# NVIDIA/tensorrt-laboratory

Measured on NVIDIA H100. Metric: ResNet-50 fp16 b=8 inferences/sec, higher is better.
Workload: dtype f16

## Files before the change

__graft_entry__.py:

```python
from __future__ import annotations

import os
import re
import shutil
import subprocess
import sysconfig
import sys

ROOT = os.path.dirname(os.path.abspath(__file__))
PKG = os.path.join(ROOT, "tensorrt_laboratory_b200")
CSRC = os.path.join(PKG, "csrc")
LIB = os.path.join(PKG, "libb200infer.so")

NVCC_FLAGS = [
    "-gencode", "arch=compute_90a,code=sm_90a", "-lineinfo", "-O3", "-std=c++17",
    "-Xcompiler", "-fPIC,-Wall,-Wno-unused-function", "-cudart", "static",
]


def _nvcc() -> str:
    for cand in (os.environ.get("NVCC"), shutil.which("nvcc"), "/usr/local/cuda/bin/nvcc"):
        if cand and os.path.exists(cand):
            return cand
    raise RuntimeError("nvcc not found")


def _sources():
    srcs = []
    for root, _, files in os.walk(CSRC):
        for f in sorted(files):
            if f.endswith((".cu", ".cc")) and not f.endswith(("_main.cc", "_module.cc")):
                srcs.append(os.path.join(root, f))
    return srcs


def _stale(target: str, deps) -> bool:
    if not os.path.exists(target):
        return True
    t = os.path.getmtime(target)
    for d in deps:
        if os.path.getmtime(d) > t:
            return True
    return False


def _all_deps():
    deps = []
    for root, _, files in os.walk(CSRC):
        deps += [os.path.join(root, f) for f in files if f.endswith((".cu", ".cc", ".h", ".cuh", ".hpp"))]
    deps.append(os.path.join(ROOT, "include", "b200infer.h"))
    inc = os.path.join(ROOT, "include")
    for root, _, files in os.walk(inc):
        deps += [os.path.join(root, f) for f in files]
    return deps


_CONV_KERNEL = re.compile(r"conv|attention_f16_wgmma|embed_ln|layernorm_h8|pooler|patchify|tokens_kernel|cls_head")


_SHARED_SM_KERNEL = re.compile(r"_ZN3b2k(?:16conv_f16_tcgen05|20conv3x3_halo_tcgen05|24conv3x3_halo_1x1_tcgen05)ILi(\d+)E")
_SHARED_SM_THREADS = 320


def _shared_sm_register_budget(bn: int):
    ctas = 3 if bn <= 64 else 2 if bn <= 128 else 1
    return None if ctas == 1 else 65536 // (_SHARED_SM_THREADS * ctas) // 8 * 8


def _ptxas_violations(log: str):
    bad = [line.strip() for line in log.splitlines() if "(C7520)" in line or "(C7518)" in line]
    func = None
    for line in log.splitlines():
        m = re.search(r"Function properties for (\S+)", line)
        if m:
            func = m.group(1)
            continue
        m = re.search(r"(\d+) bytes spill stores, (\d+) bytes spill loads", line)
        if m and func and _CONV_KERNEL.search(func) and (int(m.group(1)) or int(m.group(2))):
            bad.append(f"{func}: {line.strip()}")
        m = re.search(r"Used (\d+) registers", line)
        k = _SHARED_SM_KERNEL.match(func) if (m and func) else None
        if k:
            budget = _shared_sm_register_budget(int(k.group(1)))
            if budget is not None and int(m.group(1)) > budget:
                bad.append(f"{func}: {m.group(1)} registers, more than the {budget} at which its CTAs share an SM")
    return bad


def _compile_object(cmd, obj: str, verbose: bool) -> None:
    r = subprocess.run(cmd + ["-Xptxas", "-v"], capture_output=True, text=True)
    log = r.stdout + r.stderr
    shown = [line for line in log.splitlines() if verbose or not (line.startswith("ptxas info") or "bytes stack frame" in line)]
    if shown:
        sys.stderr.write("\n".join(shown) + "\n")
    if r.returncode:
        raise subprocess.CalledProcessError(r.returncode, cmd)
    bad = _ptxas_violations(log)
    if bad:
        os.remove(obj)
        raise RuntimeError(f"{os.path.basename(obj)}: ptxas reports serialised wgmma, spilling convolution / transformer "
                           "kernels or tile kernels over their register budget:\n  " +
                           "\n  ".join(bad))


def build(force: bool = False, verbose: bool = False) -> None:
    nvcc = _nvcc()
    objdir = os.path.join(ROOT, "build", "obj")
    os.makedirs(objdir, exist_ok=True)
    deps = _all_deps()
    objs = []
    for src in _sources():
        obj = os.path.join(objdir, os.path.relpath(src, CSRC).replace(os.sep, "_") + ".o")
        objs.append(obj)
        if force or _stale(obj, deps):
            cmd = [nvcc] + NVCC_FLAGS + ["-I", os.path.join(ROOT, "include"), "-I", CSRC]
            if src.endswith(".cc"):
                cmd += ["-x", "cu"]
            cmd += ["-c", src, "-o", obj]
            if verbose:
                print(" ".join(cmd))
            _compile_object(cmd, obj, verbose)
    if force or _stale(LIB, objs):
        cmd = [nvcc, "-shared", "-cudart", "static", "-o", LIB] + objs + ["-lpthread", "-ldl", "-lrt"]
        if verbose:
            print(" ".join(cmd))
        subprocess.run(cmd, check=True)
    main_src = os.path.join(CSRC, "trtlab", "infer_main.cc")
    exe = os.path.join(ROOT, "examples", "infer.x")
    os.makedirs(os.path.dirname(exe), exist_ok=True)
    if os.path.exists(main_src) and (force or _stale(exe, deps + [LIB])):
        cmd = [nvcc] + NVCC_FLAGS + ["-I", os.path.join(ROOT, "include"), "-I", CSRC, "-x", "cu", main_src,
                                     "-o", exe, "-L", PKG, "-lb200infer", "-Xlinker", "-rpath,$ORIGIN/../tensorrt_laboratory_b200",
                                     "-lpthread", "-ldl"]
        if verbose:
            print(" ".join(cmd))
        subprocess.run(cmd, check=True)
    py_src = os.path.join(CSRC, "pybind", "trtlab_module.cc")
    py_mod = os.path.join(PKG, "trtlab" + sysconfig.get_config_var("EXT_SUFFIX"))
    if os.path.exists(py_src) and (force or _stale(py_mod, deps + [LIB, py_src])):
        import pybind11
        cmd = [nvcc] + NVCC_FLAGS + ["-I", os.path.join(ROOT, "include"), "-I", CSRC, "-I", pybind11.get_include(),
                                     "-I", sysconfig.get_paths()["include"], "-Xcompiler", "-fvisibility=hidden", "-x", "cu", "-shared", py_src,
                                     "-o", py_mod,
# ... 25 lines not shown
```

tensorrt_laboratory_b200/csrc/engine.cu:

```cuda
#include <cuda.h>
#include <cuda_runtime.h>
#include <stdarg.h>
#include <stdio.h>
#include <stdlib.h>
#include <string.h>

#include <algorithm>
#include <map>
#include <memory>
#include <mutex>
#include <string>
#include <vector>

#include "../../include/b200infer.h"
#include "kernels.h"
#include "plan_format.h"

#include "b2_internal.h"

namespace b2i {
thread_local std::string g_err;
int fail(int code, const char* fmt, ...) {
    char buf[1024];
    va_list ap;
// ... 45 lines not shown
        }
        g_encode_im2col = reinterpret_cast<EncodeIm2colFn>(fn);
        cudaDriverGetVersion(&g_driver_version);
    });
    return g_driver_status;
}

size_t align_up(size_t v, size_t a) { return (v + a - 1) / a * a; }
constexpr size_t kSplitWorkspaceBytes = 12u << 20;
constexpr int kMaxSplitTiles = 4096;
constexpr int kSmemLimit = 227 * 1024;

int env_int(const char* name, int dflt) {
    const char* v = getenv(name);
    return v ? atoi(v) : dflt;
}

struct Tensor {
    std::string name;
    uint32_t kind, h, w, c, c_phys;
    int binding;
    float scale = 0.f;
    size_t item_bytes = 0;
    size_t offset = 0;
    int def = -1, last_use = -1;
};

struct Op {
    b2plan::OpRec r;
    int groups = 1;
    int heads = 0, vocab = 0, positions = 0, types = 0;
    int binding2 = -1, binding3 = -1, out2 = -1;
    float eps = 0.f;
    uint32_t flags = 0;
    std::string name;
    int side_join = -1;
    int kh() const { return int(r.k); }
    int kw() const { return int(r.kw ? r.kw : r.k); }
    int sh() const { return int(r.stride); }
    int sw() const { return int(r.kw ? r.stride_w : r.stride); }
    int ph() const { return int(r.pad_); }
    int pw_lo() const { return int(r.kw ? r.pad_w_lo : r.pad_); }
    int pw_hi() const { return int(r.kw ? r.pad_w_hi : r.pad_); }
    double algo_k() const { return r.ceil_mode ? double(r.ceil_mode) : double(r.cin / uint32_t(groups)) * r.taps; }
    int group_span() const {
        return groups > 1 && (r.relu & 2) ? std::max(int(r.cin) / groups, (r.relu & 4) ? 128 : 64) : 0;
    }
};

struct Binding {
    std::string name;
    bool is_input;
    int dtype;
    int tensor;
    int nd;
    int32_t dims[8];
    size_t item_bytes;
};

enum LKind { L_INPUT_CAST, L_CONV_TC, L_CONV_SIMT, L_MAXPOOL, L_AVGPOOL, L_FC, L_SOFTMAX, L_OUTPUT_CAST, L_TAIL, L_QUANTIZE, L_CONV_I8, L_AVGPOOL_I8, L_OUTPUT_CAST_I8,
             L_EMBED_LN, L_LAYERNORM, L_ATTENTION, L_POOLER, L_OUTPUT_ROWS, L_OUTPUT_UNPACK, L_QUANTIZE_F8, L_CONV_F8, L_AVGPOOL_F8,
             L_OUTPUT_CAST_F8, L_PATCHIFY, L_TOKENS, L_CLS_HEAD };

int attention_keys(int S) {
    for (int sk : {64, 128, 256, 384, 512})
        if (S <= sk) return sk;
    return 0;
}

struct Launch {
    LKind kind;
    std::string name;
    double flops = 0, bytes = 0;
    b2k::ConvLaunch conv;
    b2k::SimtConvArgs simt;
    const void* in = nullptr;
    void* out = nullptr;
    const void* w = nullptr;
    const float* bias = nullptr;
    int in_binding = -1, out_binding = -1;
    bool src_half = false;
    int max_blocks = 0;
    int side_join = -1;
    b2k::TailArgs tail{};
    b2k::I8ConvLaunch i8{};
    float qscale = 0.f;
    int C_in_phys = 0;
    b2k::EmbedArgs embed{};
    int in_binding2 = -1, in_binding3 = -1;
    b2k::AttnLaunch attn{};
    float eps = 0.f;
    const int* live = nullptr;
    const int* pos_map = nullptr;
    int N = 0, C = 0, H = 0, W = 0, C_phys = 0, Ho = 0, Wo = 0, k = 0, stride = 0, pad = 0, K = 0, Cout = 0;
};

struct Segment {
    int begin = 0, end = 0;
    bool graphable = false;
    cudaGraphExec_t exec = nullptr;
};
struct BindPatch {
    int launch = -1;
    cudaGraphNode_t node = nullptr;
    cudaKernelNodeParams np{};
    std::vector<void*> params;
    int n_params = 0;
    std::vector<std::pair<int, int>> slots;
    std::vector<void*> values;
    b2k::TailArgs tail{};
    bool is_tail = false;
};
struct Plan {
    int batch = 0;
    std::vector<Launch> launches;
    std::vector<Segment> segments;
    bool graph_failed = false;
    cudaGraph_t graph = nullptr;
    cudaGraphExec_t exec = nullptr;
    std::vector<BindPatch> patches;
    ~Plan() {
        for (Segment& sg : segments)
            if (sg.exec) cudaGraphExecDestroy(sg.exec);
        if (exec) cudaGraphExecDestroy(exec);
        if (graph) cudaGraphDestroy(graph);
    }
};

}

struct ConvConfig {
    int bn, stages, splits;
    double est_us;
    int sps = 1;
    int ws = 0;
    int cn = 1;
    int halo = 0;
};
static bool stage_depth_useful(int bn, int kb, int st, int kpc) {
    const int stgs[4] = {1, 2, 4, 8};
    int cover = 0, deepest = 0;
    for (int s2 : stgs) {
        if (!b2k::conv_config_exists(bn, kb, s2)) continue;
        deepest = s2;
        if (!cover && s2 >= kpc) cover = s2;
    }
    return st <= (cover ? cover : deepest);
}


constexpr int kHaloStagesTag = 2;

struct b2_runtime {
    b2_alloc_fn alloc = nullptr;
    b2_free_fn free_ = nullptr;
    void* user = nullptr;
};

struct b2_engine {
    b2_runtime* rt = nullptr;
    b2_alloc_fn alloc = nullptr;
    b2_free_fn free_ = nullptr;
    void* alloc_user = nullptr;
    std::string name;
    int precision = 0, max_batch = 0;
    std::vector<Tensor> tensors;
    std::vector<Op> ops;
    std::vector<Binding> bindings;
    uint8_t* d_payload = nullptr;
    size_t payload_bytes = 0;
    size_t arena_bytes = 0;
    size_t act_bytes = 0;
    int device = -1;
    bool inspect_only = false;
    double flops_per_item = 0;
    std::mutex tune_mutex;
    std::mutex tune_run_mutex;
    std::map<std::pair<int, int>, ConvConfig> tuned;
    bool tune_cache_loaded = false;
    std::map<int, float> requant_r;
    bool tactics_from_plan = false;
    bool tuned_at_load = false;
    int pack_tensor = -1;
    bool half() const { return precision != B2_PREC_FP32; }
    bool one_byte() const { return precision == B2_PREC_INT8 || precision == B2_PREC_FP8; }
    bool fp8() const { return precision == B2_PREC_FP8; }
};

struct b2_context {
    b2_engine* e = nullptr;
    uint8_t* scratch = nullptr;
    struct ScratchState {
        std::map<int, std::unique_ptr<Plan>> plans;
    };
    std::map<uint8_t*, ScratchState> states;
    ScratchState* cur = nullptr;
    int* d_counters = nullptr;
    int use_graph = 1;
    int force_simt = 0;
    int force_im2col = 0;
    int force_bn = 0;
    int force_stages = 0;
    int force_splits = 0;
    int force_sps = 0;
    int force_halo = 0;
    int force_fuse = 0;
    int force_cn = 0;
    int force_ws = 0;
    int pdl_trigger = 1;
    int no_fold = 0;
    int autotune = 4;
    int fork = 0;
    int i8_bn = 0;
    int i8_stages = 0;
    int fuse_tail = 1;
    int input_ctas = 0;
    int* d_tail_ctrl = nullptr;
    cudaStream_t side = nullptr;
    cudaEvent_t fork_ev = nullptr, join_ev = nullptr;
};

namespace {

std::string fixed_str(const char* p, size_t n) {
    size_t len = 0;
    while (len < n && p[len]) ++len;
    return std::string(p, len);
}

int validate_transformer_op(b2_engine* e, const Op& op) {
    using namespace b2plan;
    const OpRec& r = op.r;
    const char* nm = op.name.c_str();
    auto act_ok = [&](const Tensor& t) { return t.kind == T_ACT && t.scale == 0.f && t.c % 8 == 0 && t.c <= 1024; };
    switch (r.type) {
        case OP_EMBED_LN: {
            const Tensor& to = e->tensors[r.out];
            const Tensor& tm = e->tensors[op.out2];
            const uint32_t want_c = (op.flags & kOpPacked) ? to.w + 2 : to.w;
            if (!act_ok(to) || to.h != 1 || tm.kind != T_VEC || tm.c != want_c || tm.binding >= 0)
                return fail(B2_EINVAL, "plan: embedding %s: needs an fp16 [1, S, C <= 1024, C %% 8 == 0] output and an fp32 [S] mask tensor "
                            "([S + 2] packing index when packed)", nm);
            if ((op.flags & kOpPacked) && to.w % 32)
                return fail(B2_EINVAL, "plan: packed embedding %s: S = %u is not a multiple of 32", nm, to.w);
            if (op.vocab < 1 || op.types < 1 || op.positions < int(to.w))
                return fail(B2_EINVAL, "plan: embedding %s: vocab %d / positions %d / types %d do not cover S = %u", nm, op.vocab, op.positions,
                            op.types, to.w);
            if (r.w_bytes != uint64_t(op.vocab + op.positions + op.types) * to.c * 2 || r.b_bytes != uint64_t(to.c) * 8)
                return fail(B2_EINVAL, "plan: embedding %s: table / gamma / beta sizes do not match hidden size %u", nm, to.c);
            if (!(op.eps >= 0.f && op.eps < 1.f)) return fail(B2_EINVAL, "plan: embedding %s: bad eps", nm);
            break;
        }
        case OP_LAYERNORM: {
            const Tensor& ti = e->tensors[r.in];
            const Tensor& to = e->tensors[r.out];
            if (!act_ok(ti) || !act_ok(to) || ti.h != to.h || ti.w != to.w || ti.c != to.c || ti.c_phys != to.c_phys)
                return fail(B2_EINVAL, "plan: layernorm %s: needs fp16 input and output of one shape, C %% 8 == 0, C <= 1024", nm);
            if (r.w_bytes != 0 || r.b_bytes != uint64_t(ti.c) * 8) return fail(B2_EINVAL, "plan: layernorm %s: gamma / beta size mismatch", nm);
            if (!(op.eps >= 0.f && op.eps < 1.f)) return fail(B2_EINVAL, "plan: layernorm %s: bad eps", nm);
            break;
        }
        case OP_ATTENTION: {
            const Tensor& ti = e->tensors[r.in];
            const Tensor& to = e->tensors[r.out];
            if (r.res < 0) return fail(B2_EINVAL, "plan: attention %s: no mask tensor", nm);
            const Tensor& tm = e->tensors[r.res];
            if (op.heads < 1 || uint32_t(op.heads) * 64 != to.c)
                return fail(B2_EINVAL, "plan: attention %s: heads * 64 (%d * 64) != hidden size %u", nm, op.heads, to.c);
            if (!act_ok(to) || ti.kind != T_ACT || ti.scale != 0.f || ti.c != 3 * to.c || ti.c_phys != ti.c)
                return fail(B2_EINVAL, "plan: attention %s: needs a fused fp16 QKV input of 3 x %u channels", nm, to.c);
            if (ti.h != 1 || to.h != 1 || ti.w != to.w || tm.kind != T_VEC || tm.c != ((op.flags & kOpPacked) ? ti.w + 2 : ti.w))
                return fail(B2_EINVAL, "plan: attention %s: S does not match between QKV, output and mask", nm);
            if ((op.flags & kOpPacked) && (ti.w == 0 || ti.w > 512))
                return fail(B2_EINVAL, "plan: packed attention %s: S = %u (1 ... 512)", nm, ti.w);
            if (!(op.flags & kOpPacked) && ti.w != 64 && (ti.w == 0 || ti.w % 128 || ti.w > 512))
                return fail(B2_EINVAL, "plan: attention %s: S = %u (64, or a multiple of 128 up to 512)", nm, ti.w);
            if (r.w_bytes || r.b_bytes) return fail(B2_EINVAL, "plan: attention %s carries no weights", nm);
            e->flops_per_item += 4.0 * double(ti.w) * ti.w * to.c;
            break;
        }
        case OP_POOLER: {
            const Tensor& ti = e->tensors[r.in];
            const Tensor& to = e->tensors[r.out];
            if (!act_ok(ti) || ti.h != 1 || to.kind != T_VEC || to.c != ti.c)
                return fail(B2_EINVAL, "plan: pooler %s: needs an fp16 [1, S, C] input and an fp32 [C] output", nm);
            if (r.w_bytes != uint64_t(ti.c) * ti.c * 2 || r.b_bytes != uint64_t(ti.c) * 4)
                return fail(B2_EINVAL, "plan: pooler %s: weight / bias size mismatch", nm);
            e->flops_per_item += 2.0 * ti.c * ti.c;
            break;
// ... 295 lines not shown
            const Tensor& ti = e->tensors[r.in];
            const size_t K = size_t(ti.h) * ti.w * ti.c_phys;
            if (r.w_bytes != size_t(r.cout) * K * elt || r.b_bytes != size_t(r.cout) * 4)
                return fail(B2_EINVAL, "plan: fc %s weight size mismatch", op.name.c_str());
            e->flops_per_item += 2.0 * ti.h * ti.w * ti.c * r.cout;
        } else if (transformer_op) {
            int rc = validate_transformer_op(e, op);
            if (rc) return rc;
        }
        e->ops.push_back(op);
    }
    if (int rc = validate_packed_ops(e)) return rc;
    for (uint32_t i = 0; i < h.n_bindings; ++i, p += sizeof(BindingRec)) {
        BindingRec r;
        memcpy(&r, p, sizeof r);
        Binding b;
        b.name = fixed_str(r.name, 64);
        b.is_input = r.is_input != 0;
        b.dtype = r.dtype;
        b.tensor = r.tensor;
        b.nd = r.nd;
        if (r.nd == 0 || r.nd > 8) return fail(B2_EINVAL, "plan: binding %s has bad rank", b.name.c_str());
        if (r.dtype != B2_DT_FLOAT && !(r.dtype == B2_DT_HALF && b.is_input && h.precision == B2_PREC_FP16) &&
            !(r.dtype == B2_DT_INT32 && b.is_input && v3))
            return fail(B2_EINVAL, "plan: binding %s: bindings are fp32 (inputs of fp16 engines may be fp16)", b.name.c_str());
        size_t n = 1;
        for (uint32_t d = 0; d < 8; ++d) {
            b.dims[d] = d < r.nd ? r.dims[d] : 0;
            if (d < r.nd) n *= size_t(r.dims[d]);
        }
        b.item_bytes = n * (r.dtype == B2_DT_HALF ? 2 : 4);
        e->bindings.push_back(b);
    }
    for (const Op& op : e->ops) {
        const OpRec& r = op.r;
        if (r.type != OP_INPUT_CAST && r.type != OP_OUTPUT_CAST) continue;
        const Binding& b = e->bindings[size_t(r.binding)];
        const Tensor& t = e->tensors[size_t(r.type == OP_INPUT_CAST ? r.out : r.in)];
        size_t n = 1;
        for (int d = 0; d < b.nd; ++d) n *= size_t(b.dims[d] > 0 ? b.dims[d] : 0);
        const bool s2d = r.type == OP_INPUT_CAST && r.k == 2;
        if (b.is_input != (r.type == OP_INPUT_CAST) || (!s2d && n != size_t(t.c) * t.h * t.w))
            return fail(B2_EINVAL, "plan: cast op %s: binding %s and tensor %s disagree", op.name.c_str(), b.name.c_str(), t.name.c_str());
        if (b.dtype == B2_DT_INT32)
            return fail(B2_EINVAL, "plan: cast op %s reads int32 binding %s (int32 bindings feed the embedding op only)", op.name.c_str(),
                        b.name.c_str());
    }
    for (const Op& op : e->ops)
        if (op.r.type == OP_PATCHIFY)
            if (int rc = validate_patchify_binding(e, op)) return rc;
    std::vector<int> int32_readers(e->bindings.size(), 0);
    for (const Op& op : e->ops) {
        const OpRec& r = op.r;
        if (r.type == OP_POOLER && e->tensors[r.out].binding >= 0 && e->bindings[size_t(e->tensors[r.out].binding)].is_input)
            return fail(B2_EINVAL, "plan: pooler %s writes an input binding", op.name.c_str());
        if (r.type != OP_EMBED_LN) continue;
        const uint32_t S = e->tensors[r.out].w;
        for (int bi : {r.binding, op.binding2, op.binding3}) {
            if (bi < 0 || bi >= int(h.n_bindings)) return fail(B2_EINVAL, "plan: embedding %s has a bad binding", op.name.c_str());
            const Binding& b = e->bindings[size_t(bi)];
            if (b.dtype != B2_DT_INT32 || !b.is_input || b.nd != 1 || b.dims[0] != int32_t(S))
                return fail(B2_EINVAL, "plan: embedding %s: binding %s must be an int32 input of shape [S = %u]", op.name.c_str(), b.name.c_str(), S);
            ++int32_readers[size_t(bi)];
        }
    }
    for (size_t i = 0; i < e->bindings.size(); ++i) {
        if (e->bindings[i].dtype != B2_DT_INT32) continue;
        if (int32_readers[i] != 1)
            return fail(B2_EINVAL, "plan: int32 binding %s must feed exactly one embedding op slot", e->bindings[i].name.c_str());
        for (const Tensor& t : e->tensors)
            if (t.binding == int(i))
                return fail(B2_EINVAL, "plan: int32 binding %s is the storage of tensor %s (int32 bindings feed the embedding op only)",
                            e->bindings[i].name.c_str(), t.name.c_str());
    }
    if (h.n_tactics) {
        if (h.tactics_offset > nbytes || size_t(h.n_tactics) > (nbytes - h.tactics_offset) / sizeof(TacticRec))
            return fail(B2_EINVAL, "plan: tactic table outside the blob");
        for (uint32_t i = 0; i < h.n_tactics; ++i) {
            TacticRec t;
            memcpy(&t, base + h.tactics_offset + size_t(i) * sizeof(TacticRec), sizeof t);
            if (t.op >= h.n_ops || t.batch == 0 || t.batch > h.max_batch) return fail(B2_EINVAL, "plan: tactic %u out of range", i);
            ConvConfig cfg{int(t.bn), int(t.stages), int(t.splits), 0.0, int(t.sps), int(t.ws), int(t.cn)};
            cfg.halo = int(t.halo);
            e->tuned[{int(t.op), int(t.batch)}] = cfg;
        }
        e->tactics_from_plan = true;
    }
    *payload = base + h.payload_offset;
    return B2_OK;
}

int fuse_partner(const b2_engine* e, int i);

void plan_arena(b2_engine* e) {
    int busy_until = -1;
    for (size_t i = 0; i < e->ops.size(); ++i) {
        Op& op = e->ops[i];
        op.side_join = -1;
        if (int(i) <= busy_until || op.r.type != b2plan::OP_CONV || op.r.out < 0 || e->tensors[op.r.out].binding >= 0) continue;
        int consumers = 0, join = -1;
        bool as_residual_only = true;
        for (size_t k = i + 1; k < e->ops.size(); ++k) {
            const auto& rk = e->ops[k].r;
            if (rk.in == op.r.out) ++consumers, as_residual_only = false;
            if (rk.res == op.r.out) ++consumers, join = int(k);
        }
        if (consumers == 1 && as_residual_only && join > int(i) + 1) {
            op.side_join = join;
            busy_until = join;
        }
    }
    for (size_t i = 0; i < e->ops.size(); ++i) {
        const auto& r = e->ops[i].r;
        for (int t : {r.out, e->ops[i].out2})
            if (t >= 0 && e->tensors[t].def < 0) e->tensors[t].def = int(i);
        for (int t : {r.in, r.res})
            if (t >= 0) e->tensors[t].last_use = std::max(e->tensors[t].last_use, int(i));
        if (e->ops[i].side_join >= 0 && r.in >= 0) e->tensors[r.in].last_use = std::max(e->tensors[r.in].last_use, e->ops[i].side_join);
        const int j = fuse_partner(e, int(i));
        if (j >= 0) e->tensors[r.in].last_use = std::max(e->tensors[r.in].last_use, j);
    }
    if (e->pack_tensor >= 0) e->tensors[size_t(e->pack_tensor)].last_use = int(e->ops.size()) - 1;
    struct Live {
        size_t off, size;
        int last;
    };
    std::vector<Live> live;
    size_t top = 0;
    std::vector<int> order;
    for (size_t i = 0; i < e->tensors.size(); ++i)
        if (e->tensors[i].binding < 0 && e->tensors[i].def >= 0) order.push_back(int(i));
    std::stable_sort(order.begin(), order.end(), [&](int a, int b) { return e->tensors[a].def < e->tensors[b].def; });
    for (int ti : order) {
        Tensor& t = e->tensors[ti];
        if (t.last_use < t.def) t.last_use = t.def;
        const size_t size = align_up(t.item_bytes * e->max_batch, 1024);
        live.erase(std::remove_if(live.begin(), live.end(), [&](const Live& l) { return l.last < t.def; }), live.end());
        std::sort(live.begin(), live.end(), [](const Live& a, const Live& b) { return a.off < b.off; });
        size_t off = 0;
        for (const Live& l : live) {
            if (off + size <= l.off) break;
            off = std::max(off, l.off + l.size);
        }
        t.offset = off;
        live.push_back({off, size, t.last_use});
        top = std::max(top, off + size);
    }
    e->act_bytes = align_up(std::max<size_t>(top, 1024), 1024);
    e->arena_bytes = e->act_bytes + (e->half() ? kSplitWorkspaceBytes : 0);
}

int make_map_2d(CUtensorMap* map, const void* base, uint64_t inner, uint64_t outer, uint32_t box_inner,
                uint32_t box_outer, CUtensorMapSwizzle swz, bool int8 = false) {
    cuuint64_t dims[2] = {inner, outer};
    cuuint64_t strides[1] = {inner * (int8 ? 1u : 2u)};
    cuuint32_t box[2] = {box_inner, box_outer};
    cuuint32_t estr[2] = {1, 1};
    CUresult r = g_encode_tiled(map, int8 ? CU_TENSOR_MAP_DATA_TYPE_UINT8 : CU_TENSOR_MAP_DATA_TYPE_FLOAT16, 2, const_cast<void*>(base), dims, strides, box,
                                estr, CU_TENSOR_MAP_INTERLEAVE_NONE, swz, CU_TENSOR_MAP_L2_PROMOTION_L2_256B,
                                CU_TENSOR_MAP_FLOAT_OOB_FILL_NONE);
    if (r != CUDA_SUCCESS)
        return fail(B2_ECUDA, "cuTensorMapEncodeTiled failed (%d) dims=%llu,%llu box=%u,%u", int(r),
                    (unsigned long long)inner, (unsigned long long)outer, box_inner, box_outer);
    return B2_OK;
}

// ... 42 lines not shown
        if (cout_phys % bn || (group_span && group_span % bn)) continue;
        if (honor_forced && c->force_bn && bn != c->force_bn) continue;
        const int tiles = m_tiles * (cout_phys / bn);
        for (int splits = 1; splits <= 8; ++splits) {
            if (honor_forced && c->force_splits && !group_span ? splits != c->force_splits : splits != 1) continue;
            if (splits > 1 && (kb != 64 || kblocks / splits < 4 || tiles * splits > 160 || tiles > kMaxSplitTiles ||
                               size_t(tiles) * splits * 128 * bn * 4 > kSplitWorkspaceBytes))
                continue;
            const int kpc = (kblocks + splits - 1) / splits;
            if (splits > 1 && (splits - 1) * kpc >= kblocks) continue;
            for (int st : stgs) {
                if (!b2k::conv_config_exists(bn, kb, st)) continue;
                if (b2k::conv_smem_bytes(bn, st, residual) > kSmemLimit) continue;
                if (honor_forced && c->force_stages && st != c->force_stages) continue;
                if (!(honor_forced && c->force_stages) && !stage_depth_useful(bn, kb, st, kpc)) continue;
                const int per_sm = std::max(1, b2k::conv_residency(bn, kb, st, 1, residual));
                const int ctas = tiles * splits;
                const int waves = (ctas + g_sms * per_sm - 1) / (g_sms * per_sm);
                const int sharing = std::max(1, std::min(per_sm, (ctas + g_sms - 1) / g_sms));
                const double stage_bytes = 16384.0 + bn * 128.0;
                const double t_kb = std::max(stage_bytes / (70000.0 / sharing), 1.0 / st);
                double t_epi = 0.6 + bn / 64.0 * 0.4 + (residual ? 0.4 : 0.0);
                if (splits > 1) t_epi += 1.0 + 0.3 * splits;
                const double t_cta = 2.0 + kpc * t_kb + t_epi;
                double total = waves * t_cta;
                const double traffic = double(ctas) * kpc * stage_bytes;
                total = std::max(total, traffic / 5.0e6 + 2.0);
                if (total < best.est_us) best = ConvConfig{bn, st, splits, total};
            }
        }
    }
    return best;
}

bool conv_is_row_folded(const b2_context* c, const Op& op) {
    const b2plan::OpRec& r = op.r;
    return !c->no_fold && r.cin_phys == 8 && op.kw() * 8 * 2 == 64 && op.sw() == 1 && op.pw_lo() == 0 && op.pw_hi() == 0;
}
int conv_kb(const b2_context* c, const Op& op) {
    if (op.r.cin_phys % 64 == 0) return 64;
    return conv_is_row_folded(c, op) ? 32 : 8;
}
int conv_num_kblocks(const b2_context* c, const Op& op) {
    const b2plan::OpRec& r = op.r;
    if (op.group_span()) return int(r.taps) * (op.group_span() / 64);
    if (r.cin_phys % 64 == 0) return int(r.taps) * (int(r.cin_phys) / 64);
    if (conv_is_row_folded(c, op)) return (op.kh() + 1) / 2;
    return (int(r.taps_phys) + 7) / 8;
}

int conv_halo_rows(const b2_engine* e, const Op& op) {
    const b2plan::OpRec& r = op.r;
    const Tensor& ti = e->tensors[r.in];
    const Tensor& to = e->tensors[r.out];
    if (op.groups > 1 || r.cin_phys % 64 || r.cout_phys % 64 || op.kh() != 3 || op.kw() != 3 || op.sh() != 1 || op.sw() != 1 || op.ph() != 1 ||
        op.pw_lo() != 1 || op.pw_hi() != 1 || r.res >= 0 || !(r.relu & 2) || ti.h != to.h || ti.w != to.w)
        return 0;
    const int wp = int(to.w) + 2;
    if (wp > 128) return 0;
    return std::min(128 / wp, int(to.h));
}
int conv_halo_rows(const b2_context* c, const Op& op) { return conv_halo_rows(c->e, op); }
bool conv_on_tensor_cores(const b2_engine* e, const Op& op);

int fuse_partner(const b2_engine* e, int i) {
    if (!e->half() || e->one_byte() || i < 0 || size_t(i) + 1 >= e->ops.size()) return -1;
    const Op &oi = e->ops[size_t(i)], &oj = e->ops[size_t(i) + 1];
    const b2plan::OpRec &ri = oi.r, &rj = oj.r;
    if (ri.type != b2plan::OP_CONV || rj.type != b2plan::OP_CONV || (ri.relu & (4 | b2plan::kConvGelu)) || conv_halo_rows(e, oi) == 0 ||
        !b2k::conv_halo_config_exists(int(ri.cout_phys)) || ri.cin_phys / 64 > 8)
        return -1;
    if (rj.in != ri.out || rj.res < 0 || rj.res == ri.out || oj.kh() != 1 || oj.kw() != 1 || oj.sh() != 1 || oj.sw() != 1 || oj.ph() != 0 ||
        oj.pw_lo() != 0 || oj.pw_hi() != 0 || oj.groups != 1 || !(rj.relu & 2) || (rj.relu & (4 | b2plan::kConvGelu)) ||
        rj.cin_phys != ri.cout_phys || rj.cout_phys % 64 || !conv_on_tensor_cores(e, oj) || e->tensors[ri.out].binding >= 0)
        return -1;
    for (size_t k = 0; k < e->ops.size(); ++k) {
        const b2plan::OpRec& rk = e->ops[k].r;
        if (k != size_t(i) + 1 && (rk.in == ri.out || rk.res == ri.out || e->ops[k].out2 == ri.out)) return -1;
        if (k == size_t(i) + 1 && rk.res == ri.out) return -1;
    }
    return i + 1;
}

bool conv_on_tensor_cores(const b2_engine* e, const Op& op) {
    const b2plan::OpRec& r = op.r;
    const bool kb64 = r.cin_phys % 64 == 0, kb8 = r.cin_phys == 8;
    return e->half() && (kb64 || kb8) && r.cout_phys % 32 == 0 && (kb64 || r.taps_phys % 2 == 0) && (op.groups == 1 || op.group_span() > 0);
}

bool conv_takes_stem_ws(const b2_context* c, const Op& op) {
    const b2plan::OpRec& r = op.r;
    return conv_is_row_folded(c, op) && op.kh() == 7 && op.sh() == 2 && r.cout_phys == 64 && c->e->tensors[r.out].w <= 128 &&
           (r.relu & b2plan::kConvRelu) && !(r.relu & 2) && !(r.relu & b2plan::kConvGelu) && r.res < 0 && op.groups == 1;
}

bool conv_takes_ws(const b2_context* c, const Op& op) {
    return conv_takes_stem_ws(c, op) || (conv_kb(c, op) == 64 && (op.r.relu & 2) && op.groups == 1 && !(op.r.relu & b2plan::kConvGelu));
}

bool tactic_applies(const b2_context* c, const Op& op, int batch, const ConvConfig& cfg) {
    const b2plan::OpRec& r = op.r;
    const Tensor& to = c->e->tensors[r.out];
    const int span = op.group_span(), kb = conv_kb(c, op);
    if (cfg.bn <= 0 || int(r.cout_phys) % cfg.bn || cfg.splits < 1 || cfg.sps < 1 || cfg.ws < 0) return false;
    if (op.groups > 1 && (!span || span % cfg.bn || cfg.splits > 1)) return false;
    if ((op.groups > 1 || (r.relu & b2plan::kConvGelu)) && (cfg.ws || cfg.cn > 1 || cfg.halo)) return false;
    if ((op.flags & b2plan::kOpPacked) && (cfg.ws || cfg.cn > 1 || cfg.halo || cfg.splits > 1)) return false;
    if (cfg.halo == 2) {
        const int j = fuse_partner(c->e, int(&op - &c->e->ops[0]));
        const int R = conv_halo_rows(c, op), cblocks = int(r.cin_phys) / 64;
        return j >= 0 && c->force_fuse >= 0 && cfg.bn == int(r.cout_phys) && cfg.splits == 1 && !cfg.ws && cfg.cn <= 1 &&
               b2k::conv_halo_fused_smem(cfg.bn, int(to.w), R, cblocks, int(c->e->ops[size_t(j)].r.cout_phys)) <= kSmemLimit;
    }
    if (cfg.halo) {
        const int R = conv_halo_rows(c, op), cblocks = int(r.cin_phys) / 64;
        return cfg.halo == 1 && R && cfg.splits == 1 && !cfg.ws && cfg.cn <= 1 && b2k::conv_halo_config_exists(cfg.bn) && cblocks <= 8 &&
               b2k::conv_halo_smem(cfg.bn, int(to.w), R, cblocks) <= kSmemLimit;
    }
    if (cfg.ws && conv_is_row_folded(c, op))
        return conv_takes_stem_ws(c, op) && cfg.bn == 64 && cfg.stages == b2k::kStemWsRing && cfg.sps == 1 && cfg.splits == 1 &&
               cfg.cn <= 1 && b2k::conv_stem_ws_smem() <= kSmemLimit;
    if (cfg.ws)
        return conv_takes_ws(c, op) && cfg.splits == 1 && cfg.cn <= 1 && b2k::conv_ws_config_exists(cfg.bn, cfg.stages, cfg.sps) &&
               b2k::conv_ws_smem(cfg.bn, cfg.stages, cfg.sps, r.res >= 0) <= kSmemLimit;
    if (!b2k::conv_config_exists(cfg.bn, kb, cfg.stages, cfg.sps) || b2k::conv_smem_bytes(cfg.bn, cfg.stages, r.res >= 0, cfg.sps) > kSmemLimit)
        return false;
    const int grid_n = int(r.cout_phys) / cfg.bn;
    if (cfg.cn > 1 && (kb != 64 || grid_n % cfg.cn || !b2k::conv_cluster_config_exists(cfg.bn, cfg.stages, cfg.sps, cfg.cn))) return false;
    if (cfg.splits > 1) {
        const int nkb = conv_num_kblocks(c, op), kpc = (nkb + cfg.splits - 1) / cfg.splits;
        const int tiles = (batch * int(to.h * to.w) + 127) / 128 * grid_n;
        if (kb != 64 || kpc < 4 || (cfg.splits - 1) * kpc >= nkb || tiles > kMaxSplitTiles ||
            size_t(tiles) * cfg.splits * 128 * cfg.bn * 4 > kSplitWorkspaceBytes)
            return false;
    }
    return true;
}

constexpr int kFuseMinStreams = 4;

ConvConfig fused_conv_config(const Op& op) {
    ConvConfig f{int(op.r.cout_phys), kHaloStagesTag, 1, 0.0, 1, 0, 1};
    f.halo = 2;
    return f;
}

std::vector<ConvConfig> conv_candidates(const b2_context* c, const Op& op, int batch, int fixed_splits) {
    const b2plan::OpRec& r = op.r;
    const int kbsz = conv_kb(c, op), nkb = conv_num_kblocks(c, op);
    const int m_tiles = (batch * int(c->e->tensors[r.out].h * c->e->tensors[r.out].w) + 127) / 128;
    const bool ws_only = c->force_ws > 0 && conv_takes_ws(c, op);
    auto ok = [&](const ConvConfig& t) { return tactic_applies(c, op, batch, t); };
    std::vector<ConvConfig> out;
    for (int bn : {256, 128, 64, 32}) {
        if (int(r.cout_phys) % bn) continue;
        const int tiles = m_tiles * (int(r.cout_phys) / bn);
        for (int ws = 0; ws <= 1; ++ws)
        for (int sp : {1, 2, 4, 8})
        for (int sps = 1; sps <= 2; ++sps)
        for (int st : {1, 2, 4, 8}) {
            if ((fixed_splits > 0 && sp != fixed_splits) || (ws ? c->force_ws < 0 : ws_only)) continue;
            ConvConfig t{bn, st, sp, 0.0, sps, ws ? std::min(tiles, g_sms) : 0, 1};
            if (!ok(t)) continue;
            if (ws) {
                if (sps == 2 && nkb < 4) continue;
                out.push_back(t);
                if (tiles > g_sms / 2) t.ws = g_sms / 2, out.push_back(t);
                continue;
            }
            const int kpc = (nkb + sp - 1) / sp;
            if (sps == 2 ? (kpc < 4 || st * 2 > kpc + 2) : !stage_depth_useful(bn, kbsz, st, kpc)) continue;
            if (sp > 1 && (tiles >= 100 || tiles > kMaxSplitTiles / 8 || tiles * sp > 160)) continue;
            ConvConfig cl = t;
            cl.cn = c->force_cn;
            out.push_back(c->force_cn > 1 && ok(cl) ? cl : t);
        }
    }
    if (conv_takes_stem_ws(c, op) && c->force_ws >= 0 && fixed_splits <= 1) {
        const int rows = batch * int(c->e->tensors[r.out].h);
        ConvConfig t{64, b2k::kStemWsRing, 1, 0.0, 1, std::min(rows, g_sms), 1};
        if (ok(t)) {
            out.push_back(t);
            if (rows > g_sms / 2) t.ws = g_sms / 2, out.push_back(t);
        }
    }
    if (c->force_halo >= 0 && fixed_splits <= 1) {
        std::vector<ConvConfig> halo;
        for (int bn : {256, 128, 64, 32}) {
            const ConvConfig h{bn, kHaloStagesTag, 1, 0.0, 1, 0, 1, 1};
            if (ok(h)) halo.push_back(h);
        }
        if (!halo.empty() && c->force_halo > 0) out.clear();
        out.insert(out.end(), halo.begin(), halo.end());
    }
    return out;
}

ConvConfig forced_conv_config(const b2_context* c, const Op& op, int batch) {
    const b2plan::OpRec& r = op.r;
    const int M = batch * int(c->e->tensors[r.out].h * c->e->tensors[r.out].w);
    const int kbsz = conv_kb(c, op), nkb = conv_num_kblocks(c, op);
    ConvConfig cfg = pick_conv_config(M, int(r.cout_phys), nkb, kbsz, r.res >= 0, c, true, op.group_span());
    if (cfg.bn == 0 || ((op.flags & b2plan::kOpPacked) && cfg.splits > 1))
        cfg = pick_conv_config(M, int(r.cout_phys), nkb, kbsz, r.res >= 0, c, false, op.group_span());
    if (cfg.bn == 0) return cfg;
    auto force = [&](auto set) {
        ConvConfig t = cfg;
        set(t);
        if (tactic_applies(c, op, batch, t)) cfg = t;
    };
    if (c->force_sps == 2) force([](ConvConfig& t) { t.sps = 2; });
    if (c->force_ws > 0)
        force([&](ConvConfig& t) {
            if (conv_takes_stem_ws(c, op)) {
                t = ConvConfig{64, b2k::kStemWsRing, 1, t.est_us, 1, 0, 1};
                t.ws = std::min(batch * int(c->e->tensors[r.out].h), c->force_ws > 1 ? c->force_ws : g_sms);
                return;
            }
            t.ws = std::min((M + 127) / 128 * (int(r.cout_phys) / t.bn), c->force_ws > 1 ? c->force_ws : g_sms);
        });
    if (c->force_halo > 0) force([](ConvConfig& t) { t.halo = 1, t.ws = 0, t.cn = 1; });
    if (c->force_cn > 1) force([&](ConvConfig& t) { t.cn = c->force_cn; });
    return cfg;
}

int make_conv_launch(b2_context* c, const Op& op, int batch, const ConvConfig& cfg, b2k::ConvLaunch* out) {
    b2_engine* e = c->e;
// ... 23 lines not shown
    cl.cn = std::max(cfg.cn, 1);
    cl.args.cn = cl.cn;
    cl.args.tiles_m = cl.grid_m;
    cl.args.tiles_n = cl.grid_n;
    b2k::ConvArgs& a = cl.args;
    a.splits = cfg.splits;
    a.kb_per_split = (nkb + cfg.splits - 1) / cfg.splits;
    a.workspace = reinterpret_cast<float*>(c->scratch + e->act_bytes);
    a.tile_counters = c->d_counters;
    a.pdl_trigger = c->pdl_trigger;
    a.bias = reinterpret_cast<const float*>(e->d_payload + r.b_off);
    a.residual = r.res >= 0 ? reinterpret_cast<const __half*>(tptr(r.res)) : nullptr;
    a.out = reinterpret_cast<__half*>(tptr(r.out));
    a.M = M;
    a.Cout = int(r.cout_phys);
    a.taps = fold ? op.kh() : int(r.taps);
    a.taps_phys = fold ? op.kh() : int(r.taps_phys);
    a.kw = fold ? 1 : op.kw();
    a.cblocks = span ? span / 64 : kb64 ? int(r.cin_phys) / 64 : 1;
    a.group_span = span;
    a.num_kblocks = nkb;
    a.HoWo = int(to.h * to.w);
    a.Wo = int(to.w);
    a.stride_h = op.sh();
    a.stride_w = op.sw();
    a.pad_h = op.ph();
    a.pad_w = op.pw_lo();
    a.relu = int(r.relu & (b2plan::kConvRelu | b2plan::kConvGelu));
    a.wpacked = (r.relu & 2) ? w : nullptr;
    const bool tiled = r.k == 1 && op.kw() == 1 && r.stride == 1 && op.sw() == 1 && r.pad_ == 0 && op.pw_lo() == 0 &&
                       op.pw_hi() == 0 && kb64 && (!c->force_im2col || gelu || (op.flags & b2plan::kOpPacked));
    a.a_mode = tiled ? b2k::A_TILED : b2k::A_IM2COL;
    if (cfg.halo) {
        const int R = conv_halo_rows(c, op);
        cl.halo = 1;
        cl.ws_ctas = 0, cl.cn = 1, a.cn = 1, a.splits = 1, cl.stages = kHaloStagesTag, cl.sps = 1;
        a.halo_rows = R;
        cl.grid_m = batch * ((int(to.h) + R - 1) / R);
        int rc = make_map_nhwc(&cl.mapA, tptr(r.in), int(r.cin_phys), int(ti.w), int(ti.h), batch, uint32_t(ti.w) + 2, uint32_t(R) + 2);
        if (rc) return rc;
        cl.mapB = cl.mapA;
        if (cfg.halo == 2) {
            const Op& oj = e->ops[size_t(fuse_partner(e, int(&op - &e->ops[0])))];
            const b2plan::OpRec& rj = oj.r;
            cl.halo = 2;
            cl.c2.wpacked = e->d_payload + rj.w_off;
            cl.c2.bias = reinterpret_cast<const float*>(e->d_payload + rj.b_off);
            cl.c2.Cout = int(rj.cout_phys);
            cl.c2.relu = int(rj.relu & b2plan::kConvRelu);
            rc = make_map_nhwc(&cl.mapOut, tptr(rj.out), int(rj.cout_phys), int(to.w), int(to.h), batch, uint32_t(to.w) + 2, uint32_t(R));
            if (!rc) rc = make_map_nhwc(&cl.mapRes, tptr(rj.res), int(rj.cout_phys), int(to.w), int(to.h), batch, uint32_t(to.w) + 2, uint32_t(R));
            return rc;
        }
        rc = make_map_nhwc(&cl.mapOut, tptr(r.out), int(r.cout_phys), int(to.w), int(to.h), batch, uint32_t(to.w) + 2, uint32_t(R));
        cl.mapRes = cl.mapOut;
        return rc;
    }
    const CUtensorMapSwizzle swz = kb64 ? CU_TENSOR_MAP_SWIZZLE_128B : (fold ? CU_TENSOR_MAP_SWIZZLE_64B : CU_TENSOR_MAP_SWIZZLE_NONE);
    const uint64_t pix = uint64_t(r.cin_phys) * 2, rowb = uint64_t(ti.w) * pix, imgb = uint64_t(ti.h) * rowb;
    int rc;
    if (tiled)
        rc = make_map_2d(&cl.mapA, tptr(r.in), r.cin_phys, uint64_t(M), 64, uint32_t(128 / cl.cn), swz);
    else if (fold)
        rc = make_map_im2col(&cl.mapA, tptr(r.in), int(r.cin_phys) * op.kw(), int(ti.w) - op.kw() + 1, int(ti.h), batch, pix,
                             rowb, imgb, op.kh(), 1, op.sh(), 1, op.ph(), 0, 0, 32, 128, swz);
    else
        rc = make_map_im2col(&cl.mapA, tptr(r.in), int(r.cin_phys), int(ti.w), int(ti.h), batch, pix, rowb, imgb, op.kh(),
                             op.kw(), op.sh(), op.sw(), op.ph(), op.pw_lo(), op.pw_hi(), uint32_t(cl.kb), uint32_t(128 / cl.cn), swz);
    if (rc) return rc;
    if (r.relu & 2)
        cl.mapB = cl.mapA;
    else
        rc = make_map_2d(&cl.mapB, w, uint64_t(r.taps_phys) * r.cin_phys, r.cout_phys, uint32_t(cl.kb), uint32_t(cl.bn), swz);
    if (rc) return rc;
    if (cfg.ws && fold) {
        rc = make_map_nhwc(&cl.mapOut, tptr(r.out), int(r.cout_phys), int(to.w), int(to.h), batch, 128, 1);
        cl.mapRes = cl.mapOut;
        return rc;
    }
    const uint32_t ow = cl.bn >= 64 ? 64 : 32;
    const CUtensorMapSwizzle oswz = cl.bn >= 64 ? CU_TENSOR_MAP_SWIZZLE_128B : CU_TENSOR_MAP_SWIZZLE_64B;
    rc = make_map_2d(&cl.mapOut, tptr(r.out), r.cout_phys, uint64_t(M), ow, 128, oswz);
    if (rc) return rc;
    if (r.res >= 0) rc = make_map_2d(&cl.mapRes, tptr(r.res), r.cout_phys, uint64_t(M), ow, 128, oswz);
    else cl.mapRes = cl.mapOut;
    return rc;
}

int make_i8_conv_launch(b2_context* c, const Op& op, int batch, int bn, int stages, b2k::I8ConvLaunch* out) {
    b2_engine* e = c->e;
    const b2plan::OpRec& r = op.r;
    const Tensor& ti = e->tensors[r.in];
    const Tensor& to = e->tensors[r.out];
    auto tptr = [&](int idx) -> uint8_t* { return c->scratch + e->tensors[idx].offset; };
    b2k::I8ConvLaunch& cl = *out;
    memset(&cl, 0, sizeof cl);
    const int M = batch * int(to.h) * int(to.w);
    cl.bn = bn, cl.stages = stages;
    cl.grid_m = (M + 127) / 128;
    cl.grid_n = int(r.cout_phys) / bn;
    b2k::I8ConvArgs& a = cl.args;
    a.wpacked = e->d_payload + r.w_off;
    const float* rq = reinterpret_cast<const float*>(e->d_payload + r.b_off);
    a.m = rq;
    a.b = rq + r.cout_phys;
    a.r = e->requant_r.at(int(&op - &e->ops[0]));
    a.has_res = r.res >= 0 ? 1 : 0;
    a.relu = int(r.relu & 1);
    a.M = M, a.Cout = int(r.cout_phys);
    const int span = op.group_span(), cpg = int(r.cin) / op.groups;
    a.group_span = span;
    cl.group_mode = !span ? 0 : cpg <= 32 ? 32 : cpg == 64 ? 64 : 128;
    a.cblocks = (span ? span : int(r.cin_phys)) / 128;
    a.last_cb_mmas = (int(r.cin) % 128) ? (int(r.cin) % 128 + 31) / 32 : 4;
    a.cout_real = int(r.cout);
    a.num_kblocks = int(r.taps) * a.cblocks;
    a.kw = op.kw(), a.HoWo = int(to.h * to.w), a.Wo = int(to.w);
    a.stride_h = op.sh(), a.stride_w = op.sw(), a.pad_h = op.ph(), a.pad_w = op.pw_lo();
    const bool tiled = r.k == 1 && r.stride == 1 && r.pad_ == 0;
    a.a_mode = tiled ? b2k::A_TILED : b2k::A_IM2COL;
    int rc;
    if (tiled)
        rc = make_map_2d(&cl.mapA, tptr(r.in), r.cin_phys, uint64_t(M), 128, 128, CU_TENSOR_MAP_SWIZZLE_128B, true);
    else {
        const uint64_t pix = uint64_t(r.cin_phys), rowb = uint64_t(ti.w) * pix, imgb = uint64_t(ti.h) * rowb;
        rc = make_map_im2col(&cl.mapA, tptr(r.in), int(r.cin_phys), int(ti.w), int(ti.h), batch, pix, rowb, imgb, op.kh(), op.kw(), op.sh(),
                             op.sw(), op.ph(), op.pw_lo(), op.pw_hi(), 128, 128, CU_TENSOR_MAP_SWIZZLE_128B, true);
    }
    if (rc) return rc;
    rc = make_map_2d(&cl.mapOut, tptr(r.out), r.cout_phys, uint64_t(M), 128, 128, CU_TENSOR_MAP_SWIZZLE_128B, true);
    if (rc) return rc;
    if (r.res >= 0) rc = make_map_2d(&cl.mapRes, tptr(r.res), r.cout_phys, uint64_t(M), 128, 128, CU_TENSOR_MAP_SWIZZLE_128B, true);
    else cl.mapRes = cl.mapOut;
    return rc;
}

struct TuneTimer {
    const int ns;
    const int iters = std::max(4, env_int("B2_TUNE_ITERS", 12));
    const int reps = std::max(1, env_int("B2_TUNE_REPS", 3));
    std::vector<cudaStream_t> ss;
    std::vector<cudaEvent_t> done;
    cudaEvent_t e0 = nullptr, e1 = nullptr;

    explicit TuneTimer(const b2_context* c) : ns(std::max(1, std::min(c->autotune, 8))), ss(size_t(ns), nullptr), done(size_t(ns), nullptr) {}
    ~TuneTimer() {
        for (auto s : ss)
            if (s) cudaStreamDestroy(s);
        for (auto d : done)
            if (d) cudaEventDestroy(d);
        if (e0) cudaEventDestroy(e0);
        if (e1) cudaEventDestroy(e1);
    }
    int init() {
        bool ok = cudaEventCreate(&e0) == cudaSuccess && cudaEventCreate(&e1) == cudaSuccess;
        for (int i = 0; i < ns && ok; ++i)
            ok = cudaStreamCreateWithFlags(&ss[size_t(i)], cudaStreamNonBlocking) == cudaSuccess &&
                 cudaEventCreateWithFlags(&done[size_t(i)], cudaEventDisableTiming) == cudaSuccess;
        if (ok) return B2_OK;
        cudaGetLastError();
        return fail(B2_ECUDA, "autotune: cannot create streams/events");
    }
    template <class F>
    cudaError_t time(F launch, float* ms) {
        int rc = 0;
        for (int i = 0; i < 2 && !rc; ++i)
            for (int k = 0; k < ns && !rc; ++k) rc = launch(k, ss[size_t(k)]);
        for (auto s : ss) cudaStreamSynchronize(s);
        *ms = 1e30f;
// ... 2 lines not shown
        cudaGraphExec_t ge = nullptr;
        cudaError_t se = cudaStreamBeginCapture(ss[0], cudaStreamCaptureModeThreadLocal);
        if (se != cudaSuccess) return se;
        cudaEventRecord(done[0], ss[0]);
        for (int k = 1; k < ns; ++k) cudaStreamWaitEvent(ss[size_t(k)], done[0], 0);
        for (int i = 0; i < iters && !rc; ++i)
            for (int k = 0; k < ns && !rc; ++k) rc = launch(k, ss[size_t(k)]);
        for (int k = 1; k < ns; ++k) {
            cudaEventRecord(done[size_t(k)], ss[size_t(k)]);
            cudaStreamWaitEvent(ss[0], done[size_t(k)], 0);
        }
        se = cudaStreamEndCapture(ss[0], &g);
        if (!rc && se == cudaSuccess) se = cudaGraphInstantiate(&ge, g, 0);
        if (!rc && se == cudaSuccess) se = cudaGraphLaunch(ge, ss[0]);
        if (!rc && se == cudaSuccess) se = cudaStreamSynchronize(ss[0]);
        for (int rep = 0; rep < reps && !rc && se == cudaSuccess; ++rep) {
            cudaEventRecord(e0, ss[0]);
            se = cudaGraphLaunch(ge, ss[0]);
            cudaEventRecord(e1, ss[0]);
            if (se == cudaSuccess) se = cudaStreamSynchronize(ss[0]);
            float t = 0.f;
            if (se == cudaSuccess && cudaEventElapsedTime(&t, e0, e1) == cudaSuccess) *ms = std::min(*ms, t);
        }
        if (ge) cudaGraphExecDestroy(ge);
        if (g) cudaGraphDestroy(g);
        if (rc || se != cudaSuccess) cudaGetLastError();
        return rc ? cudaError_t(rc) : se;
    }
    double us_per_launch(double ms) const { return ms * 1e3 / (iters * ns); }
};

int autotune_conv(b2_context* c, const Op& op, int batch, int fixed_splits, ConvConfig* best_out) {
    const b2plan::OpRec& r = op.r;
    const Tensor& to = c->e->tensors[r.out];
    const int M = batch * int(to.h) * int(to.w);
    TuneTimer tt(c);
    int status = tt.init();
    if (status) return status;
    const int verbose = env_int("B2_TUNE_VERBOSE", 0);
    ConvConfig best = *best_out;
    double best_ms = 1e30;
    for (const ConvConfig& cand : conv_candidates(c, op, batch, fixed_splits)) {
        b2k::ConvLaunch cl0;
        if ((status = make_conv_launch(c, op, batch, cand, &cl0))) return status;
        std::vector<b2k::ConvLaunch> cls(size_t(tt.ns), cl0);
        void* tmp_ws = nullptr;
        if (cand.splits > 1) {
            const size_t ws_bytes = size_t(cl0.grid_m) * cl0.grid_n * cand.splits * 128 * cand.bn * 4;
            if (cudaMalloc(&tmp_ws, ws_bytes * tt.ns) != cudaSuccess) {
                cudaGetLastError();
                continue;
            }
            for (int k = 0; k < tt.ns; ++k) {
                cls[size_t(k)].args.workspace = reinterpret_cast<float*>(static_cast<uint8_t*>(tmp_ws) + ws_bytes * k);
                cls[size_t(k)].args.tile_counters = c->d_counters + k * (kMaxSplitTiles / 8);
            }
        }
        float ms = 0.f;
        const cudaError_t err = tt.time([&](int k, cudaStream_t s) { return b2k::launch_conv_f16_tcgen05(cls[size_t(k)], s); }, &ms);
        if (tmp_ws) cudaFree(tmp_ws);
        if (err != cudaSuccess)
            return fail(B2_ECUDA, "autotune of %s (bn=%d st=%d) failed: %s", op.name.c_str(), cand.bn, cand.stages, cudaGetErrorString(err));
        if (verbose > 1)
            fprintf(stderr, "[b2 tune]   %s b=%d cand bn=%d st=%d sp=%d sps=%d ws=%d cn=%d halo=%d : %.3f us/launch\n", op.name.c_str(),
                    batch, cand.bn, cand.stages, cand.splits, cand.sps, cand.ws, cand.cn, cand.halo, tt.us_per_launch(ms));
        if (ms < best_ms) best_ms = ms, best = cand;
    }
    best.est_us = tt.us_per_launch(best_ms);
    if (verbose)
        fprintf(stderr, "[b2 tune] %s b=%d M=%d N=%d K=%d best bn=%d st=%d sp=%d sps=%d ws=%d cn=%d halo=%d : %.3f us/launch (%d streams)\n",
                op.name.c_str(), batch, M, int(r.cout_phys), conv_num_kblocks(c, op) * conv_kb(c, op), best.bn, best.stages, best.splits,
                best.sps, best.ws, best.cn, best.halo, best.est_us, tt.ns);
    *best_out = best;
    return B2_OK;
}

void tune_cache_load(b2_engine* e) {
    if (e->tune_cache_loaded) return;
    e->tune_cache_loaded = true;
    const char* path = getenv("B2_TUNE_CACHE");
    if (!path) return;
    FILE* f = fopen(path, "r");
    if (!f) return;
    char name[128];
    int op, batch, bn, st, sp, sps, ws, cn, halo;
    while (fscanf(f, "%127s %d %d %d %d %d %d %d %d %d", name, &op, &batch, &bn, &st, &sp, &sps, &ws, &cn, &halo) == 10)
        if (e->name == name && op >= 0 && op < int(e->ops.size())) {
            ConvConfig cfg{bn, st, sp, 0.0, sps, ws, cn};
            cfg.halo = halo;
            e->tuned[{op, batch}] = cfg;
        }
    fclose(f);
}
void tune_cache_append(const b2_engine* e, int op, int batch, const ConvConfig& cfg) {
    const char* path = getenv("B2_TUNE_CACHE");
    if (!path) return;
    FILE* f = fopen(path, "a");
    if (!f) return;
    fprintf(f, "%s %d %d %d %d %d %d %d %d %d\n", e->name.c_str(), op, batch, cfg.bn, cfg.stages, cfg.splits, cfg.sps, cfg.ws, cfg.cn,
            cfg.halo);
    fclose(f);
}

bool i8_bn_fits(const Op& op, int bn) {
    const int span = op.group_span();
    return int(op.r.cout_phys) % bn == 0 && (!span || span % bn == 0);
}
bool i8_tactic_ok(const Op& op, int bn, int stages) { return i8_bn_fits(op, bn) && b2k::conv_i8_config_exists(bn, stages); }

int autotune_i8_conv(b2_context* c, const Op& op, int batch, ConvConfig* best_out) {
    const b2plan::OpRec& r = op.r;
    TuneTimer tt(c);
    int status = tt.init();
    if (status) return status;
    const int verbose = env_int("B2_TUNE_VERBOSE", 0);
    const bool fp8 = c->e->fp8();
    const char* fmt = fp8 ? "fp8" : "int8";
    double best_ms = 1e30;
    ConvConfig best = *best_out;
    for (int bn : {128, 256}) {
        for (int st = 1; st <= 4; ++st) {
            if (!i8_tactic_ok(op, bn, st)) continue;
            b2k::I8ConvLaunch cl;
            if ((status = make_i8_conv_launch(c, op, batch, bn, st, &cl))) return status;
            float ms = 0.f;
            const cudaError_t err = tt.time(
                [&](int, cudaStream_t s) { return fp8 ? b2k::launch_conv_f8_tcgen05(cl, s) : b2k::launch_conv_i8_tcgen05(cl, s); }, &ms);
            if (err != cudaSuccess)
                return fail(B2_ECUDA, "autotune of %s (%s bn=%d st=%d) failed: %s", op.name.c_str(), fmt, bn, st, cudaGetErrorString(err));
            if (verbose > 1)
                fprintf(stderr, "[b2 tune]   %s b=%d cand %s bn=%d st=%d : %.3f us/launch\n", op.name.c_str(), batch, fmt, bn, st,
                        tt.us_per_launch(ms));
            if (ms < best_ms) best_ms = ms, best = ConvConfig{bn, st, 1, 0.0, 1, 0, 1};
        }
    }
    best.est_us = tt.us_per_launch(best_ms);
    if (verbose) {
        const Tensor& to = c->e->tensors[r.out];
        const long long M = (long long)batch * to.h * to.w, K = (long long)r.k * r.k * r.cin_phys;
        fprintf(stderr, "[b2 tune] %s b=%d M=%lld N=%d K=%lld best %s bn=%d st=%d : %.3f us/launch (%d streams) %.0f TOP/s\n",
                op.name.c_str(), batch, M, int(r.cout_phys), K, fmt, best.bn, best.stages, best.est_us, tt.ns,
                2.0 * M * r.cout_phys * K / best.est_us * 1e-6);
    }
    *best_out = best;
    return B2_OK;
}

int tune_engine_batch(b2_context* c, int batch) {
    b2_engine* e = c->e;
    for (size_t i = 0; i < e->ops.size(); ++i) {
        const Op& op = e->ops[i];
        const b2plan::OpRec& r = op.r;
        if (r.type != b2plan::OP_CONV || !e->half()) continue;
        if (r.relu & 4) {
            {
                std::lock_guard<std::mutex> lock(e->tune_mutex);
                if (e->tuned.count({int(i), batch})) continue;
            }
            ConvConfig cfg{128, 2, 1, 0.0, 1, 0, 1};
            int rc = autotune_i8_conv(c, op, batch, &cfg);
            if (rc) return rc;
            std::lock_guard<std::mutex> lock(e->tune_mutex);
            e->tuned[{int(i), batch}] = cfg;
            tune_cache_append(e, int(i), batch, cfg);
            continue;
        }
        if (!conv_on_tensor_cores(e, op)) continue;
        {
            std::lock_guard<std::mutex> lock(e->tune_mutex);
            if (e->tuned.count({int(i), batch})) continue;
        }
        const Tensor& to = e->tensors[r.out];
        const int kbsz = conv_kb(c, op), nkb = conv_num_kblocks(c, op);
        const bool side = op.side_join >= 0;
        const bool no_split = side || op.groups > 1;
        static const bool tune_splitk = env_int("B2_TUNE_SPLITK", 0) != 0;
        int splits = (no_split || !tune_splitk) ? 1 : 0;
        if (batch != e->max_batch && !no_split && tune_splitk) {
            std::lock_guard<std::mutex> lock(e->tune_mutex);
            auto it = e->tuned.find({int(i), e->max_batch});
            if (it != e->tuned.end()) splits = it->second.splits;
        }
        ConvConfig cfg = pick_conv_config(batch * int(to.h) * int(to.w), int(r.cout_phys), nkb, kbsz, r.res >= 0, c, false,
                                          op.group_span());
        int rc = autotune_conv(c, op, batch, splits, &cfg);
        if (rc) return rc;
        std::lock_guard<std::mutex> lock(e->tune_mutex);
        e->tuned[{int(i), batch}] = cfg;
        tune_cache_append(e, int(i), batch, cfg);
    }
    for (size_t i = 0; i < e->ops.size() && c->force_fuse >= 0 && c->autotune >= kFuseMinStreams; ++i) {
        const Op& op = e->ops[i];
        const int j = fuse_partner(e, int(i));
        if (j < 0) continue;
        double unfused_us = 0;
        {
            std::lock_guard<std::mutex> lock(e->tune_mutex);
            const auto a = e->tuned.find({int(i), batch}), b = e->tuned.find({j, batch});
            if (a == e->tuned.end() || b == e->tuned.end() || a->second.halo == 2 || !(a->second.est_us > 0) || !(b->second.est_us > 0)) continue;
            unfused_us = a->second.est_us + b->second.est_us;
        }
        ConvConfig f = fused_conv_config(op);
        if (!tactic_applies(c, op, batch, f)) continue;
        b2k::ConvLaunch cl;
        int rc = make_conv_launch(c, op, batch, f, &cl);
        if (rc) return rc;
        TuneTimer tt(c);
        if ((rc = tt.init())) return rc;
        float ms = 0.f;
        const cudaError_t err = tt.time([&](int, cudaStream_t s) { return b2k::launch_conv_f16_tcgen05(cl, s); }, &ms);
        if (err != cudaSuccess) return fail(B2_ECUDA, "autotune of %s fused with %s failed: %s", op.name.c_str(), e->ops[size_t(j)].name.c_str(), cudaGetErrorString(err));
        f.est_us = tt.us_per_launch(ms);
        if (env_int("B2_TUNE_VERBOSE", 0))
            fprintf(stderr, "[b2 tune] %s+%s b=%d fused : %.3f us/launch against %.3f unfused (%d streams) -> %s\n", op.name.c_str(),
                    e->ops[size_t(j)].name.c_str(), batch, f.est_us, unfused_us, tt.ns, f.est_us < unfused_us ? "fused" : "unfused");
        if (f.est_us < unfused_us) {
            std::lock_guard<std::mutex> lock(e->tune_mutex);
            e->tuned[{int(i), batch}] = f;
            tune_cache_append(e, int(i), batch, f);
        }
    }
    return B2_OK;
}

void fuse_bottlenecks(b2_context* c, Plan* plan, int batch) {
    std::vector<Launch>& ls = plan->launches;
    if (std::none_of(ls.begin(), ls.end(), [](const Launch& L) { return L.kind == L_CONV_TC && L.conv.halo == 2; })) return;
    std::vector<int> new_index(ls.size());
    std::vector<Launch> out;
    for (size_t k = 0; k < ls.size(); ++k) {
        new_index[k] = int(out.size());
        if (ls[k].kind == L_CONV_TC && ls[k].conv.halo == 2 && k + 1 < ls.size()) {
            Launch& J = ls[k + 1];
            Launch L = std::move(ls[k]);
            const Tensor& mid = c->e->tensors[c->e->ops[k].r.out];
            L.name += "+" + J.name;
            L.flops += J.flops;
            L.bytes += J.bytes - 2.0 * batch * double(mid.item_bytes);
            new_index[k + 1] = new_index[k];
            ++k;
            out.push_back(std::move(L));
            continue;
        }
        out.push_back(std::move(ls[k]));
    }
    for (Launch& L : out)
        if (L.side_join >= 0) L.side_join = new_index[size_t(L.side_join)];
    ls = std::move(out);
}

void fuse_tail(b2_context* c, Plan* plan, int batch) {
    if (!c->fuse_tail || !c->e->half()) return;
    std::vector<Launch>& ls = plan->launches;
    for (size_t i = 0; i + 2 < ls.size(); ++i) {
        const Launch &P = ls[i], &F = ls[i + 1], &S = ls[i + 2];
        if (P.kind != L_AVGPOOL || F.kind != L_FC || S.kind != L_SOFTMAX) continue;
        if (F.in != P.out || S.in != F.out || F.out_binding >= 0 || S.in_binding >= 0 || S.out_binding < 0 || P.C_phys % 8) continue;
        if (F.K != P.C_phys || S.C != F.Cout || !b2k::tail_f16_applies(batch, P.H * P.W, P.C_phys, F.Cout)) continue;
        Launch T;
        T.kind = L_TAIL;
        T.name = P.name + "+" + F.name + "+" + S.name;
        T.N = batch;
        T.flops = F.flops, T.bytes = P.bytes + F.bytes + S.bytes;
        T.out_binding = S.out_binding;
        T.tail.in = static_cast<const __half*>(P.in);
        T.tail.w = static_cast<const __half*>(F.w);
        T.tail.bias = F.bias;
        T.tail.pooled = static_cast<__half*>(P.out);
        T.tail.logits = static_cast<float*>(F.out);
        T.tail.ctrl = c->d_tail_ctrl;
        T.tail.N = batch, T.tail.HW = P.H * P.W, T.tail.C = P.C_phys, T.tail.Cout = F.Cout;
        ls[i] = std::move(T);
        ls.erase(ls.begin() + long(i) + 1, ls.begin() + long(i) + 3);
        return;
    }
}

int build_plan(b2_context* c, int batch, Plan** out) {
    b2_engine* e = c->e;
    if (!c->scratch || !c->cur) return fail(B2_ESTATE, "b2_context_set_device_memory has not been called");
    auto it = c->cur->plans.find(batch);
    if (it != c->cur->plans.end()) {
        *out = it->second.get();
        return B2_OK;
    }
    if (load_driver_entry_points() != 0) return fail(B2_ECUDA, "cuTensorMapEncode* driver entry points unavailable");
    auto plan = std::make_unique<Plan>();
    plan->batch = batch;
    const bool half = e->half();
    const size_t elt = half ? 2 : 4;
    auto tptr = [&](int ti) -> uint8_t* {
        const Tensor& t = e->tensors[ti];
        return t.binding >= 0 ? nullptr : c->scratch + t.offset;
    };
    int* pos_map = nullptr;
    int* seq_off = nullptr;
    if (e->pack_tensor >= 0) {
        pos_map = reinterpret_cast<int*>(tptr(e->pack_tensor));
        seq_off = pos_map + size_t(batch) * (e->tensors[size_t(e->pack_tensor)].c - 2);
    }
    for (const Op& op : e->ops) {
        const b2plan::OpRec& r = op.r;
        Launch L;
        L.name = op.name;
        L.N = batch;
        L.side_join = op.side_join;
        switch (r.type) {
            case b2plan::OP_INPUT_CAST: {
                const Tensor& t = e->tensors[r.out];
                L.kind = L_INPUT_CAST;
                L.in_binding = r.binding;
                L.src_half = e->bindings[r.binding].dtype == B2_DT_HALF;
                L.out = tptr(r.out);
                L.C = t.c, L.H = t.h, L.W = t.w, L.C_phys = t.c_phys;
                L.k = int(r.k);
                L.max_blocks = c->input_ctas;
                if (r.k == 2) {
                    const Binding& b = e->bindings[r.binding];
                    if (!half || b.nd != 3 || b.dims[0] > 4 || t.c_phys != 8 || int(t.h) != b.dims[1] ||
                        int(t.w) != b.dims[2] / 2 + int(r.pad_) + int(r.stride) || b.dims[2] % 2)
                        return fail(B2_EINVAL, "input cast %s: inconsistent space-to-depth geometry", op.name.c_str());
                    L.C = b.dims[0], L.W = b.dims[2];
                    L.pad = int(r.pad_), L.stride = int(r.stride);
                }
                L.bytes = double(batch) * t.h * t.w * (t.c * 4.0 + t.c_phys * elt);
                break;
            }
            case b2plan::OP_QUANTIZE: {
                const Tensor& ti = e->tensors[r.in];
                const Tensor& to = e->tensors[r.out];
                L.kind = e->fp8() ? L_QUANTIZE_F8 : L_QUANTIZE;
                L.in = tptr(r.in), L.out = tptr(r.out);
                L.C = ti.c, L.H = ti.h, L.W = ti.w, L.C_in_phys = ti.c_phys, L.C_phys = to.c_phys;
                L.qscale = float(1.0 / double(to.scale));
                L.bytes = double(batch) * (ti.item_bytes + to.item_bytes);
                break;
            }
            case b2plan::OP_OUTPUT_CAST: {
                const Tensor& t = e->tensors[r.in];
                L.kind = t.scale > 0.f ? (e->fp8() ? L_OUTPUT_CAST_F8 : L_OUTPUT_CAST_I8) : (op.flags & b2plan::kOpPacked) ? L_OUTPUT_UNPACK : (op.flags & 1) ? L_OUTPUT_ROWS : L_OUTPUT_CAST;
                if (L.kind == L_OUTPUT_UNPACK) L.pos_map = pos_map;
                if (L.kind == L_OUTPUT_ROWS && !half) return fail(B2_EINVAL, "output cast %s: channels-last outputs need an fp16 engine", op.name.c_str());
                L.qscale = t.scale;
                L.in = tptr(r.in);
                L.out_binding = r.binding;
                L.C = t.c, L.H = t.h, L.W = t.w, L.C_phys = t.c_phys;
                L.bytes = double(batch) * t.h * t.w * (t.c * 4.0 + t.c_phys * elt);
                break;
            }
            case b2plan::OP_CONV: {
                const Tensor& ti = e->tensors[r.in];
                const Tensor& to = e->tensors[r.out];
                const uint8_t* w = e->d_payload + r.w_off;
                const float* bias = reinterpret_cast<const float*>(e->d_payload + r.b_off);
                const int M = batch * int(to.h) * int(to.w);
                L.flops = 2.0 * M * r.cout * op.algo_k();
                L.bytes = double(batch) * (ti.item_bytes + to.item_bytes * (r.res >= 0 ? 2 : 1)) + double(r.w_bytes);
                if (r.relu & 4) {
                    L.kind = e->fp8() ? L_CONV_F8 : L_CONV_I8;
                    const int m_tiles = (batch * int(e->tensors[r.out].h * e->tensors[r.out].w) + 127) / 128;
                    int bn = 128, st = m_tiles * (int(r.cout_phys) / 128) >= 2 * g_sms ? 1 : 2;
                    if (c->autotune) {
                        std::lock_guard<std::mutex> lock(e->tune_mutex);
                        tune_cache_load(e);
                        const int op_index = int(&op - &e->ops[0]);
                        auto it = e->tuned.find({op_index, batch});
                        if (it == e->tuned.end()) it = e->tuned.find({op_index, e->max_batch});
                        if (it != e->tuned.end()) bn = it->second.bn, st = it->second.stages;
                    }
                    if (c->i8_bn > 0) bn = c->i8_bn;
                    if (c->i8_stages > 0) st = c->i8_stages;
                    if (!i8_bn_fits(op, bn)) bn = 128;
                    if (!i8_tactic_ok(op, bn, st)) bn = 128, st = 2;
                    int rc = make_i8_conv_launch(c, op, batch, bn, st, &L.i8);
                    if (rc) return rc;
                } else if (!c->force_simt && conv_on_tensor_cores(e, op)) {
                    L.kind = L_CONV_TC;
                    ConvConfig cfg = forced_conv_config(c, op, batch);
                    if (cfg.bn == 0) return fail(B2_EINVAL, "conv %s: no kernel configuration", op.name.c_str());
                    const bool forced = c->force_bn || c->force_stages || c->force_splits || c->force_sps;
                    const int op_index = int(&op - &e->ops[0]);
                    if (!forced && c->autotune) {
                        std::lock_guard<std::mutex> lock(e->tune_mutex);
                        tune_cache_load(e);
                        auto it = e->tuned.find({op_index, batch});
                        if (it == e->tuned.end()) it = e->tuned.find({op_index, e->max_batch});
                        if (it != e->tuned.end() && tactic_applies(c, op, batch, it->second)) cfg = it->second;
                    }
                    if (c->force_fuse > 0) {
                        const ConvConfig f = fused_conv_config(op);
                        if (tactic_applies(c, op, batch, f)) cfg = f;
                    }
                    if (op.side_join >= 0 && cfg.splits > 1) cfg.splits = 1;
                    int rc = make_conv_launch(c, op, batch, cfg, &L.conv);
                    if (rc) return rc;
                    if (op.flags & b2plan::kOpPacked) L.conv.args.live_rows = seq_off + batch, L.conv.args.live = 1;
                } else {
                    L.kind = L_CONV_SIMT;
                    b2k::SimtConvArgs& a = L.simt;
                    memset(&a, 0, sizeof a);
                    a.in = tptr(r.in), a.w = w, a.bias = bias;
                    a.residual = r.res >= 0 ? tptr(r.res) : nullptr;
                    a.out = tptr(r.out);
                    a.N = batch, a.H = int(ti.h), a.W = int(ti.w), a.Cin = int(r.cin), a.Cin_phys = int(r.cin_phys);
                    a.Ho = int(to.h), a.Wo = int(to.w), a.Cout = int(r.cout), a.Cout_phys = int(r.cout_phys);
                    a.kh = op.kh(), a.kw = op.kw(), a.taps_phys = int(r.taps_phys);
                    a.stride_h = op.sh(), a.stride_w = op.sw(), a.pad_h = op.ph(), a.pad_w = op.pw_lo();
                    a.relu = int(r.relu & (b2plan::kConvRelu | b2plan::kConvGelu));
                    a.w_packed = int((r.relu >> 1) & 1);
                    a.groups = op.groups;
                    a.wk_tap = op.groups == 1 ? int(r.cin_phys) : op.group_span() ? op.group_span() : int(r.cin) / op.groups;
                }
                break;
            }
            case b2plan::OP_MAXPOOL: {
                const Tensor& ti = e->tensors[r.in];
                const Tensor& to = e->tensors[r.out];
                L.kind = L_MAXPOOL;
                L.in = tptr(r.in), L.out = tptr(r.out);
                L.H = ti.h, L.W = ti.w, L.C_phys = ti.c_phys, L.Ho = to.h, L.Wo = to.w;
                L.k = r.k, L.stride = r.stride, L.pad = r.pad_;
                L.bytes = double(batch) * (ti.item_bytes + to.item_bytes);
                break;
            }
            case b2plan::OP_AVGPOOL: {
                const Tensor& ti = e->tensors[r.in];
                L.kind = ti.scale > 0.f ? (e->fp8() ? L_AVGPOOL_F8 : L_AVGPOOL_I8) : L_AVGPOOL;
                L.in = tptr(r.in), L.out = tptr(r.out);
                L.H = ti.h, L.W = ti.w, L.C_phys = ti.c_phys;
                if (ti.scale > 0.f) {
                    L.C = ti.c, L.C_in_phys = ti.c_phys, L.C_phys = e->tensors[r.out].c_phys;
                    L.qscale = float(double(ti.scale) / double(ti.h * ti.w));
                }
                L.bytes = double(batch) * ti.item_bytes;
                break;
            }
            case b2plan::OP_FC: {
                const Tensor& ti = e->tensors[r.in];
                const Tensor& to = e->tensors[r.out];
                L.kind = L_FC;
                L.in = tptr(r.in);
                L.out = tptr(r.out);
                L.out_binding = to.binding;
                L.w = e->d_payload + r.w_off;
                L.bias = reinterpret_cast<const float*>(e->d_payload + r.b_off);
                L.K = int(ti.h * ti.w * ti.c_phys);
                L.Cout = int(r.cout);
                L.flops = 2.0 * batch * ti.h * ti.w * ti.c * r.cout;
                L.bytes = double(r.w_bytes) + double(batch) * (ti.item_bytes + to.item_bytes);
                break;
            }
            case b2plan::OP_SOFTMAX: {
                const Tensor& ti = e->tensors[r.in];
                const Tensor& to = e->tensors[r.out];
                L.kind = L_SOFTMAX;
                L.in = tptr(r.in);
                L.in_binding = ti.binding;
                L.out = tptr(r.out);
                L.out_binding = to.binding;
                L.C = int(ti.c);
                L.bytes = double(batch) * ti.c * 8.0;
                break;
            }
            case b2plan::OP_EMBED_LN: {
                const Tensor& to = e->tensors[r.out];
                L.kind = L_EMBED_LN;
                L.in_binding = r.binding, L.in_binding2 = op.binding2, L.in_binding3 = op.binding3;
                b2k::EmbedArgs& a = L.embed;
                a.tables = reinterpret_cast<const __half*>(e->d_payload + r.w_off);
                a.gamma = reinterpret_cast<const float*>(e->d_payload + r.b_off);
                a.beta = a.gamma + to.c;
                a.out = reinterpret_cast<__half*>(tptr(r.out));
                if (op.flags & b2plan::kOpPacked) a.pack = reinterpret_cast<int*>(tptr(op.out2));
                else a.mask_add = reinterpret_cast<float*>(tptr(op.out2));
                a.N = batch, a.S = int(to.w), a.C = int(to.c), a.C_phys = int(to.c_phys);
// ... 7 lines not shown
                L.in = tptr(r.in), L.out = tptr(r.out);
                L.bias = reinterpret_cast<const float*>(e->d_payload + r.b_off);
                L.H = int(ti.h) * int(ti.w), L.C = int(ti.c), L.C_phys = int(ti.c_phys), L.eps = op.eps;
                if (op.flags & b2plan::kOpPacked) L.live = seq_off + batch;
                L.bytes = 2.0 * batch * ti.item_bytes;
                break;
            }
            case b2plan::OP_ATTENTION: {
                const Tensor& ti = e->tensors[r.in];
                const Tensor& to = e->tensors[r.out];
                L.kind = L_ATTENTION;
                b2k::AttnLaunch& a = L.attn;
                if (op.flags & b2plan::kOpPacked) a.seq_off = seq_off;
                else a.mask_add = reinterpret_cast<const float*>(tptr(r.res));
                a.out = reinterpret_cast<__half*>(tptr(r.out));
                a.N = batch, a.S = int(ti.w), a.heads = op.heads, a.H = int(to.c), a.out_pitch = int(to.c_phys);
                if (op.flags & b2plan::kOpPacked) a.S = attention_keys(int(ti.w));
                L.W = int(ti.w);
                int rc = make_map_2d(&a.mapQKV, tptr(r.in), ti.c_phys, uint64_t(batch) * ti.w, 64, 64, CU_TENSOR_MAP_SWIZZLE_128B);
                if (rc) return rc;
                L.flops = 4.0 * batch * double(ti.w) * ti.w * to.c;
                L.bytes = double(batch) * (ti.item_bytes + to.item_bytes);
                break;
            }
            case b2plan::OP_POOLER: {
                const Tensor& ti = e->tensors[r.in];
                const Tensor& to = e->tensors[r.out];
                L.kind = L_POOLER;
                L.in = tptr(r.in);
                L.out = tptr(r.out);
                L.out_binding = to.binding;
                L.w = e->d_payload + r.w_off;
                L.bias = reinterpret_cast<const float*>(e->d_payload + r.b_off);
                L.W = int(ti.w), L.C = int(ti.c), L.C_phys = int(ti.c_phys);
                if (op.flags & b2plan::kOpPacked) L.pos_map = pos_map;
                L.flops = 2.0 * batch * ti.c * ti.c;
                L.bytes = double(r.w_bytes) + double(batch) * (ti.c * 2.0 + to.item_bytes);
                break;
            }
            case b2plan::OP_PATCHIFY: {
                const Tensor& to = e->tensors[r.out];
                const Binding& b = e->bindings[r.binding];
                L.kind = L_PATCHIFY;
                L.in_binding = r.binding;
                L.out = tptr(r.out);
                L.H = b.dims[1], L.W = b.dims[2], L.k = int(r.k);
                L.max_blocks = c->input_ctas;
                L.bytes = double(batch) * (3.0 * b.dims[1] * b.dims[2] * 4 + to.item_bytes);
                break;
            }
            case b2plan::OP_TOKENS: {
                const Tensor& ti = e->tensors[r.in];
                const Tensor& to = e->tensors[r.out];
                L.kind = L_TOKENS;
                L.in = tptr(r.in), L.out = tptr(r.out);
                L.w = e->d_payload + r.w_off;
                L.pos_map = pos_map;
                L.W = int(to.w), L.C = int(to.c);
                L.flops = double(batch) * to.w * to.c;
                L.bytes = double(batch) * (ti.item_bytes + to.item_bytes + (to.w + 2) * 4.0) + double(r.w_bytes);
                break;
            }
            case b2plan::OP_CLS_HEAD: {
                const Tensor& ti = e->tensors[r.in];
                const Tensor& to = e->tensors[r.out];
                L.kind = L_CLS_HEAD;
                L.in = tptr(r.in);
                L.out = tptr(r.out);
                L.out_binding = to.binding;
                L.w = e->d_payload + r.w_off;
                L.bias = reinterpret_cast<const float*>(e->d_payload + r.b_off);
                L.W = int(ti.w), L.C = int(ti.c), L.Cout = int(r.cout), L.eps = op.eps;
                if (op.flags & b2plan::kOpPacked) L.pos_map = pos_map;
                L.flops = 2.0 * batch * double(r.cout) * ti.c;
                L.bytes = double(r.w_bytes) + double(batch) * (ti.c * 2.0 + to.item_bytes);
                break;
            }
            default:
                return fail(B2_EINVAL, "op %s: unknown type", op.name.c_str());
        }
        plan->launches.push_back(std::move(L));
    }
    fuse_bottlenecks(c, plan.get(), batch);
    fuse_tail(c, plan.get(), batch);
    {
        const std::vector<Launch>& ls = plan->launches;
        size_t i = 0;
        while (i < ls.size()) {
            const bool dep = ls[i].in_binding >= 0 || ls[i].out_binding >= 0;
            size_t j = i + 1;
            if (!dep)
                while (j < ls.size() && ls[j].in_binding < 0 && ls[j].out_binding < 0) ++j;
            Segment sg;
            sg.begin = int(i), sg.end = int(j);
            sg.graphable = !dep && (j - i) >= 3;
            plan->segments.push_back(sg);
            i = j;
        }
    }
    *out = plan.get();
    c->cur->plans[batch] = std::move(plan);
    return B2_OK;
}

int run_launch(const b2_engine* e, const Launch& L, void* const* bindings, cudaStream_t s) {
    const bool half = e->half();
    const void* in = L.in_binding >= 0 ? bindings[L.in_binding] : L.in;
    void* out = L.out_binding >= 0 ? bindings[L.out_binding] : L.out;
    switch (L.kind) {
        case L_INPUT_CAST:
            if (L.k == 2) return b2k::launch_input_cast_s2d(in, L.src_half, out, L.N, L.C, L.H, L.W, L.pad, L.stride, L.max_blocks, s);
            return b2k::launch_input_cast(in, L.src_half, out, L.N, L.C, L.H, L.W, L.C_phys, half, L.max_blocks, s);
        case L_OUTPUT_CAST:
            return b2k::launch_output_cast(in, static_cast<float*>(out), L.N, L.C, L.H, L.W, L.C_phys, half, s);
        case L_CONV_TC:
            return b2k::launch_conv_f16_tcgen05(L.conv, s);
        case L_CONV_SIMT:
            return b2k::launch_conv_simt(L.simt, half, s);
        case L_MAXPOOL:
            return b2k::launch_maxpool(in, out, L.N, L.H, L.W, L.C_phys, L.Ho, L.Wo, L.k, L.stride, L.pad, half, s);
        case L_AVGPOOL:
            return b2k::launch_avgpool(in, out, L.N, L.H * L.W, L.C_phys, half, s);
        case L_FC:
            return b2k::launch_fc(in, L.w, L.bias, static_cast<float*>(out), L.N, L.K, L.Cout, half, s);
        case L_SOFTMAX:
            return b2k::launch_softmax(static_cast<const float*>(in), static_cast<float*>(out), L.N, L.C, s);
        case L_QUANTIZE:
            return b2k::launch_quantize_h_to_i8(in, out, static_cast<long long>(L.N) * L.H * L.W, L.C, L.C_in_phys, L.C_phys, L.qscale, s);
        case L_CONV_I8:
            return b2k::launch_conv_i8_tcgen05(L.i8, s);
        case L_AVGPOOL_I8:
            return b2k::launch_avgpool_i8(in, out, L.N, L.H * L.W, L.C, L.C_in_phys, L.C_phys, L.qscale, s);
        case L_OUTPUT_CAST_I8:
            return b2k::launch_output_cast_i8(in, static_cast<float*>(out), L.N, L.C, L.H, L.W, L.C_phys, L.qscale, s);
        case L_QUANTIZE_F8:
            return b2k::launch_quantize_h_to_f8(in, out, static_cast<long long>(L.N) * L.H * L.W, L.C, L.C_in_phys, L.C_phys, L.qscale, s);
        case L_CONV_F8:
            return b2k::launch_conv_f8_tcgen05(L.i8, s);
        case L_AVGPOOL_F8:
            return b2k::launch_avgpool_f8(in, out, L.N, L.H * L.W, L.C, L.C_in_phys, L.C_phys, L.qscale, s);
        case L_OUTPUT_CAST_F8:
            return b2k::launch_output_cast_f8(in, static_cast<float*>(out), L.N, L.C, L.H, L.W, L.C_phys, L.qscale, s);
        case L_TAIL: {
            b2k::TailArgs t = L.tail;
            t.out = static_cast<float*>(out);
            return b2k::launch_tail_f16(t, s);
        }
        case L_EMBED_LN: {
            b2k::EmbedArgs a = L.embed;
            a.ids = static_cast<const int*>(in);
            a.segs = static_cast<const int*>(bindings[L.in_binding2]);
            a.mask = static_cast<const int*>(bindings[L.in_binding3]);
            return b2k::launch_embed_ln(a, s);
        }
        case L_LAYERNORM:
            return b2k::launch_layernorm(static_cast<const __half*>(in), static_cast<__half*>(out), L.bias, L.bias + L.C,
                                         static_cast<long long>(L.N) * L.H, L.C, L.C_phys, L.eps, L.live, s);
        case L_ATTENTION:
            return b2k::launch_attention(L.attn, s);
        case L_POOLER:
            return b2k::launch_pooler(static_cast<const __half*>(in), static_cast<const __half*>(L.w), L.bias, static_cast<float*>(out), L.N,
                                      L.W, L.C, L.C_phys, L.pos_map, s);
        case L_OUTPUT_ROWS:
            return b2k::launch_output_cast_rows(static_cast<const __half*>(in), static_cast<float*>(out), static_cast<long long>(L.N) * L.H * L.W,
                                                L.C, L.C_phys, s);
        case L_OUTPUT_UNPACK:
// ... 275 lines not shown
        if (rt && rt->alloc) {
            e->alloc = rt->alloc, e->free_ = rt->free_, e->alloc_user = rt->user;
            e->d_payload = static_cast<uint8_t*>(rt->alloc(rt->user, bytes, 256, 0));
            if (!e->d_payload) return fail(B2_ENOMEM, "user allocator returned null for %zu weight bytes", bytes);
        } else {
            void* p = nullptr;
            if (cudaMalloc(&p, bytes) != cudaSuccess) {
                cudaGetLastError();
                return fail(B2_ENOMEM, "cudaMalloc(%zu) for weights failed", bytes);
            }
            e->d_payload = static_cast<uint8_t*>(p);
        }
        if (e->payload_bytes) B2_CUDA(cudaMemcpy(e->d_payload, payload, e->payload_bytes, cudaMemcpyHostToDevice));
    }
    *out = e.release();
    return B2_OK;
}

int b2_engine_deserialize(b2_runtime* rt, const void* blob, size_t nbytes, b2_engine** out) {
    return deserialize_impl(rt, blob, nbytes, false, out);
}

int b2_engine_inspect(const void* blob, size_t nbytes, b2_engine** out) {
    return deserialize_impl(nullptr, blob, nbytes, true, out);
}

void b2_engine_destroy(b2_engine* e) {
    if (!e) return;
    if (e->d_payload) {
        if (e->free_)
            e->free_(e->alloc_user, e->d_payload);
        else
            cudaFree(e->d_payload);
    }
    delete e;
}

int b2_engine_nb_bindings(const b2_engine* e) { return e ? int(e->bindings.size()) : 0; }
const char* b2_engine_binding_name(const b2_engine* e, int i) {
    return (e && i >= 0 && i < int(e->bindings.size())) ? e->bindings[i].name.c_str() : nullptr;
}
int b2_engine_binding_index(const b2_engine* e, const char* name) {
    if (!e || !name) return -1;
    for (size_t i = 0; i < e->bindings.size(); ++i)
        if (e->bindings[i].name == name) return int(i);
    return -1;
}
int b2_engine_binding_is_input(const b2_engine* e, int i) {
    return (e && i >= 0 && i < int(e->bindings.size())) ? int(e->bindings[i].is_input) : 0;
}
int b2_engine_binding_dtype(const b2_engine* e, int i) {
    return (e && i >= 0 && i < int(e->bindings.size())) ? e->bindings[i].dtype : -1;
}
int b2_engine_binding_dims(const b2_engine* e, int i, int32_t* dims, int* nd) {
    if (!e || i < 0 || i >= int(e->bindings.size()) || !dims || !nd) return fail(B2_EINVAL, "bad binding query");
    *nd = e->bindings[i].nd;
    for (int d = 0; d < 8; ++d) dims[d] = e->bindings[i].dims[d];
    return B2_OK;
}
int b2_engine_max_batch(const b2_engine* e) { return e ? e->max_batch : 0; }
int b2_engine_precision(const b2_engine* e) { return e ? e->precision : -1; }
const char* b2_engine_name(const b2_engine* e) { return e ? e->name.c_str() : nullptr; }
size_t b2_engine_device_memory_size(const b2_engine* e) { return e ? e->arena_bytes : 0; }
size_t b2_engine_weights_size(const b2_engine* e) { return e ? e->payload_bytes : 0; }
double b2_engine_flops(const b2_engine* e, int batch) { return e ? e->flops_per_item * batch : 0.0; }
int b2_engine_nb_layers(const b2_engine* e) { return e ? int(e->ops.size()) : 0; }

int b2_context_create(b2_engine* e, b2_context** out) {
    if (!e || !out) return fail(B2_EINVAL, "null engine or out");
    if (e->inspect_only) return fail(B2_ESTATE, "engine was loaded with b2_engine_inspect (no device resources)");
    b2_context* c = new b2_context();
    c->e = e;
    c->use_graph = env_int("B2_GRAPH", 1);
    c->force_simt = env_int("B2_FORCE_SIMT", 0);
    c->force_im2col = env_int("B2_FORCE_IM2COL", 0);
    c->force_bn = env_int("B2_FORCE_BN", 0);
    c->force_stages = env_int("B2_FORCE_STAGES", 0);
    c->force_splits = env_int("B2_FORCE_SPLITS", 0);
    c->force_sps = env_int("B2_FORCE_SPS", 0);
    c->force_ws = env_int("B2_FORCE_WS", 0);
    c->force_cn = env_int("B2_FORCE_CN", 0);
    c->force_halo = env_int("B2_FORCE_HALO", 0);
    c->force_fuse = env_int("B2_FORCE_FUSE", 0);
    c->pdl_trigger = env_int("B2_PDL_TRIGGER", 1);
    c->autotune = env_int("B2_AUTOTUNE", 4);
    c->fork = env_int("B2_FORK", 0);
    c->fuse_tail = env_int("B2_FUSE_TAIL", 1);
    c->input_ctas = env_int("B2_INPUT_CTAS", 0);
    c->i8_bn = env_int("B2_I8_BN", 0);
    c->i8_stages = env_int("B2_I8_STAGES", 0);
    if (getenv("B2_PDL")) b2k::set_pdl(env_int("B2_PDL", 1) != 0);
    void* p = nullptr;
    if (cudaMalloc(&p, (kMaxSplitTiles + 16) * sizeof(int)) != cudaSuccess || cudaMemset(p, 0, (kMaxSplitTiles + 16) * sizeof(int)) != cudaSuccess) {
        cudaGetLastError();
        delete c;
        return fail(B2_ENOMEM, "cudaMalloc for split-K counters failed");
    }
    c->d_counters = static_cast<int*>(p);
    c->d_tail_ctrl = c->d_counters + kMaxSplitTiles;
    *out = c;
    return B2_OK;
}

static void drop_cached(b2_context* c) {
    c->states.clear();
    c->cur = c->scratch ? &c->states[c->scratch] : nullptr;
}

void b2_context_destroy(b2_context* c) {
    if (!c) return;
    drop_cached(c);
    if (c->d_counters) cudaFree(c->d_counters);
    if (c->side) cudaStreamDestroy(c->side);
    if (c->fork_ev) cudaEventDestroy(c->fork_ev);
    if (c->join_ev) cudaEventDestroy(c->join_ev);
    delete c;
}

int b2_context_set_device_memory(b2_context* c, void* scratch) {
    if (!c || !scratch) return fail(B2_EINVAL, "null context or scratch");
    if (reinterpret_cast<uintptr_t>(scratch) % 256 != 0) return fail(B2_EINVAL, "scratch must be 256-byte aligned (cudaMalloc alignment)");
    if (c->states.size() >= 32 && c->states.find(static_cast<uint8_t*>(scratch)) == c->states.end()) drop_cached(c);
    c->scratch = static_cast<uint8_t*>(scratch);
    c->cur = &c->states[c->scratch];
    return B2_OK;
}

int b2_context_set_option(b2_context* c, const char* key, int value) {
    if (!c || !key) return fail(B2_EINVAL, "null context or key");
    const std::string k(key);
    if (k == "graph") {
        c->use_graph = value;
        return B2_OK;
    }
    if (k == "pdl") {
        b2k::set_pdl(value != 0);
        value = 0;
    } else if (k == "simt") c->force_simt = value;
    else if (k == "im2col") c->force_im2col = value;
    else if (k == "bn") c->force_bn = value;
    else if (k == "stages") c->force_stages = value;
    else if (k == "splits") c->force_splits = value;
    else if (k == "sps") c->force_sps = value;
    else if (k == "ws") c->force_ws = value;
    else if (k == "cn") c->force_cn = value;
    else if (k == "halo") c->force_halo = value;
    else if (k == "fuse") c->force_fuse = value;
    else if (k == "fork") c->fork = value;
    else if (k == "fuse_tail") c->fuse_tail = value;
    else if (k == "i8_bn") c->i8_bn = value;
    else if (k == "i8_stages") c->i8_stages = value;
    else if (k == "input_ctas") c->input_ctas = value;
    else if (k == "pdl_trigger") c->pdl_trigger = value;
    else if (k == "autotune") c->autotune = value;
    else if (k == "no_fold") c->no_fold = value;
    else return fail(B2_EINVAL, "unknown option '%s'", key);
    drop_cached(c);
    return B2_OK;
}

int b2_context_nb_launches(b2_context* c, int batch) {
    if (!c) return -1;
    Plan* plan = nullptr;
    if (build_plan(c, batch, &plan)) return -1;
    return int(plan->launches.size());
}

int b2_engine_tune(b2_engine* e, int streams, int all_batches) {
    if (!e) return fail(B2_EINVAL, "null engine");
    if (e->inspect_only) return fail(B2_ESTATE, "engine was loaded with b2_engine_inspect (no device resources)");
    if (!e->half() || e->tactics_from_plan) return B2_OK;
    std::lock_guard<std::mutex> run_lock(e->tune_run_mutex);
    b2_context* c = nullptr;
    int rc = b2_context_create(e, &c);
    if (rc) return rc;
    c->autotune = streams > 0 ? streams : c->autotune;
    void* scratch = nullptr;
    if (c->autotune <= 0) {
        b2_context_destroy(c);
        return B2_OK;
    }
    if (cudaMalloc(&scratch, std::max<size_t>(e->arena_bytes, 1024)) != cudaSuccess) {
        cudaGetLastError();
        b2_context_destroy(c);
        return fail(B2_ENOMEM, "cudaMalloc(%zu) for the tuning arena failed", e->arena_bytes);
    }
    rc = b2_context_set_device_memory(c, scratch);
    if (!rc && load_driver_entry_points() != 0) rc = fail(B2_ECUDA, "cuTensorMapEncode* driver entry points unavailable");
    {
        std::lock_guard<std::mutex> lock(e->tune_mutex);
        tune_cache_load(e);
    }
    if (!rc) rc = tune_engine_batch(c, e->max_batch);
    for (int b = 1; !rc && all_batches && b < e->max_batch; ++b) rc = tune_engine_batch(c, b);
    cudaDeviceSynchronize();
    b2_context_destroy(c);
    cudaFree(scratch);
    if (!rc) e->tuned_at_load = true;
    return rc;
}

namespace {
struct RefineCtx {
    b2_context* c = nullptr;
    void* scratch = nullptr;
    std::vector<void*> bind;
    cudaStream_t s = nullptr;
};
}

int b2_engine_refine_tactics(b2_engine* e, int streams, int passes, double* gain_out) {
    if (gain_out) *gain_out = 1.0;
    if (!e) return fail(B2_EINVAL, "null engine");
    if (e->inspect_only) return fail(B2_ESTATE, "engine was loaded with b2_engine_inspect (no device resources)");
    if (!e->half() || e->tactics_from_plan) return B2_OK;
    streams = std::max(1, std::min(streams > 0 ? streams : 4, 8));
    int rc = b2_engine_tune(e, streams, 0);
    if (rc) return rc;
    std::lock_guard<std::mutex> run_lock(e->tune_run_mutex);
    const int batch = e->max_batch;
    std::vector<RefineCtx> ctx(static_cast<size_t>(streams));
    cudaEvent_t e0 = nullptr, e1 = nullptr;
    auto cleanup = [&] {
        cudaDeviceSynchronize();
        for (auto& x : ctx) {
            if (x.c) b2_context_destroy(x.c);
            if (x.scratch) cudaFree(x.scratch);
            for (void* p : x.bind)
                if (p) cudaFree(p);
            if (x.s) cudaStreamDestroy(x.s);
// ... 44 lines not shown
            if (cudaStreamSynchronize(ctx[0].s) != cudaSuccess) {
                status = fail(B2_ECUDA, "refine: forward pass failed: %s", cudaGetErrorString(cudaGetLastError()));
                break;
            }
            float ms = 0.f;
            cudaEventElapsedTime(&ms, e0, e1);
            if (rep > 0) best = std::min(best, double(ms) / (double(n) * double(ctx.size())));
        }
        return best;
    };
    double base = measure();
    const double first = base;
    const double keep = 1.0 - std::max(0.0, double(env_int("B2_REFINE_MIN_GAIN_PERMILLE", 7))) / 1000.0;
    for (int pass = 0; pass < std::max(1, passes) && !status; ++pass) {
        int changed = 0;
        for (size_t i = 0; i < e->ops.size() && !status; ++i) {
            const Op& op = e->ops[i];
            const b2plan::OpRec& r = op.r;
            if (r.type != b2plan::OP_CONV || (r.relu & 4)) continue;
            ConvConfig cur;
            {
                std::lock_guard<std::mutex> lock(e->tune_mutex);
                auto it = e->tuned.find({int(i), batch});
                if (it == e->tuned.end()) continue;
                cur = it->second;
            }
            const int kbsz = conv_kb(ctx[0].c, op);
            if (kbsz != 64 || cur.ws || cur.cn > 1) continue;
            const int nkb = conv_num_kblocks(ctx[0].c, op);
            std::vector<ConvConfig> cands;
            if (env_int("B2_TUNE_SPLITK", 0) != 0 && !(op.side_join >= 0) && op.groups == 1 && cur.splits == 1 && !cur.halo) {
                const int m_tiles = (batch * int(e->tensors[r.out].h * e->tensors[r.out].w) + 127) / 128;
                for (int sp : {2, 4}) {
                    const int tiles = m_tiles * (int(r.cout_phys) / cur.bn);
                    if (nkb < 16 || tiles >= 100 || tiles * sp > 160 || tiles > kMaxSplitTiles / 8) continue;
                    for (int st : {2, 4})
                        if (tactic_applies(ctx[0].c, op, batch, ConvConfig{cur.bn, st, sp, 0.0, 1, 0, 1}))
                            cands.push_back(ConvConfig{cur.bn, st, sp, 0.0, 1, 0, 1});
                }
            }
            if (cur.splits > 1) continue;
            for (const ConvConfig& t : conv_candidates(ctx[0].c, op, batch, 1))
                if (!t.ws && t.cn <= 1 && t.splits == 1 &&
                    !(t.bn == cur.bn && t.stages == cur.stages && t.sps == cur.sps && t.halo == cur.halo))
                    cands.push_back(t);
            if (streams >= kFuseMinStreams && cur.halo != 2 && tactic_applies(ctx[0].c, op, batch, fused_conv_config(op)))
                cands.push_back(fused_conv_config(op));
            ConvConfig best = cur;
            for (const ConvConfig& cand : cands) {
                {
                    std::lock_guard<std::mutex> lock(e->tune_mutex);
                    e->tuned[{int(i), batch}] = cand;
                }
                const double t = measure();
                if (status) break;
                if (t < base * keep) base = t, best = cand, ++changed;
            }
            std::lock_guard<std::mutex> lock(e->tune_mutex);
            e->tuned[{int(i), batch}] = best;
        }
        if (!changed) break;
    }
    if (!status) {
        const double last = measure();
        if (gain_out && last > 0 && last < 1e29) *gain_out = first / last;
    }
    cleanup();
    return status;
}

int b2_engine_nb_tactics(const b2_engine* e) {
    if (!e) return 0;
    std::lock_guard<std::mutex> lock(const_cast<b2_engine*>(e)->tune_mutex);
    return int(e->tuned.size());
}
int b2_engine_get_tactics(const b2_engine* e, uint32_t* out, int cap) {
    if (!e || !out) return 0;
    std::lock_guard<std::mutex> lock(const_cast<b2_engine*>(e)->tune_mutex);
    int n = 0;
    for (const auto& kv : e->tuned) {
        if (n >= cap) break;
        const ConvConfig& g = kv.second;
        const uint32_t rec[10] = {uint32_t(kv.first.first), uint32_t(kv.first.second), uint32_t(g.bn), uint32_t(g.stages), uint32_t(g.splits),
                                  uint32_t(g.sps), uint32_t(g.ws), uint32_t(g.cn), uint32_t(g.halo), 0u};
        memcpy(out + size_t(n) * 10, rec, sizeof rec);
        ++n;
    }
    return n;
}

int b2_context_prepare(b2_context* c, int batch, b2_stream_t stream_) {
    if (!c) return fail(B2_EINVAL, "null context");
    if (batch < 1 || batch > c->e->max_batch) return fail(B2_EINVAL, "batch %d outside [1, %d]", batch, c->e->max_batch);
    Plan* plan = nullptr;
    int rc = build_plan(c, batch, &plan);
    if (rc) return rc;
    if (!c->use_graph) return B2_OK;
    cudaStream_t stream = static_cast<cudaStream_t>(stream_);
    cudaStream_t own = nullptr;
    if (!stream) {
        B2_CUDA(cudaStreamCreateWithFlags(&own, cudaStreamNonBlocking));
        stream = own;
    }
    std::vector<void*> dummy(c->e->bindings.size(), reinterpret_cast<void*>(uintptr_t(256)));
    if (c->use_graph != 3 && !plan->exec && !plan->graph_failed) {
        rc = instantiate_plan_graph(c, plan, dummy.data(), stream);
        plan->graph_failed = !rc && plan->exec == nullptr;
    }
    if (!rc && !plan->exec)
        for (Segment& sg : plan->segments)
            if (sg.graphable && !sg.exec && (rc = instantiate_segment(c, plan, &sg, dummy.data(), stream))) break;
    if (own) cudaStreamDestroy(own);
    return rc;
}

int b2_context_enqueue(b2_context* c, int batch, void* const* bindings, b2_stream_t stream_, b2_event_t consumed) {
    int rc = check_args(c, batch, bindings);
    if (rc) return rc;
    cudaStream_t stream = static_cast<cudaStream_t>(stream_);
    Plan* plan = nullptr;
    if ((rc = build_plan(c, batch, &plan))) return rc;
    cudaStreamCaptureStatus cap = cudaStreamCaptureStatusNone;
    B2_CUDA(cudaStreamIsCapturing(stream, &cap));
    if (cap != cudaStreamCaptureStatusNone || !c->use_graph) {
        if ((rc = run_all(c, *plan, bindings, stream))) return rc;
    } else {
        if (c->use_graph != 3 && !plan->exec && !plan->graph_failed) {
            if ((rc = instantiate_plan_graph(c, plan, bindings, stream))) return rc;
            plan->graph_failed = plan->exec == nullptr;
        }
        if (plan->exec) {
            if ((rc = patch_plan_graph(plan, bindings))) return rc;
            B2_CUDA(cudaGraphLaunch(plan->exec, stream));
        } else {
            for (Segment& sg : plan->segments) {
                if (!sg.graphable) {
                    if ((rc = run_range(c, *plan, size_t(sg.begin), size_t(sg.end), bindings, stream))) return rc;
                    continue;
                }
                if (!sg.exec && (rc = instantiate_segment(c, plan, &sg, bindings, stream))) return rc;
                B2_CUDA(cudaGraphLaunch(sg.exec, stream));
            }
        }
    }
    if (consumed) B2_CUDA(cudaEventRecord(static_cast<cudaEvent_t>(consumed), stream));
    return B2_OK;
}

int b2_context_profile(b2_context* c, int batch, void* const* bindings, b2_stream_t stream_, float* ms, int cap) {
    if (check_args(c, batch, bindings)) return -1;
    cudaStream_t stream = static_cast<cudaStream_t>(stream_);
    Plan* plan = nullptr;
    if (build_plan(c, batch, &plan)) return -1;
    const int n = int(plan->launches.size());
    std::vector<cudaEvent_t> ev(n + 1);
    for (auto& e : ev) cudaEventCreate(&e);
    int rc = 0;
    cudaEventRecord(ev[0], stream);
    for (int i = 0; i < n && !rc; ++i) {
        rc = run_launch(c->e, plan->launches[i], bindings, stream);
        cudaEventRecord(ev[i + 1], stream);
    }
    cudaError_t se = cudaStreamSynchronize(stream);
    if (rc || se != cudaSuccess) {
        fail(B2_ECUDA, "profile run failed: %s", cudaGetErrorString(rc ? cudaError_t(rc) : se));
        n > 0 ? (void)0 : (void)0;
    } else {
        for (int i = 0; i < n && i < cap; ++i) cudaEventElapsedTime(&ms[i], ev[i], ev[i + 1]);
    }
    for (auto& e : ev) cudaEventDestroy(e);
    return (rc || se != cudaSuccess) ? -1 : n;
}

static const Launch* get_launch(b2_context* c, int batch, int i) {
    if (!c) return nullptr;
    Plan* plan = nullptr;
    if (build_plan(c, batch, &plan)) return nullptr;
    if (i < 0 || i >= int(plan->launches.size())) return nullptr;
    return &plan->launches[i];
}
int b2_context_debug_conv_timing(b2_context* c, int batch, int i, int reps, b2_stream_t stream_, long long* stamps,
                                 int cap_ctas, int* n_ctas) {
    const int dbg_mode = env_int("B2_DBG_MODE", 0);
    Plan* plan = nullptr;
    if (!c || build_plan(c, batch, &plan)) return fail(B2_EINVAL, "no plan");
    if (i < 0 || i >= int(plan->launches.size()) || plan->launches[i].kind != L_CONV_TC) return fail(B2_EINVAL, "not a tcgen05 conv launch");
    b2k::ConvLaunch cl = plan->launches[i].conv;
    const int ctas = cl.ws_ctas > 0 ? cl.ws_ctas : cl.grid_m * cl.grid_n * cl.args.splits;
    if (n_ctas) *n_ctas = ctas;
    if (ctas > cap_ctas) return fail(B2_EINVAL, "stamp buffer too small (%d CTAs)", ctas);
    long long* d = nullptr;
    B2_CUDA(cudaMalloc(&d, size_t(ctas) * 16 * sizeof(long long)));
    cudaMemset(d, 0, size_t(ctas) * 16 * sizeof(long long));
    cl.args.dbg = d;
    cl.args.dbg_mode = dbg_mode;
    cudaStream_t s = static_cast<cudaStream_t>(stream_);
    int rc = 0;
    for (int r = 0; r < reps && !rc; ++r) rc = b2k::launch_conv_f16_tcgen05(cl, s);
    cudaError_t se = cudaStreamSynchronize(s);
    if (!rc && se == cudaSuccess) cudaMemcpy(stamps, d, size_t(ctas) * 16 * sizeof(long long), cudaMemcpyDeviceToHost);
    cudaFree(d);
    if (rc || se != cudaSuccess) return fail(B2_ECUDA, "debug launch failed: %s", cudaGetErrorString(rc ? cudaError_t(rc) : se));
    return B2_OK;
}

int b2_debug_conv_residency(int bn, int kb, int stages, int sps, int residual, int halo_w, int halo_rows, int cblocks,
                            int* ctas_per_sm) {
    if (!ctas_per_sm) return fail(B2_EINVAL, "null output");
    const int rc = b2k::init_conv_kernels();
    if (rc) return fail(B2_ECUDA, "kernel attribute setup failed: %s", cudaGetErrorString(cudaError_t(rc)));
    *ctas_per_sm = b2k::conv_residency(bn, kb, stages, sps, residual != 0, halo_w, halo_rows, cblocks);
    if (*ctas_per_sm <= 0)
        return fail(B2_EINVAL, "no residency for bn=%d kb=%d st=%dx%d res=%d halo_w=%d", bn, kb, stages, sps, residual, halo_w);
    return B2_OK;
}

const char* b2_context_launch_name(b2_context* c, int batch, int i) {
    static thread_local std::string s;
    const Launch* L = get_launch(c, batch, i);
    if (!L) return nullptr;
    static const char* kinds[] = {"input_cast", "conv_tcgen05", "conv_simt", "maxpool", "avgpool", "fc", "softmax", "output_cast", "tail_pool_fc_softmax",
                                  "quantize", "conv_i8_tcgen05", "avgpool_i8", "output_cast_i8", "embed_ln", "layernorm", "attention_f16_wgmma",
                                  "pooler", "output_cast_rows", "output_unpack_rows", "quantize_f8", "conv_f8_tcgen05", "avgpool_f8",
                                  "output_cast_f8", "patchify", "tokens", "cls_head"};
    static_assert(sizeof(kinds) / sizeof(kinds[0]) == L_CLS_HEAD + 1, "kinds[] is indexed by LKind");
    s = std::string(kinds[L->kind]) + (L->kind == L_ATTENTION && L->attn.S > 128 ? "_ks" : "") +
        (L->kind == L_ATTENTION && L->attn.seq_off ? "_varlen" : "") + ":" + L->name;
    if (L->kind == L_ATTENTION && L->attn.S != L->W) s += " sk=" + std::to_string(L->attn.S);
    if (L->kind == L_CONV_TC)
        s += " bn=" + std::to_string(L->conv.bn) + " kb=" + std::to_string(L->conv.kb) +
             " st=" + std::to_string(L->conv.stages) + "x" + std::to_string(L->conv.sps) +
             (L->conv.ws_ctas ? " ws=" + std::to_string(L->conv.ws_ctas) : std::string()) +
             (L->conv.cn > 1 ? " cn=" + std::to_string(L->conv.cn) : std::string()) +
             (L->conv.halo == 2 ? " halo fused" : L->conv.halo ? " halo" : "") +
             (L->conv.args.a_mode == b2k::A_TILED ? " tiled" : " im2col") +
             " grid=" + std::to_string(L->conv.grid_n) + "x" + std::to_string(L->conv.grid_m) + "x" +
             std::to_string(L->conv.args.splits) + " kblk=" + std::to_string(L->conv.args.num_kblocks) +
             (L->conv.args.group_span ? " span=" + std::to_string(L->conv.args.group_span) : std::string()) +
             ((L->conv.args.relu & b2plan::kConvGelu) ? " gelu" : "") + (L->conv.args.live ? " live" : "");
    if (L->kind == L_CONV_I8 || L->kind == L_CONV_F8)
        s += " bn=" + std::to_string(L->i8.bn) + " st=" + std::to_string(L->i8.stages) + (L->i8.args.a_mode == b2k::A_TILED ? " tiled" : " im2col") + " grid=" +
             std::to_string(L->i8.grid_n) + "x" + std::to_string(L->i8.grid_m) + " kblk=" + std::to_string(L->i8.args.num_kblocks) +
             (L->i8.group_mode ? " span=" + std::to_string(L->i8.args.group_span) + " mode=" +
                                     (L->i8.group_mode == 128 ? std::string("dense") : std::to_string(L->i8.group_mode))
                               : std::string());
    if (L->side_join >= 0) s += " side";
    return s.c_str();
}
double b2_context_launch_flops(b2_context* c, int batch, int i) {
    const Launch* L = get_launch(c, batch, i);
    return L ? L->flops : 0.0;
}
double b2_context_launch_bytes(b2_context* c, int batch, int i) {
    const Launch* L = get_launch(c, batch, i);
    return L ? L->bytes : 0.0;
}

}
```

tensorrt_laboratory_b200/csrc/kernels.cu:

```cuda
#include "kernels.h"

#include <stdio.h>
#include <stdlib.h>
#include <string.h>

#include <array>
#include <map>
#include <mutex>

#include "ptx_sm90.cuh"
#include "wgmma_sm90.cuh"

namespace b2k {

template <int BN, int STAGES, int SPS = 1>
struct ConvCfg {
    static constexpr int A_SUBBLK = 128 * 64 * 2;
    static constexpr int B_SUBBLK = BN * 64 * 2;
    static constexpr int A_STAGE = SPS * A_SUBBLK;
    static constexpr int B_STAGE = SPS * B_SUBBLK;
    static constexpr int PIPE_BYTES = STAGES * (A_STAGE + B_STAGE);
    static constexpr int TILE_BYTES = 128 * BN * 2;
    static_assert(TILE_BYTES <= PIPE_BYTES, "the output staging tile reuses the pipeline buffers");
};

__host__ __device__ constexpr int conv_smem_layout_bytes(int bn, int stages, bool residual, int sps = 1) {
    return stages * sps * (128 * 64 * 2 + bn * 64 * 2) + (residual ? 128 * bn * 2 : 0) + 256 + bn * 4 + 1024;
}

constexpr int kConvThreads = 320;
constexpr int kConsumerWarps = 8;
constexpr int kActWarp = 8;
constexpr int kWgtWarp = 9;
__host__ __device__ constexpr int conv_min_ctas(int bn) { return bn <= 64 ? 3 : bn <= 128 ? 2 : 1; }
constexpr int kConvWsThreads = 384;

struct FragPos {
    int row0, col0;
    __device__ FragPos(int consumer_warp, int lane)
        : row0(64 * (consumer_warp >> 2) + 16 * (consumer_warp & 3) + (lane >> 2)), col0(2 * (lane & 3)) {}
};

template <int BN, int KB, int STAGES, int SPS, int CN = 1, bool DBG = false, int AV = 0, bool GELU = false, bool LIVE = false>
__global__ void __launch_bounds__(kConvThreads, conv_min_ctas(BN))
conv_f16_tcgen05(const __grid_constant__ CUtensorMap mapA, const __grid_constant__ CUtensorMap mapB,
                 const __grid_constant__ CUtensorMap mapOut, const __grid_constant__ CUtensorMap mapRes,
                 const ConvArgs p) {
    static_assert(SPS == 1 || KB == 64, "multi-sub-block stages exist for the 64-wide K path only");
    static_assert(!LIVE || AV == 2, "live-row instantiations exist for the tiled packed-weight path only");
    using Cfg = ConvCfg<BN, STAGES, SPS>;
    constexpr int TPS = 64 / KB;
    constexpr int A_SUB = 128 * KB * 2;
    constexpr int B_SUB = BN * KB * 2;
    constexpr int OW = BN >= 64 ? 64 : 32;
    constexpr int OROWB = OW * 2;
    constexpr int NBOX = BN / OW;

    extern __shared__ uint8_t smem_raw[];
    uint8_t* smem = smem_raw + ((1024u - (smem_u32(smem_raw) & 1023u)) & 1023u);
    const bool has_res = p.residual != nullptr;
    uint8_t* sA = smem;
    uint8_t* sB = smem + STAGES * Cfg::A_STAGE;
    uint8_t* sOut = smem;
    uint8_t* sRes = smem + Cfg::PIPE_BYTES;
    uint8_t* tail = sRes + (has_res ? Cfg::TILE_BYTES : 0);
    uint64_t* full_bar = reinterpret_cast<uint64_t*>(tail);
    uint64_t* empty_bar = full_bar + STAGES;
    uint64_t* accum_bar = empty_bar + STAGES;
    uint64_t* res_bar = accum_bar + 1;
    uint32_t* last_flag = reinterpret_cast<uint32_t*>(res_bar + 1);
    float* s_bias = reinterpret_cast<float*>(tail + 256);

    const int warp = threadIdx.x >> 5;
    const int lane = threadIdx.x & 31;
    const int n0 = blockIdx.x * BN;
    const int m0 = blockIdx.y * 128;
    long long* dbg = (DBG && p.dbg) ? p.dbg + 16ll * ((blockIdx.z * gridDim.y + blockIdx.y) * gridDim.x + blockIdx.x) : nullptr;
    if (dbg && threadIdx.x == 0) {
        dbg[0] = clock64();
        unsigned long long gt;
        asm volatile("mov.u64 %0, %%globaltimer;" : "=l"(gt));
        dbg[8] = static_cast<long long>(gt);
        unsigned smid;
        asm volatile("mov.u32 %0, %%smid;" : "=r"(smid));
        dbg[10] = smid;
    }
    const int kb_begin = blockIdx.z * p.kb_per_split;
    const int kb_end = min(p.num_kblocks, kb_begin + p.kb_per_split);
    const int nk = (kb_end - kb_begin + SPS - 1) / SPS;
    auto subs_in_step = [&](int i) -> int {
        const int rem = (kb_end - kb_begin) - i * SPS;
        return rem < SPS ? rem : SPS;
    };
    const bool split = p.splits > 1;
    bool dead = false;
    static_assert(AV == 0 || (KB == 64 && CN == 1 && !DBG), "resolved operand paths exist for the plain 64-wide K kernels");
    const bool a_tiled = AV == 2 ? true : (AV == 1 ? false : p.a_mode == A_TILED);
    const bool w_packed = AV != 0 ? true : p.wpacked != nullptr;
    static_assert(CN == 1 || KB == 64, "clusters exist for the 64-wide K path only");
    constexpr int cn = CN;
    const uint32_t crank = cn > 1 ? cluster_ctarank() : 0u;
    constexpr uint16_t cmask = static_cast<uint16_t>((1u << cn) - 1u);

    if (threadIdx.x == 0) {
        tma_prefetch_desc(&mapA);
        tma_prefetch_desc(&mapB);
        tma_prefetch_desc(&mapOut);
        if (has_res) tma_prefetch_desc(&mapRes);
        for (int s = 0; s < STAGES; ++s) {
            mbar_init(&full_bar[s], 1);
            mbar_init(&empty_bar[s], static_cast<uint32_t>(kConsumerWarps * cn));
        }
        mbar_init(res_bar, 1);
        fence_barrier_init();
        fence_proxy_async();
    }
    __syncthreads();
    if (cn > 1) cluster_sync_all();
    if (warp == kWgtWarp) {
#pragma unroll
        for (int i = 0; i < BN / 32; ++i) s_bias[lane + 32 * i] = __ldg(p.bias + n0 + lane + 32 * i);
    }
    if (p.pdl_trigger == 0) pdl_launch_dependents();
    if (dbg && threadIdx.x == 0) dbg[1] = clock64();

    auto sub_tiles = [&](int kb) -> int {
        if (KB == 64) return 1;
        const int n = p.taps_phys - kb * TPS;
        return n > TPS ? TPS : n;
    };
    const bool skip_a = DBG && KB == 64 && (p.dbg_mode & 2), skip_b = DBG && KB == 64 && (p.dbg_mode & 4);
    auto stage_bytes = [&](int kb) -> uint32_t {
        if (KB == 64) {
            const int ns = subs_in_step((kb - kb_begin) / SPS);
            return static_cast<uint32_t>(ns * ((skip_a ? 0 : Cfg::A_SUBBLK) + (skip_b ? 0 : Cfg::B_SUBBLK)));
        }
        return static_cast<uint32_t>(sub_tiles(kb) * (A_SUB + B_SUB));
    };
    auto load_b = [&](int kb, int s) {
        if (skip_b) return;
        uint8_t* b_dst = sB + s * Cfg::B_STAGE;
        if (KB == 64) {
            const int ns = subs_in_step((kb - kb_begin) / SPS);
            for (int u = 0; u < ns; ++u) {
                if (w_packed) {
                    bulk_load_1d(&full_bar[s], b_dst + u * Cfg::B_SUBBLK,
                                 p.wpacked + (static_cast<size_t>(kb + u) * (p.Cout >> 5) + (n0 >> 5)) * 4096, BN * 128);
                } else {
                    tma_load_2d(&mapB, &full_bar[s], b_dst + u * Cfg::B_SUBBLK, (kb + u) * 64, n0);
                }
            }
        } else {
            const int nt = sub_tiles(kb);
            for (int t = 0; t < nt; ++t) tma_load_2d(&mapB, &full_bar[s], b_dst + t * B_SUB, (kb * TPS + t) * KB, n0);
        }
    };
    auto load_residual = [&]() {
        mbar_expect_tx(res_bar, Cfg::TILE_BYTES);
#pragma unroll
        for (int b = 0; b < NBOX; ++b) tma_load_2d(&mapRes, res_bar, sRes + b * (128 * OROWB), n0 + b * OW, m0);
    };

    if (warp == kActWarp) {
        {
            int img0 = 0, p0 = 0, q0 = 0;
            const int slice_rows = 128 / cn;
            int ms = m0 + static_cast<int>(crank) * slice_rows;
            const uint32_t slice_off = crank * static_cast<uint32_t>(slice_rows) * 128u;
            if (!a_tiled) {
                if (ms >= p.M) ms = 0;
                img0 = ms / p.HoWo;
                const int rem = ms - img0 * p.HoWo;
                p0 = rem / p.Wo;
                q0 = rem - p0 * p.Wo;
            }
            const int base_w = q0 * p.stride_w - p.pad_w;
            const int base_h = p0 * p.stride_h - p.pad_h;
            int cur_cb = 0, cur_r = 0, cur_sx = 0;
            int cb0 = 0;
            if (KB == 64) {
                const int tap0 = kb_begin / p.cblocks;
                cur_cb = kb_begin - tap0 * p.cblocks;
                cur_r = tap0 / p.kw;
                cur_sx = tap0 - cur_r * p.kw;
                if (p.group_span) cb0 = (n0 / p.group_span) * (p.group_span >> 6);
            }
            auto load_a = [&](int kb, int s) {
                if (skip_a) return;
                uint8_t* a_dst = sA + s * Cfg::A_STAGE;
                if (KB == 64) {
                    const int ns = subs_in_step((kb - kb_begin) / SPS);
                    for (int u = 0; u < ns; ++u) {
                        const int c0 = (cb0 + cur_cb) * 64;
                        if (cn > 1) {
                            if (a_tiled) {
                                tma_load_2d_mc(&mapA, &full_bar[s], a_dst + u * Cfg::A_SUBBLK + slice_off, c0, ms, cmask);
                            } else {
                                tma_load_im2col_4d_mc(&mapA, &full_bar[s], a_dst + u * Cfg::A_SUBBLK + slice_off, c0, base_w,
                                                      base_h, img0, static_cast<uint16_t>(cur_sx), static_cast<uint16_t>(cur_r), cmask);
                            }
                        } else if (a_tiled) {
                            tma_load_2d(&mapA, &full_bar[s], a_dst + u * Cfg::A_SUBBLK, c0, m0);
                        } else {
                            tma_load_im2col_4d(&mapA, &full_bar[s], a_dst + u * Cfg::A_SUBBLK, c0, base_w, base_h, img0,
                                               static_cast<uint16_t>(cur_sx), static_cast<uint16_t>(cur_r));
                        }
                        if (++cur_cb == p.cblocks) {
                            cur_cb = 0;
                            if (++cur_sx == p.kw) {
                                cur_sx = 0;
                                ++cur_r;
                            }
                        }
                    }
                } else {
                    const int nt = sub_tiles(kb);
                    for (int t = 0; t < nt; ++t) {
                        const int tap = kb * TPS + t;
                        const int tap_a = tap < p.taps ? tap : p.taps - 1;
                        const int r = tap_a / p.kw;
                        const int sx = tap_a - r * p.kw;
                        tma_load_im2col_4d(&mapA, &full_bar[s], a_dst + t * A_SUB, 0, base_w, base_h, img0,
                                           static_cast<uint16_t>(sx), static_cast<uint16_t>(r));
                    }
                }
            };
            constexpr bool kSplitProducers = KB == 64;
            const int npre = nk < STAGES ? nk : STAGES;
            if (!LIVE && elect_one_sync()) {
                for (int i = 0; i < npre; ++i) {
                    mbar_expect_tx(&full_bar[i], stage_bytes(kb_begin + i * SPS));
                    if (!kSplitProducers) load_b(kb_begin + i * SPS, i);
                }
            }
            __syncwarp();
            pdl_wait();
            if constexpr (LIVE) {
                dead = m0 >= *p.live_rows;
                if (elect_one_sync())
                    for (int i = 0; i < npre; ++i)
                        mbar_expect_tx(&full_bar[i], dead ? static_cast<uint32_t>(subs_in_step(i) * Cfg::B_SUBBLK) : stage_bytes(kb_begin + i * SPS));
                __syncwarp();
                if (dead)
                    for (int i = 0; i < npre; ++i) mbar_wait(&full_bar[i], 0);
            }
            if (dbg && lane == 0) dbg[2] = clock64();
            if (!dead && elect_one_sync()) {
                for (int i = 0; i < npre; ++i) load_a(kb_begin + i * SPS, i);
                if (has_res && !split) load_residual();
            }
            __syncwarp();
            long long tw = 0, te = 0, tl = 0;
            for (int i = npre; i < (dead ? 0 : nk); ++i) {
                const int s = i % STAGES;
                const uint32_t ph = (i / STAGES) & 1;
                long long c0 = 0, c1 = 0, c3 = 0;
                if (dbg) c0 = clock64();
                mbar_wait(&empty_bar[s], ph ^ 1);
                if (dbg) c1 = clock64();
                if (elect_one_sync()) {
                    mbar_expect_tx(&full_bar[s], stage_bytes(kb_begin + i * SPS));
                    load_a(kb_begin + i * SPS, s);
                    if (!kSplitProducers) load_b(kb_begin + i * SPS, s);
                }
                __syncwarp();
                if (dbg) {
                    c3 = clock64();
                    tw += c1 - c0, tl += c3 - c1;
                }
            }
            if (dbg && lane == 0) dbg[11] = tw, dbg[12] = te, dbg[13] = tl;
        }
        __syncwarp();
    }

    const int cw = warp;
    const bool consumer = warp < kConsumerWarps;
    float acc[BN / 2];
    if (consumer) {
        if constexpr (LIVE) {
            pdl_wait();
            dead = m0 >= *p.live_rows;
        }
        const int nk_mma = dead ? 0 : nk;
        const uint32_t wg = static_cast<uint32_t>(cw >> 2);
        auto release_stage = [&](int st) {
            __syncwarp();
            if (lane == 0) {
                if (cn > 1) {
                    for (uint32_t r = 0; r < static_cast<uint32_t>(cn); ++r) mbar_arrive_cluster(&empty_bar[st], r);
                } else {
                    mbar_arrive(&empty_bar[st]);
                }
            }
        };
        long long mw = 0, mi = 0;
        for (int i = 0; i < nk_mma; ++i) {
            const int s = i % STAGES;
            const uint32_t ph = (i / STAGES) & 1;
            long long m0c = 0, m1c = 0;
            if (dbg) m0c = clock64();
            mbar_wait(&full_bar[s], ph);
            if (dbg) m1c = clock64(), mw += m1c - m0c;
            if (dbg && i == 0 && cw == 0 && lane == 0) dbg[3] = clock64();
            const uint32_t a_addr = smem_u32(sA + s * Cfg::A_STAGE);
            const uint32_t b_addr = smem_u32(sB + s * Cfg::B_STAGE);
            if constexpr (KB == 64) {
                auto mma = [&](int t) {
                    const int u = t >> 2, j = t & 3;
                    const uint64_t ad = make_wgmma_desc(a_addr + u * Cfg::A_SUBBLK + wg * 8192 + j * 32, 16, 1024, WG_SW128);
                    const uint64_t bd = make_wgmma_desc(b_addr + u * Cfg::B_SUBBLK + j * 32, 16, 1024, WG_SW128);
                    wgmma_f16<BN>(acc, ad, bd, (i > 0 || t > 0) ? 1u : 0u);
                };
                if (SPS == 1 || subs_in_step(i) == SPS) wgmma_group<4 * SPS>(mma);
                else wgmma_group<4>(mma);
            } else if constexpr (KB == 32) {
                auto mma = [&](int t) {
                    const int st = t >> 1, j = t & 1;
                    const uint64_t ad = make_wgmma_desc(a_addr + st * A_SUB + wg * 4096 + j * 32, 16, 512, WG_SW64);
                    const uint64_t bd = make_wgmma_desc(b_addr + st * B_SUB + j * 32, 16, 512, WG_SW64);
                    wgmma_f16<BN>(acc, ad, bd, (i > 0 || t > 0) ? 1u : 0u);
                };
                if (sub_tiles(kb_begin + i) == TPS) wgmma_group<2 * TPS>(mma);
                else wgmma_group<2>(mma);
            } else {
                auto mma = [&](int j) {
                    const uint64_t ad = make_wgmma_desc(a_addr + 2 * j * A_SUB + wg * 1024, A_SUB, 128, WG_NOSWZ);
                    const uint64_t bd = make_wgmma_desc(b_addr + 2 * j * B_SUB, B_SUB, 128, WG_NOSWZ);
                    wgmma_f16<BN>(acc, ad, bd, (i > 0 || j > 0) ? 1u : 0u);
                };
                wgmma_group_upto<TPS / 2>(sub_tiles(kb_begin + i) / 2, mma);
            }
            if constexpr (STAGES == 1) {
                wgmma_wait<0>();
                release_stage(0);
            } else {
                wgmma_wait<1>();
                if (i > 0) release_stage((i - 1) % STAGES);
            }
            if (dbg) mi += clock64() - m1c;
        }
        if constexpr (STAGES > 1) {
            wgmma_wait<0>();
            if (nk_mma > 0) release_stage((nk_mma - 1) % STAGES);
        }
        if (dbg && cw == 0 && lane == 0) dbg[4] = clock64(), dbg[14] = mw, dbg[15] = mi;
    }

    if (warp == kWgtWarp && KB == 64) {
        for (int i = 0; i < nk; ++i) {
            const int s = i % STAGES;
            if constexpr (LIVE) {
                if (i == STAGES) {
                    pdl_wait();
                    if (m0 >= *p.live_rows) break;
                }
            }
            if (i >= STAGES) mbar_wait(&empty_bar[s], ((i / STAGES) & 1) ^ 1);
            if (elect_one_sync()) load_b(kb_begin + i * SPS, s);
            __syncwarp();
        }
    }

    pdl_wait();
    __syncthreads();
    if constexpr (LIVE) {
        if (m0 >= *p.live_rows) return;
    }
    if (dbg && threadIdx.x == 0) dbg[5] = clock64();
    if (p.pdl_trigger == 1) pdl_launch_dependents();
    const FragPos fp(cw, lane);

    auto finish_pair = [&](int row, int col, float v0, float v1) {
        const int box = col / OW;
        const int chunk = (col % OW) / 8;
        const uint32_t so = static_cast<uint32_t>(box * (128 * OROWB)) + swz_off<OROWB>(row, chunk) + (col % 8) * 2;
        v0 += s_bias[col];
        v1 += s_bias[col + 1];
        if (has_res) {
            const float2 rf = __half22float2(*reinterpret_cast<const __half2*>(sRes + so));
            v0 += rf.x;
            v1 += rf.y;
        }
        if constexpr (GELU) {
            v0 = gelu_erf(v0);
            v1 = gelu_erf(v1);
        } else if (p.relu) {
            v0 = fmaxf(v0, 0.0f);
            v1 = fmaxf(v1, 0.0f);
        }
        *reinterpret_cast<__half2*>(sOut + so) = __floats2half2_rn(v0, v1);
    };

    bool do_store = true;
    if (!split) {
        if (consumer) {
            if (has_res) mbar_wait(res_bar, 0);
#pragma unroll
            for (int j = 0; j < BN / 8; ++j)
#pragma unroll
                for (int h = 0; h < 2; ++h) finish_pair(fp.row0 + 8 * h, 8 * j + fp.col0, acc[4 * j + 2 * h], acc[4 * j + 2 * h + 1]);
        }
    } else {
        const int tile = blockIdx.y * gridDim.x + blockIdx.x;
        float* ws_tile = p.workspace + static_cast<size_t>(tile) * p.splits * (128 * BN);
        if (consumer) {
            float* mine = ws_tile + static_cast<size_t>(blockIdx.z) * (128 * BN);
#pragma unroll
            for (int j = 0; j < BN / 8; ++j)
#pragma unroll
                for (int h = 0; h < 2; ++h)
                    __stcg(reinterpret_cast<float2*>(mine + (fp.row0 + 8 * h) * BN + 8 * j + fp.col0),
                           make_float2(acc[4 * j + 2 * h], acc[4 * j + 2 * h + 1]));
        }
        __syncthreads();
        if (threadIdx.x == kActWarp * 32) {
            __threadfence();
            const int prev = atomicAdd(p.tile_counters + tile, 1);
            const uint32_t last = (prev == p.splits - 1) ? 1u : 0u;
            if (last) {
                p.tile_counters[tile] = 0;
                if (has_res) load_residual();
            }
            *last_flag = last;
        }
        __syncthreads();
        do_store = *last_flag != 0;
        if (do_store && consumer) {
            __threadfence();
            if (has_res) mbar_wait(res_bar, 0);
#pragma unroll 4
            for (int j = 0; j < BN / 8; ++j) {
#pragma unroll
                for (int h = 0; h < 2; ++h) {
                    const int row = fp.row0 + 8 * h, col = 8 * j + fp.col0;
                    float f0 = 0.f, f1 = 0.f;
                    for (int sp = 0; sp < p.splits; ++sp) {
                        const float2 t = __ldcg(reinterpret_cast<const float2*>(ws_tile + static_cast<size_t>(sp) * (128 * BN) + row * BN + col));
                        f0 += t.x;
                        f1 += t.y;
                    }
                    finish_pair(row, col, f0, f1);
                }
            }
        }
    }
    if (dbg && threadIdx.x == 0) dbg[6] = clock64();
    if (p.pdl_trigger == 2) pdl_launch_dependents();
    fence_proxy_async();
    __syncthreads();
    if (threadIdx.x == kActWarp * 32 && do_store) {
#pragma unroll
        for (int b = 0; b < NBOX; ++b) tma_store_2d(&mapOut, sOut + b * (128 * OROWB), n0 + b * OW, m0);
        tma_store_commit_and_wait_read();
    }
    if (cn > 1) {
        if (warp == kWgtWarp) {
            const int first = nk > STAGES ? nk - STAGES : 0;
            for (int i = first; i < nk; ++i) mbar_wait(&empty_bar[i % STAGES], (i / STAGES) & 1);
        }
        __syncthreads();
        cluster_sync_all();
    }
    if (dbg && threadIdx.x == 0) {
        dbg[7] = clock64();
        unsigned long long gt;
        asm volatile("mov.u64 %0, %%globaltimer;" : "=l"(gt));
        dbg[9] = static_cast<long long>(gt);
    }
}

__host__ __device__ constexpr int conv_ws_smem_bytes(int bn, int stages, int sps, bool residual) {
    return stages * sps * (128 * 64 * 2 + bn * 64 * 2) + 2 * 128 * bn * 2 + (residual ? 2 * 128 * bn * 2 : 0) + 256 + 1024;
}

template <int BN, int STAGES, int SPS>
__global__ void __launch_bounds__(kConvWsThreads, 1)
conv_f16_tcgen05_ws(const __grid_constant__ CUtensorMap mapA, const __grid_constant__ CUtensorMap mapOut,
                    const __grid_constant__ CUtensorMap mapRes, const ConvArgs p) {
    constexpr int A_SUBBLK = 128 * 64 * 2;
    constexpr int B_SUBBLK = BN * 64 * 2;
    constexpr int A_STAGE = SPS * A_SUBBLK;
    constexpr int B_STAGE = SPS * B_SUBBLK;
    constexpr int PIPE_BYTES = STAGES * (A_STAGE + B_STAGE);
    constexpr int TILE_BYTES = 128 * BN * 2;
    constexpr int OW = BN >= 64 ? 64 : 32;
    constexpr int OROWB = OW * 2;
    constexpr int NBOX = BN / OW;

    extern __shared__ uint8_t smem_raw[];
    uint8_t* smem = smem_raw + ((1024u - (smem_u32(smem_raw) & 1023u)) & 1023u);
    const bool has_res = p.residual != nullptr;
    uint8_t* sA = smem;
    uint8_t* sB = smem + STAGES * A_STAGE;
    uint8_t* sOut = smem + PIPE_BYTES;
    uint8_t* sRes = sOut + 2 * TILE_BYTES;
    uint8_t* tail = sRes + (has_res ? 2 * TILE_BYTES : 0);
    uint64_t* full_bar = reinterpret_cast<uint64_t*>(tail);
    uint64_t* empty_bar = full_bar + STAGES;
    uint64_t* res_full = empty_bar + STAGES;
    uint64_t* res_empty = res_full + 2;

    const int warp = threadIdx.x >> 5;
    const int lane = threadIdx.x & 31;
    const int num_tiles = p.tiles_m * p.tiles_n;
    const int nsteps = (p.num_kblocks + SPS - 1) / SPS;
    auto subs_in_step = [&](int i) -> int {
        const int rem = p.num_kblocks - i * SPS;
        return rem < SPS ? rem : SPS;
    };

    if (threadIdx.x == 0) {
        if (p.dbg) p.dbg[static_cast<size_t>(blockIdx.x) * 16] = clock64();
        tma_prefetch_desc(&mapA);
        tma_prefetch_desc(&mapOut);
        if (has_res) tma_prefetch_desc(&mapRes);
        for (int s = 0; s < STAGES; ++s) {
            mbar_init(&full_bar[s], 1);
            mbar_init(&empty_bar[s], kConsumerWarps);
        }
        for (int b = 0; b < 2; ++b) {
            mbar_init(&res_full[b], 1);
            mbar_init(&res_empty[b], 1);
        }
        fence_barrier_init();
        fence_proxy_async();
    }
    __syncthreads();
    if (p.pdl_trigger == 0) pdl_launch_dependents();
    long long* const dbg = p.dbg ? p.dbg + static_cast<size_t>(blockIdx.x) * 16 : nullptr;
    if (dbg && threadIdx.x == 0) dbg[1] = clock64();

    if (warp == 0) {
        pdl_wait();
        long long w_stage = 0;
        int g = 0;
        for (int tile = blockIdx.x; tile < num_tiles; tile += gridDim.x) {
            const int mt = tile / p.tiles_n;
            const int m0 = mt * 128;
            int img0 = 0, p0 = 0, q0 = 0;
            if (p.a_mode == A_IM2COL) {
                img0 = m0 / p.HoWo;
                const int rem = m0 - img0 * p.HoWo;
                p0 = rem / p.Wo;
                q0 = rem - p0 * p.Wo;
            }
            const int base_w = q0 * p.stride_w - p.pad_w;
            const int base_h = p0 * p.stride_h - p.pad_h;
            int cur_cb = 0, cur_r = 0, cur_sx = 0;
            for (int i = 0; i < nsteps; ++i, ++g) {
                const int s = g % STAGES;
                const long long t1 = dbg ? clock64() : 0;
// ... 677 lines not shown
    return static_cast<int>(cudaLaunchKernelEx(&cfg, kern, args...));
}
template <typename Kern, typename... Args>
static int launch_kernel(Kern kern, dim3 grid, dim3 block, size_t smem, cudaStream_t stream, bool pdl, Args... args) {
    return launch_kernel_cluster(kern, grid, block, smem, stream, pdl, 1u, args...);
}

template <int BN, int KB, int STAGES, int SPS, int CN = 1>
static int launch_one(const ConvLaunch& L, cudaStream_t stream) {
    dim3 grid(L.grid_n, L.grid_m, L.args.splits);
    const size_t smem = size_t(conv_smem_layout_bytes(BN, STAGES, L.args.residual != nullptr, SPS));
    if (CN > 1 && (KB != 64 || L.grid_n % CN != 0 || L.args.cn != CN)) return static_cast<int>(cudaErrorInvalidValue);
    if (L.args.live) {
        if constexpr (CN == 1 && KB == 64) {
            if (L.args.wpacked != nullptr && L.args.a_mode == A_TILED && L.args.splits == 1 && L.args.dbg == nullptr && L.args.dbg_mode == 0) {
                if (L.args.relu & 8)
                    return launch_kernel_cluster(conv_f16_tcgen05<BN, KB, STAGES, SPS, 1, false, 2, true, true>, grid, dim3(kConvThreads), smem,
                                                 stream, true, 1u, L.mapA, L.mapB, L.mapOut, L.mapRes, L.args);
                return launch_kernel_cluster(conv_f16_tcgen05<BN, KB, STAGES, SPS, 1, false, 2, false, true>, grid, dim3(kConvThreads), smem,
                                             stream, true, 1u, L.mapA, L.mapB, L.mapOut, L.mapRes, L.args);
            }
        }
        return static_cast<int>(cudaErrorInvalidValue);
    }
    if (L.args.relu & 8) {
        if constexpr (CN == 1 && KB == 64) {
            if (L.args.wpacked != nullptr && L.args.a_mode == A_TILED && L.args.dbg == nullptr && L.args.dbg_mode == 0)
                return launch_kernel_cluster(conv_f16_tcgen05<BN, KB, STAGES, SPS, 1, false, 2, true>, grid, dim3(kConvThreads), smem, stream,
                                             true, 1u, L.mapA, L.mapB, L.mapOut, L.mapRes, L.args);
        }
        return static_cast<int>(cudaErrorInvalidValue);
    }
    if (CN == 1 && (L.args.dbg != nullptr || L.args.dbg_mode != 0))
        return launch_kernel_cluster(conv_f16_tcgen05<BN, KB, STAGES, SPS, 1, true>, grid, dim3(kConvThreads), smem, stream, true, 1u, L.mapA,
                                     L.mapB, L.mapOut, L.mapRes, L.args);
    if constexpr (CN == 1 && KB == 64) {
        if (L.args.wpacked != nullptr) {
            if (L.args.a_mode == A_TILED)
                return launch_kernel_cluster(conv_f16_tcgen05<BN, KB, STAGES, SPS, 1, false, 2>, grid, dim3(kConvThreads), smem, stream, true, 1u,
                                             L.mapA, L.mapB, L.mapOut, L.mapRes, L.args);
            return launch_kernel_cluster(conv_f16_tcgen05<BN, KB, STAGES, SPS, 1, false, 1>, grid, dim3(kConvThreads), smem, stream, true, 1u,
                                         L.mapA, L.mapB, L.mapOut, L.mapRes, L.args);
        }
    }
    return launch_kernel_cluster(conv_f16_tcgen05<BN, KB, STAGES, SPS, CN>, grid, dim3(kConvThreads), smem, stream, true,
                                 static_cast<unsigned>(CN), L.mapA, L.mapB, L.mapOut, L.mapRes, L.args);
}

template <typename Kern>
static int set_conv_smem(Kern kern, int bytes) {
    int e = static_cast<int>(cudaFuncSetAttribute(kern, cudaFuncAttributeMaxDynamicSharedMemorySize, bytes));
    if (!e) e = static_cast<int>(cudaFuncSetAttribute(kern, cudaFuncAttributePreferredSharedMemoryCarveout, cudaSharedmemCarveoutMaxShared));
    return e;
}

template <int BN, int KB, int STAGES, int SPS, int CN = 1>
static int init_one() {
    const int want = conv_smem_layout_bytes(BN, STAGES, true, SPS);
    const int bytes = want > 227 * 1024 ? conv_smem_layout_bytes(BN, STAGES, false, SPS) : want;
    if (CN == 1) {
        int e = set_conv_smem(conv_f16_tcgen05<BN, KB, STAGES, SPS, 1, true>, bytes);
        if (e) return e;
        if constexpr (KB == 64) {
            if ((e = set_conv_smem(conv_f16_tcgen05<BN, KB, STAGES, SPS, 1, false, 1>, bytes))) return e;
            if ((e = set_conv_smem(conv_f16_tcgen05<BN, KB, STAGES, SPS, 1, false, 2>, bytes))) return e;
            if ((e = set_conv_smem(conv_f16_tcgen05<BN, KB, STAGES, SPS, 1, false, 2, true>, bytes))) return e;
            if ((e = set_conv_smem(conv_f16_tcgen05<BN, KB, STAGES, SPS, 1, false, 2, false, true>, bytes))) return e;
            if ((e = set_conv_smem(conv_f16_tcgen05<BN, KB, STAGES, SPS, 1, false, 2, true, true>, bytes))) return e;
        }
    }
    return set_conv_smem(conv_f16_tcgen05<BN, KB, STAGES, SPS, CN>, bytes);
}

int conv_smem_bytes(int bn, int stages, bool residual, int sps) { return conv_smem_layout_bytes(bn, stages, residual, sps); }

#define B2_FOR_EACH_CONV(X) \
    X(32, 64, 1, 1) X(32, 64, 2, 1) X(32, 64, 4, 1) X(32, 64, 8, 1) \
    X(64, 64, 1, 1) X(64, 64, 2, 1) X(64, 64, 4, 1) X(64, 64, 8, 1) \
    X(128, 64, 1, 1) X(128, 64, 2, 1) X(128, 64, 4, 1) X(256, 64, 2, 1) X(256, 64, 4, 1) \
    X(32, 64, 2, 2) X(32, 64, 4, 2) X(64, 64, 2, 2) X(64, 64, 4, 2) X(128, 64, 2, 2) X(256, 64, 2, 2) \
    X(32, 8, 2, 1) X(32, 8, 4, 1) X(64, 8, 2, 1) X(64, 8, 4, 1) X(64, 8, 8, 1) X(128, 8, 4, 1) \
    X(32, 32, 2, 1) X(32, 32, 4, 1) X(64, 32, 1, 1) X(64, 32, 2, 1) X(64, 32, 4, 1) X(128, 32, 2, 1) X(128, 32, 4, 1)

int conv_halo_smem(int bn, int w, int r, int cblocks) { return halo_smem_bytes(bn, w, r, cblocks); }
bool conv_halo_config_exists(int bn) { return bn == 64 || bn == 128 || bn == 256; }
static int init_conv_halo_kernels() {
    int e;
    if ((e = set_conv_smem(conv3x3_halo_tcgen05<64>, 227 * 1024))) return e;
    if ((e = set_conv_smem(conv3x3_halo_tcgen05<128>, 227 * 1024))) return e;
    if ((e = set_conv_smem(conv3x3_halo_tcgen05<256>, 227 * 1024))) return e;
    if ((e = set_conv_smem(conv3x3_halo_1x1_tcgen05<64>, 227 * 1024))) return e;
    if ((e = set_conv_smem(conv3x3_halo_1x1_tcgen05<128>, 227 * 1024))) return e;
    return set_conv_smem(conv3x3_halo_1x1_tcgen05<256>, 227 * 1024);
}
int conv_halo_fused_smem(int bn, int w, int r, int cblocks, int cout2) { return halo_fused_smem_bytes(bn, w, r, cblocks, cout2); }
static int launch_conv_halo_fused(const ConvLaunch& L, cudaStream_t stream) {
    const int R = L.args.halo_rows;
    const size_t smem = size_t(halo_fused_smem_bytes(L.bn, L.args.Wo, R, L.args.cblocks, L.c2.Cout));
    if (smem > 227 * 1024 || R < 1 || R * (L.args.Wo + 2) > 128 || L.args.cblocks > kHaloMaxCBlocks || L.grid_n != 1 ||
        L.bn != L.args.Cout || L.c2.Cout < kFuseChunk || L.c2.Cout % kFuseChunk)
        return static_cast<int>(cudaErrorInvalidValue);
    dim3 grid(1, L.grid_m, 1);
    switch (L.bn) {
        case 64: return launch_kernel(conv3x3_halo_1x1_tcgen05<64>, grid, dim3(kConvThreads), smem, stream, true, L.mapA, L.mapRes, L.mapOut, L.args, L.c2);
        case 128: return launch_kernel(conv3x3_halo_1x1_tcgen05<128>, grid, dim3(kConvThreads), smem, stream, true, L.mapA, L.mapRes, L.mapOut, L.args, L.c2);
        case 256: return launch_kernel(conv3x3_halo_1x1_tcgen05<256>, grid, dim3(kConvThreads), smem, stream, true, L.mapA, L.mapRes, L.mapOut, L.args, L.c2);
    }
    return static_cast<int>(cudaErrorInvalidValue);
}
static int launch_conv_halo(const ConvLaunch& L, cudaStream_t stream) {
    if (L.halo == 2) return launch_conv_halo_fused(L, stream);
    const int R = L.args.halo_rows;
    const size_t smem = size_t(halo_smem_bytes(L.bn, L.args.Wo, R, L.args.cblocks));
    if (smem > 227 * 1024 || R < 1 || R * (L.args.Wo + 2) > 128 || L.args.cblocks > kHaloMaxCBlocks) return static_cast<int>(cudaErrorInvalidValue);
    dim3 grid(L.grid_n, L.grid_m, 1);
    switch (L.bn) {
        case 64: return launch_kernel(conv3x3_halo_tcgen05<64>, grid, dim3(kConvThreads), smem, stream, true, L.mapA, L.mapOut, L.args);
        case 128: return launch_kernel(conv3x3_halo_tcgen05<128>, grid, dim3(kConvThreads), smem, stream, true, L.mapA, L.mapOut, L.args);
        case 256: return launch_kernel(conv3x3_halo_tcgen05<256>, grid, dim3(kConvThreads), smem, stream, true, L.mapA, L.mapOut, L.args);
    }
    return static_cast<int>(cudaErrorInvalidValue);
}

#define B2_FOR_EACH_CONV_CLUSTER(X) \
    X(32, 4, 1, 2) X(32, 4, 1, 4) X(64, 1, 1, 2) X(64, 2, 1, 2) X(64, 2, 1, 4) X(64, 2, 2, 2) X(64, 4, 2, 2) X(64, 4, 2, 4) \
    X(128, 2, 1, 2) X(128, 2, 1, 4) X(128, 2, 2, 2)

int init_conv_ws_kernels();
int launch_conv_f16_tcgen05_ws(const ConvLaunch& L, cudaStream_t stream);

int conv_stem_ws_smem() { return conv_stem_ws_smem_bytes(); }
static int launch_conv_stem_ws(const ConvLaunch& L, cudaStream_t stream) {
    const ConvArgs& a = L.args;
    if (L.bn != 64 || a.Cout != 64 || a.Wo > 128 || a.taps != kStemRows || a.stride_h != kStemStride || a.residual != nullptr)
        return static_cast<int>(cudaErrorInvalidValue);
    return launch_kernel(conv_stem_ws_tcgen05, dim3(L.ws_ctas), dim3(kConvWsThreads), size_t(conv_stem_ws_smem_bytes()), stream, true,
                         L.mapA, L.mapB, L.mapOut, L.args);
}

int init_conv_kernels() {
    int e = init_conv_ws_kernels();
    if (e) return e;
    if ((e = static_cast<int>(cudaFuncSetAttribute(conv_stem_ws_tcgen05, cudaFuncAttributeMaxDynamicSharedMemorySize,
                                                   conv_stem_ws_smem_bytes()))))
        return e;
    if ((e = init_conv_halo_kernels())) return e;
#define B2_INIT(BN_, KB_, ST_, SPS_) \
    if ((e = init_one<BN_, KB_, ST_, SPS_>())) return e;
    B2_FOR_EACH_CONV(B2_INIT)
#undef B2_INIT
#define B2_INIT_CL(BN_, ST_, SPS_, CN_) \
    if ((e = init_one<BN_, 64, ST_, SPS_, CN_>())) return e;
    B2_FOR_EACH_CONV_CLUSTER(B2_INIT_CL)
#undef B2_INIT_CL
    return 0;
}

int launch_conv_f16_tcgen05(const ConvLaunch& L, cudaStream_t stream) {
    if (L.halo) return launch_conv_halo(L, stream);
    if (L.ws_ctas > 0) return L.kb == 32 ? launch_conv_stem_ws(L, stream) : launch_conv_f16_tcgen05_ws(L, stream);
    if (L.cn > 1) {
#define B2_CASE_CL(BN_, ST_, SPS_, CN_) \
    if (L.bn == BN_ && L.kb == 64 && L.stages == ST_ && L.sps == SPS_ && L.cn == CN_) return launch_one<BN_, 64, ST_, SPS_, CN_>(L, stream);
        B2_FOR_EACH_CONV_CLUSTER(B2_CASE_CL)
#undef B2_CASE_CL
        return static_cast<int>(cudaErrorInvalidValue);
    }
#define B2_CASE(BN_, KB_, ST_, SPS_) \
    if (L.bn == BN_ && L.kb == KB_ && L.stages == ST_ && L.sps == SPS_) return launch_one<BN_, KB_, ST_, SPS_>(L, stream);
    B2_FOR_EACH_CONV(B2_CASE)
#undef B2_CASE
    return static_cast<int>(cudaErrorInvalidValue);
}

#define B2_FOR_EACH_CONV_WS(X) \
    X(32, 4, 1) X(64, 2, 1) X(64, 4, 1) X(64, 2, 2) X(64, 4, 2) X(128, 2, 1) X(128, 4, 1) X(128, 2, 2)

template <int BN, int STAGES, int SPS>
static int launch_one_ws(const ConvLaunch& L, cudaStream_t stream) {
    const size_t smem = size_t(conv_ws_smem_bytes(BN, STAGES, SPS, L.args.residual != nullptr));
    return launch_kernel(conv_f16_tcgen05_ws<BN, STAGES, SPS>, dim3(L.ws_ctas), dim3(kConvWsThreads), smem, stream, true, L.mapA, L.mapOut,
                         L.mapRes, L.args);
}

int init_conv_ws_kernels() {
    int e = 0;
#define B2_INIT_WS(BN_, ST_, SPS_)                                                                                        \
    {                                                                                                                     \
        const int want = conv_ws_smem_bytes(BN_, ST_, SPS_, true);                                                        \
        e = static_cast<int>(cudaFuncSetAttribute(conv_f16_tcgen05_ws<BN_, ST_, SPS_>,                                    \
                                                  cudaFuncAttributeMaxDynamicSharedMemorySize,                            \
                                                  want > 227 * 1024 ? conv_ws_smem_bytes(BN_, ST_, SPS_, false) : want)); \
        if (e) return e;                                                                                                  \
    }
    B2_FOR_EACH_CONV_WS(B2_INIT_WS)
#undef B2_INIT_WS
    return 0;
}

int launch_conv_f16_tcgen05_ws(const ConvLaunch& L, cudaStream_t stream) {
#define B2_CASE_WS(BN_, ST_, SPS_) \
    if (L.bn == BN_ && L.stages == ST_ && L.sps == SPS_) return launch_one_ws<BN_, ST_, SPS_>(L, stream);
    B2_FOR_EACH_CONV_WS(B2_CASE_WS)
#undef B2_CASE_WS
    return static_cast<int>(cudaErrorInvalidValue);
}

bool conv_ws_config_exists(int bn, int stages, int sps) {
#define B2_HAS_WS(BN_, ST_, SPS_) \
    if (bn == BN_ && stages == ST_ && sps == SPS_) return true;
    B2_FOR_EACH_CONV_WS(B2_HAS_WS)
#undef B2_HAS_WS
    return false;
}

int conv_ws_smem(int bn, int stages, int sps, bool residual) { return conv_ws_smem_bytes(bn, stages, sps, residual); }

bool conv_cluster_config_exists(int bn, int stages, int sps, int cn) {
#define B2_HAS_CL(BN_, ST_, SPS_, CN_) \
    if (bn == BN_ && stages == ST_ && sps == SPS_ && cn == CN_) return true;
    B2_FOR_EACH_CONV_CLUSTER(B2_HAS_CL)
#undef B2_HAS_CL
    return false;
}

bool conv_config_exists(int bn, int kb, int stages, int sps) {
#define B2_HAS(BN_, KB_, ST_, SPS_) \
    if (bn == BN_ && kb == KB_ && stages == ST_ && sps == SPS_) return true;
    B2_FOR_EACH_CONV(B2_HAS)
#undef B2_HAS
    return false;
}

int conv_residency(int bn, int kb, int stages, int sps, bool residual, int halo_w, int halo_rows, int cblocks) {
    static std::mutex mu;
    static std::map<std::array<int, 8>, int> cache;
    const std::array<int, 8> key{bn, kb, stages, sps, residual ? 1 : 0, halo_w, halo_rows, cblocks};
    {
        std::lock_guard<std::mutex> lock(mu);
        const auto it = cache.find(key);
        if (it != cache.end()) return it->second;
    }
// ... 819 lines not shown
```

tensorrt_laboratory_b200/csrc/kernels.h:

```cpp
#pragma once
#include <cuda.h>
#include <cuda_fp16.h>
#include <cuda_runtime.h>
#include <stdint.h>

namespace b2k {

enum { A_TILED = 0, A_IM2COL = 1 };

struct ConvArgs {
    const float* bias;
    const __half* residual;
    __half* out;
    int M;
    int Cout;
    int num_kblocks;
    int cblocks;
    int taps;
    int taps_phys;
    int kw;
    int HoWo, Wo;
    int stride_h, stride_w;
    int pad_h, pad_w;
    int relu;
    int a_mode;
    int splits;
    int kb_per_split;
    float* workspace;
    union {
        int* tile_counters;
        const int* live_rows;
    };
    int pdl_trigger;
    const uint8_t* wpacked;
    int halo_rows;
    int cn;
    int tiles_m, tiles_n;
    int dbg_mode;
    long long* dbg;
    int group_span;
    int live;
};
static_assert(sizeof(ConvArgs) == 168, "ConvArgs layout");

struct Conv1x1Args {
    const uint8_t* wpacked;
    const float* bias;
    int Cout;
    int relu;
};

struct ConvLaunch {
    CUtensorMap mapA;
    CUtensorMap mapB;
    CUtensorMap mapOut;
    CUtensorMap mapRes;
    ConvArgs args;
    int bn;
    int kb;
    int stages;
    int sps;
    int grid_m, grid_n;
    int cn;
    int halo;
    int ws_ctas;
    Conv1x1Args c2;
};

int launch_conv_f16_tcgen05(const ConvLaunch& L, cudaStream_t stream);
int init_conv_kernels();
bool conv_config_exists(int bn, int kb, int stages, int sps = 1);
int conv_smem_bytes(int bn, int stages, bool residual, int sps = 1);
bool conv_cluster_config_exists(int bn, int stages, int sps, int cn);
bool conv_halo_config_exists(int bn);
int conv_halo_smem(int bn, int w, int r, int cblocks);
int conv_halo_fused_smem(int bn, int w, int r, int cblocks, int cout2);
int conv_residency(int bn, int kb, int stages, int sps, bool residual, int halo_w = 0, int halo_rows = 0, int cblocks = 0);
bool conv_ws_config_exists(int bn, int stages, int sps);
int conv_ws_smem(int bn, int stages, int sps, bool residual);
constexpr int kStemWsRing = 16;
int conv_stem_ws_smem();
void set_pdl(bool on);
bool get_pdl();

struct I8ConvArgs {
    const uint8_t* wpacked;
    const float* m;
    const float* b;
    float r;
    int has_res, relu;
    int M, Cout, num_kblocks, cblocks;
    int kw, HoWo, Wo, stride_h, stride_w, pad_h, pad_w, a_mode;
    int last_cb_mmas, cout_real;
    int group_span;
};
struct I8ConvLaunch {
    CUtensorMap mapA;
    CUtensorMap mapOut;
    CUtensorMap mapRes;
    I8ConvArgs args;
    int bn, stages, grid_m, grid_n;
    int group_mode;
};
int init_conv_i8_kernels();
bool conv_i8_config_exists(int bn, int stages);
int conv_i8_smem_bytes(int bn, int stages, bool residual);
int launch_conv_i8_tcgen05(const I8ConvLaunch& L, cudaStream_t stream);
int launch_conv_f8_tcgen05(const I8ConvLaunch& L, cudaStream_t stream);
int launch_quantize_h_to_f8(const void* src, void* dst, long long pixels, int C, int C_in_phys, int C_out_phys, float inv_s,
                            cudaStream_t stream);
int launch_avgpool_f8(const void* src, void* dst, int N, int HW, int C, int C_in_phys, int C_out_phys, float k, cudaStream_t stream);
int launch_output_cast_f8(const void* src, float* dst, int N, int C, int H, int W, int C_phys, float s, cudaStream_t stream);
int launch_quantize_h_to_i8(const void* src, void* dst, long long pixels, int C, int C_in_phys, int C_out_phys, float inv_s,
                            cudaStream_t stream);
int launch_avgpool_i8(const void* src, void* dst, int N, int HW, int C, int C_in_phys, int C_out_phys, float k, cudaStream_t stream);
int launch_output_cast_i8(const void* src, float* dst, int N, int C, int H, int W, int C_phys, float s, cudaStream_t stream);

struct SimtConvArgs {
    const void* in;
    const void* w;
    const float* bias;
    const void* residual;
    void* out;
    int N, H, W, Cin, Cin_phys, Ho, Wo, Cout, Cout_phys;
    int kh, kw, taps_phys, stride_h, stride_w, pad_h, pad_w, relu;
    int w_packed;
    int groups;
    int wk_tap;
};
int launch_conv_simt(const SimtConvArgs& a, bool half_storage, cudaStream_t stream);

int launch_input_cast(const void* src, bool src_half, void* dst, int N, int C, int H, int W, int C_phys,
                      bool half_storage, int max_blocks, cudaStream_t stream);
int launch_input_cast_s2d(const void* src, bool src_half, void* dst, int N, int C, int H, int W, int pad_l, int pad_r,
                          int max_blocks, cudaStream_t stream);
int launch_output_cast(const void* src, float* dst, int N, int C, int H, int W, int C_phys,
                       bool half_storage, cudaStream_t stream);
int launch_maxpool(const void* src, void* dst, int N, int H, int W, int C_phys, int Ho, int Wo, int k,
                   int stride, int pad, bool half_storage, cudaStream_t stream);
int launch_avgpool(const void* src, void* dst, int N, int HW, int C_phys, bool half_storage,
                   cudaStream_t stream);
int launch_fc(const void* in, const void* w, const float* bias, float* out, int N, int K, int Cout,
              bool half_storage, cudaStream_t stream);
int launch_softmax(const float* in, float* out, int N, int C, cudaStream_t stream);

struct TailArgs {
    const __half* in;
    const __half* w;
    const float* bias;
    float* out;
    __half* pooled;
    float* logits;
    int* ctrl;
    int N, HW, C, Cout;
};
bool tail_f16_applies(int N, int HW, int C, int Cout);
// ... 40 lines not shown
```

tensorrt_laboratory_b200/csrc/plan_format.h:

```cpp
#pragma once
#include <stdint.h>

namespace b2plan {

constexpr char kMagic[8] = {'B', '2', 'E', 'N', 'G', 'I', 'N', 'E'};
constexpr uint32_t kVersion = 1;
constexpr uint32_t kVersionGrouped = 2;
constexpr uint32_t kVersionTransformer = 3;

enum OpType : uint32_t {
    OP_INPUT_CAST = 0,
    OP_CONV = 1,
    OP_MAXPOOL = 2,
    OP_AVGPOOL = 3,
    OP_FC = 4,
    OP_SOFTMAX = 5,
    OP_OUTPUT_CAST = 6,
    OP_QUANTIZE = 7,
    OP_EMBED_LN = 8,
    OP_LAYERNORM = 9,
    OP_ATTENTION = 10,
    OP_POOLER = 11,
    OP_PATCHIFY = 12,
    OP_TOKENS = 13,
    OP_CLS_HEAD = 14,
};

enum TensorKind : uint32_t { T_ACT = 0 , T_VEC = 1  };

#pragma pack(push, 1)
struct Header {
    char magic[8];
    uint32_t version;
    uint32_t precision;
    uint32_t max_batch;
    uint32_t n_tensors;
    uint32_t n_ops;
    uint32_t n_bindings;
    uint64_t payload_offset;
    uint64_t payload_bytes;
    char name[64];
    uint32_t n_tactics;
    uint32_t reserved;
    uint64_t tactics_offset;
};
struct TacticRec {
    uint32_t op, batch, bn, stages, splits, sps, ws, cn, halo, reserved;
};
struct TensorRec {
    char name[64];
    uint32_t kind;
    uint32_t h, w, c, c_phys;
    int32_t binding;
    float scale;
    uint8_t pad[4];
};
struct OpRec {
    char name[64];
    uint32_t type;
    int32_t in, res, out;
    int32_t binding;
    uint32_t k, stride, pad_;
    uint32_t relu;
    uint32_t ceil_mode;
    uint32_t cin, cout, cin_phys, cout_phys, taps, taps_phys;
    uint64_t w_off, w_bytes, b_off, b_bytes;
    uint32_t kw, stride_w, pad_w_lo, pad_w_hi;
};
struct OpRecV2 {
    OpRec v1;
    uint32_t groups;
    uint8_t reserved[12];
};
struct OpRecV3 {
    OpRec v1;
    uint32_t groups;
    uint32_t heads;
    uint32_t vocab, positions, types;
    int32_t binding2, binding3;
    int32_t out2;
    float eps;
    uint32_t flags;
    uint8_t reserved[8];
};
enum : uint32_t { kConvRelu = 1, kConvPacked = 2, kConvInt8 = 4, kConvGelu = 8 };
enum : uint32_t { kOpRowsOut = 1, kOpPacked = 2 };
struct BindingRec {
    char name[64];
    uint32_t is_input;
    uint32_t dtype;
    int32_t tensor;
    uint32_t nd;
    int32_t dims[8];
    uint8_t pad[16];
};
#pragma pack(pop)

static_assert(sizeof(Header) == 128, "Header size");
static_assert(sizeof(TacticRec) == 40, "TacticRec size");
static_assert(sizeof(TensorRec) == 96, "TensorRec size");
static_assert(sizeof(OpRec) == 176, "OpRec size");
static_assert(sizeof(OpRecV2) == 192, "OpRecV2 size");
static_assert(sizeof(OpRecV3) == 224, "OpRecV3 size");
static_assert(sizeof(BindingRec) == 128, "BindingRec size");

}
```

Before: 32940.

## Fuse ResNet projection shortcut 1x1 conv into the residual-joining 1x1 conv kernel

Adds a conv_f16_proj_tcgen05 kernel that computes the downsample projection 1x1 conv in the same CTA as the bottleneck's final 1x1 conv. It runs extra k-blocks over the block input, adds bias and optional relu, and stages the result in shared memory as the residual. The projection's output tensor never goes to global memory and one launch is dropped. Autotuning only picks the fused variant when its timed cost beats the separate launches, including the interaction with the halo-fused 3x3. This adds kernel variants, tactic-cache and plan fields, and a new accumulator-reset path in the wgmma loop.

```diff
diff --git a/__graft_entry__.py b/__graft_entry__.py
--- a/__graft_entry__.py
+++ b/__graft_entry__.py
@@ -58,7 +58,7 @@
 _CONV_KERNEL = re.compile(r"conv|attention_f16_wgmma|embed_ln|layernorm_h8|pooler|patchify|tokens_kernel|cls_head")
 
 
-_SHARED_SM_KERNEL = re.compile(r"_ZN3b2k(?:16conv_f16_tcgen05|20conv3x3_halo_tcgen05|24conv3x3_halo_1x1_tcgen05)ILi(\d+)E")
+_SHARED_SM_KERNEL = re.compile(r"_ZN3b2k(?:16conv_f16_tcgen05|21conv_f16_proj_tcgen05|20conv3x3_halo_tcgen05|24conv3x3_halo_1x1_tcgen05)ILi(\d+)E")
 _SHARED_SM_THREADS = 320
 
 
diff --git a/tensorrt_laboratory_b200/csrc/engine.cu b/tensorrt_laboratory_b200/csrc/engine.cu
--- a/tensorrt_laboratory_b200/csrc/engine.cu
+++ b/tensorrt_laboratory_b200/csrc/engine.cu
@@ -151,6 +151,8 @@
     bool src_half = false;
     int max_blocks = 0;
     int side_join = -1;
+    int op = -1;
+    std::string proj_of;
     b2k::TailArgs tail{};
     b2k::I8ConvLaunch i8{};
     float qscale = 0.f;
@@ -205,6 +207,7 @@
     int ws = 0;
     int cn = 1;
     int halo = 0;
+    int proj = 0;
 };
 static bool stage_depth_useful(int bn, int kb, int st, int kpc) {
     const int stgs[4] = {1, 2, 4, 8};
@@ -274,6 +277,7 @@
     int force_sps = 0;
     int force_halo = 0;
     int force_fuse = 0;
+    int force_proj = 0;
     int force_cn = 0;
     int force_ws = 0;
     int pdl_trigger = 1;
@@ -735,6 +739,7 @@
             if (t.op >= h.n_ops || t.batch == 0 || t.batch > h.max_batch) return fail(B2_EINVAL, "plan: tactic %u out of range", i);
             ConvConfig cfg{int(t.bn), int(t.stages), int(t.splits), 0.0, int(t.sps), int(t.ws), int(t.cn)};
             cfg.halo = int(t.halo);
+            cfg.proj = int(t.proj);
             e->tuned[{int(t.op), int(t.batch)}] = cfg;
         }
         e->tactics_from_plan = true;
@@ -943,6 +948,31 @@
     return i + 1;
 }
 
+int proj_partner(const b2_engine* e, int j) {
+    if (!e->half() || e->one_byte() || j < 0 || size_t(j) >= e->ops.size()) return -1;
+    const Op& oj = e->ops[size_t(j)];
+    const b2plan::OpRec& rj = oj.r;
+    if (rj.type != b2plan::OP_CONV || rj.res < 0) return -1;
+    auto plain_1x1 = [&](const Op& o) {
+        const b2plan::OpRec& r = o.r;
+        return o.kh() == 1 && o.kw() == 1 && o.sh() == o.sw() && o.ph() == 0 && o.pw_lo() == 0 && o.pw_hi() == 0 && o.groups == 1 &&
+               (r.relu & 2) && !(r.relu & (4 | b2plan::kConvGelu)) && r.cin_phys % 64 == 0 && !(o.flags & b2plan::kOpPacked) &&
+               conv_on_tensor_cores(e, o);
+    };
+    if (!plain_1x1(oj) || oj.sh() != 1) return -1;
+    for (size_t k = 0; k < size_t(j); ++k) {
+        const Op& op = e->ops[k];
+        const b2plan::OpRec& rp = op.r;
+        if (rp.type != b2plan::OP_CONV || rp.out != rj.res) continue;
+        const Tensor &tp = e->tensors[rp.out], &tj = e->tensors[rj.out];
+        if (op.side_join != j || !plain_1x1(op) || tp.binding >= 0 || e->tensors[rp.in].binding >= 0 || tp.h != tj.h || tp.w != tj.w ||
+            rp.cout_phys != rj.cout_phys)
+            return -1;
+        return int(k);
+    }
+    return -1;
+}
+
 bool conv_on_tensor_cores(const b2_engine* e, const Op& op) {
     const b2plan::OpRec& r = op.r;
     const bool kb64 = r.cin_phys % 64 == 0, kb8 = r.cin_phys == 8;
@@ -967,6 +997,10 @@
     if (op.groups > 1 && (!span || span % cfg.bn || cfg.splits > 1)) return false;
     if ((op.groups > 1 || (r.relu & b2plan::kConvGelu)) && (cfg.ws || cfg.cn > 1 || cfg.halo)) return false;
     if ((op.flags & b2plan::kOpPacked) && (cfg.ws || cfg.cn > 1 || cfg.halo || cfg.splits > 1)) return false;
+    if (cfg.proj)
+        return proj_partner(c->e, int(&op - &c->e->ops[0])) >= 0 && c->force_proj >= 0 && !c->force_im2col && !cfg.halo && !cfg.ws && cfg.cn <= 1 &&
+               cfg.splits == 1 && cfg.sps == 1 && b2k::conv_proj_config_exists(cfg.bn, cfg.stages) &&
+               b2k::conv_proj_smem(cfg.bn, cfg.stages) <= kSmemLimit;
     if (cfg.halo == 2) {
         const int j = fuse_partner(c->e, int(&op - &c->e->ops[0]));
         const int R = conv_halo_rows(c, op), cblocks = int(r.cin_phys) / 64;
@@ -1004,6 +1038,17 @@
     ConvConfig f{int(op.r.cout_phys), kHaloStagesTag, 1, 0.0, 1, 0, 1};
     f.halo = 2;
     return f;
+}
+
+std::vector<ConvConfig> proj_conv_candidates(const b2_context* c, const Op& op, int batch) {
+    std::vector<ConvConfig> out;
+    for (int bn : {256, 128, 64})
+        for (int st : {2, 4}) {
+            ConvConfig t{bn, st, 1, 0.0, 1, 0, 1};
+            t.proj = 1;
+            if (tactic_applies(c, op, batch, t)) out.push_back(t);
+        }
+    return out;
 }
 
 std::vector<ConvConfig> conv_candidates(const b2_context* c, const Op& op, int batch, int fixed_splits) {
@@ -1193,9 +1238,25 @@
     const CUtensorMapSwizzle oswz = cl.bn >= 64 ? CU_TENSOR_MAP_SWIZZLE_128B : CU_TENSOR_MAP_SWIZZLE_64B;
     rc = make_map_2d(&cl.mapOut, tptr(r.out), r.cout_phys, uint64_t(M), ow, 128, oswz);
     if (rc) return rc;
-    if (r.res >= 0) rc = make_map_2d(&cl.mapRes, tptr(r.res), r.cout_phys, uint64_t(M), ow, 128, oswz);
+    if (r.res >= 0 && !cfg.proj) rc = make_map_2d(&cl.mapRes, tptr(r.res), r.cout_phys, uint64_t(M), ow, 128, oswz);
     else cl.mapRes = cl.mapOut;
-    return rc;
+    if (rc || !cfg.proj) return rc;
+    const Op& op_p = e->ops[size_t(proj_partner(e, int(&op - &e->ops[0])))];
+    const b2plan::OpRec& rp = op_p.r;
+    const Tensor& tx = e->tensors[rp.in];
+    const int nkb_p = int(rp.cin_phys) / 64;
+    cl.proj = 1;
+    cl.pj.wpacked = e->d_payload + rp.w_off;
+    cl.pj.bias = reinterpret_cast<const float*>(e->d_payload + rp.b_off);
+    cl.pj.num_kblocks = nkb_p;
+    cl.pj.relu = int(rp.relu & b2plan::kConvRelu);
+    a.residual = nullptr;
+    a.num_kblocks = a.kb_per_split = nkb + nkb_p;
+    a.stride_h = a.stride_w = op_p.sh();
+    a.pad_h = a.pad_w = 0;
+    const uint64_t xpix = uint64_t(rp.cin_phys) * 2, xrow = uint64_t(tx.w) * xpix;
+    return make_map_im2col(&cl.mapX, tptr(rp.in), int(rp.cin_phys), int(tx.w), int(tx.h), batch, xpix, xrow, uint64_t(tx.h) * xrow, 1, 1,
+                           op_p.sh(), op_p.sw(), 0, 0, 0, 64, 128, CU_TENSOR_MAP_SWIZZLE_128B);
 }
 
 int make_i8_conv_launch(b2_context* c, const Op& op, int batch, int bn, int stages, b2k::I8ConvLaunch* out) {
@@ -1364,14 +1425,19 @@
     if (!path) return;
     FILE* f = fopen(path, "r");
     if (!f) return;
-    char name[128];
-    int op, batch, bn, st, sp, sps, ws, cn, halo;
-    while (fscanf(f, "%127s %d %d %d %d %d %d %d %d %d", name, &op, &batch, &bn, &st, &sp, &sps, &ws, &cn, &halo) == 10)
+    char line[512], name[128];
+    int op, batch, bn, st, sp, sps, ws, cn, halo, proj;
+    while (fgets(line, sizeof line, f)) {
+        proj = 0;
+        const int n = sscanf(line, "%127s %d %d %d %d %d %d %d %d %d %d", name, &op, &batch, &bn, &st, &sp, &sps, &ws, &cn, &halo, &proj);
+        if (n < 10) break;
         if (e->name == name && op >= 0 && op < int(e->ops.size())) {
             ConvConfig cfg{bn, st, sp, 0.0, sps, ws, cn};
             cfg.halo = halo;
+            cfg.proj = proj;
             e->tuned[{op, batch}] = cfg;
         }
+    }
     fclose(f);
 }
 void tune_cache_append(const b2_engine* e, int op, int batch, const ConvConfig& cfg) {
@@ -1379,8 +1445,8 @@
     if (!path) return;
     FILE* f = fopen(path, "a");
     if (!f) return;
-    fprintf(f, "%s %d %d %d %d %d %d %d %d %d\n", e->name.c_str(), op, batch, cfg.bn, cfg.stages, cfg.splits, cfg.sps, cfg.ws, cfg.cn,
-            cfg.halo);
+    fprintf(f, "%s %d %d %d %d %d %d %d %d %d", e->name.c_str(), op, batch, cfg.bn, cfg.stages, cfg.splits, cfg.sps, cfg.ws, cfg.cn, cfg.halo);
+    fprintf(f, cfg.proj ? " %d\n" : "\n", cfg.proj);
     fclose(f);
 }
 
@@ -1471,16 +1537,19 @@
         e->tuned[{int(i), batch}] = cfg;
         tune_cache_append(e, int(i), batch, cfg);
     }
+    std::map<int, ConvConfig> unfused_3x3;
     for (size_t i = 0; i < e->ops.size() && c->force_fuse >= 0 && c->autotune >= kFuseMinStreams; ++i) {
         const Op& op = e->ops[i];
         const int j = fuse_partner(e, int(i));
         if (j < 0) continue;
         double unfused_us = 0;
+        ConvConfig own;
         {
             std::lock_guard<std::mutex> lock(e->tune_mutex);
             const auto a = e->tuned.find({int(i), batch}), b = e->tuned.find({j, batch});
             if (a == e->tuned.end() || b == e->tuned.end() || a->second.halo == 2 || !(a->second.est_us > 0) || !(b->second.est_us > 0)) continue;
             unfused_us = a->second.est_us + b->second.est_us;
+            own = a->second;
         }
         ConvConfig f = fused_conv_config(op);
         if (!tactic_applies(c, op, batch, f)) continue;
@@ -1500,6 +1569,62 @@
             std::lock_guard<std::mutex> lock(e->tune_mutex);
             e->tuned[{int(i), batch}] = f;
             tune_cache_append(e, int(i), batch, f);
+            unfused_3x3[int(i)] = own;
+        }
+    }
+    for (size_t j = 0; j < e->ops.size() && c->force_proj >= 0 && c->autotune >= kFuseMinStreams; ++j) {
+        const Op& op = e->ops[j];
+        const int p = proj_partner(e, int(j));
+        if (p < 0) continue;
+        const int i = int(j) - 1;
+        const auto fused_with = unfused_3x3.find(i);
+        double rival_us = 0, own_3x3_us = 0;
+        {
+            std::lock_guard<std::mutex> lock(e->tune_mutex);
+            const auto a = e->tuned.find({p, batch}), b = e->tuned.find({int(j), batch});
+            if (a == e->tuned.end() || b == e->tuned.end() || b->second.proj || !(a->second.est_us > 0) || !(b->second.est_us > 0)) continue;
+            const auto f = e->tuned.find({i, batch});
+            const bool fused = i >= 0 && f != e->tuned.end() && f->second.halo == 2;
+            if (fused && fused_with == unfused_3x3.end()) continue;
+            if (fused) {
+                if (!(f->second.est_us > 0)) continue;
+                rival_us = a->second.est_us + f->second.est_us;
+                own_3x3_us = fused_with->second.est_us;
+            } else {
+                rival_us = a->second.est_us + b->second.est_us;
+            }
+        }
+        ConvConfig best{};
+        double best_us = 1e30;
+        for (const ConvConfig& t : proj_conv_candidates(c, op, batch)) {
+            b2k::ConvLaunch cl;
+            int rc = make_conv_launch(c, op, batch, t, &cl);
+            if (rc) return rc;
+            TuneTimer tt(c);
+            if ((rc = tt.init())) return rc;
+            float ms = 0.f;
+            const cudaError_t err = tt.time([&](int, cudaStream_t s) { return b2k::launch_conv_f16_tcgen05(cl, s); }, &ms);
+            if (err != cudaSuccess)
+                return fail(B2_ECUDA, "autotune of %s with its projection %s failed: %s", op.name.c_str(), e->ops[size_t(p)].name.c_str(),
+                            cudaGetErrorString(err));
+            if (tt.us_per_launch(ms) < best_us) best_us = tt.us_per_launch(ms), best = t;
+        }
+        if (best_us >= 1e30) continue;
+        best.est_us = best_us;
+        const bool win = best_us + own_3x3_us < rival_us;
+        if (env_int("B2_TUNE_VERBOSE", 0))
+            fprintf(stderr, "[b2 tune] %s+%s b=%d proj=1 bn=%d st=%d : %.3f us/launch%s against %.3f unfused%s (%d streams) -> %s\n",
+                    e->ops[size_t(p)].name.c_str(), op.name.c_str(), batch, best.bn, best.stages, best_us,
+                    own_3x3_us > 0 ? (" + " + std::to_string(own_3x3_us) + " for the 3x3 alone").c_str() : "", rival_us,
+                    own_3x3_us > 0 ? " (with the fused 3x3)" : "", c->autotune, win ? "proj" : "unfused");
+        if (win) {
+            std::lock_guard<std::mutex> lock(e->tune_mutex);
+            e->tuned[{int(j), batch}] = best;
+            tune_cache_append(e, int(j), batch, best);
+            if (own_3x3_us > 0) {
+                e->tuned[{i, batch}] = fused_with->second;
+                tune_cache_append(e, i, batch, fused_with->second);
+            }
         }
     }
     return B2_OK;
@@ -1525,6 +1650,32 @@
             continue;
         }
         out.push_back(std::move(ls[k]));
+    }
+    for (Launch& L : out)
+        if (L.side_join >= 0) L.side_join = new_index[size_t(L.side_join)];
+    ls = std::move(out);
+}
+
+void fuse_projections(b2_context* c, Plan* plan, int batch) {
+    std::vector<Launch>& ls = plan->launches;
+    std::vector<bool> drop(ls.size(), false);
+    for (Launch& J : ls) {
+        if (J.kind != L_CONV_TC || !J.conv.proj) continue;
+        const int p = proj_partner(c->e, J.op);
+        const auto P = std::find_if(ls.begin(), ls.end(), [&](const Launch& L) { return L.op == p; });
+        if (P == ls.end()) continue;
+        const Tensor& mid = c->e->tensors[c->e->ops[size_t(p)].r.out];
+        J.proj_of = P->name;
+        J.flops += P->flops;
+        J.bytes += P->bytes - 2.0 * batch * double(mid.item_bytes);
+        drop[size_t(P - ls.begin())] = true;
+    }
+    if (std::none_of(drop.begin(), drop.end(), [](bool d) { return d; })) return;
+    std::vector<int> new_index(ls.size());
+    std::vector<Launch> out;
+    for (size_t k = 0; k < ls.size(); ++k) {
+        new_index[k] = int(out.size());
+        if (!drop[k]) out.push_back(std::move(ls[k]));
     }
     for (Launch& L : out)
         if (L.side_join >= 0) L.side_join = new_index[size_t(L.side_join)];
@@ -1587,6 +1738,7 @@
         L.name = op.name;
         L.N = batch;
         L.side_join = op.side_join;
+        L.op = int(&op - &e->ops[0]);
         switch (r.type) {
             case b2plan::OP_INPUT_CAST: {
                 const Tensor& t = e->tensors[r.out];
@@ -1673,6 +1825,19 @@
                         const ConvConfig f = fused_conv_config(op);
                         if (tactic_applies(c, op, batch, f)) cfg = f;
                     }
+                    if (c->force_proj > 0 && !cfg.proj) {
+                        ConvConfig f = cfg;
+                        f.proj = 1, f.sps = 1, f.splits = 1, f.ws = 0, f.cn = 1, f.halo = 0;
+                        if (!tactic_applies(c, op, batch, f))
+                            for (const ConvConfig& t : proj_conv_candidates(c, op, batch))
+                                if (!tactic_applies(c, op, batch, f) || t.bn == cfg.bn) {
+                                    f = t;
+                                    if (t.bn == cfg.bn) break;
+                                }
+                        if (tactic_applies(c, op, batch, f)) cfg = f;
+                    }
+                    if (cfg.proj && !plan->launches.empty() && plan->launches.back().kind == L_CONV_TC && plan->launches.back().conv.halo == 2)
+                        cfg.proj = 0;
                     if (op.side_join >= 0 && cfg.splits > 1) cfg.splits = 1;
                     int rc = make_conv_launch(c, op, batch, cfg, &L.conv);
                     if (rc) return rc;
@@ -1846,6 +2011,7 @@
         plan->launches.push_back(std::move(L));
     }
     fuse_bottlenecks(c, plan.get(), batch);
+    fuse_projections(c, plan.get(), batch);
     fuse_tail(c, plan.get(), batch);
     {
         const std::vector<Launch>& ls = plan->launches;
@@ -2287,6 +2453,7 @@
     c->force_cn = env_int("B2_FORCE_CN", 0);
     c->force_halo = env_int("B2_FORCE_HALO", 0);
     c->force_fuse = env_int("B2_FORCE_FUSE", 0);
+    c->force_proj = env_int("B2_FORCE_PROJ", 0);
     c->pdl_trigger = env_int("B2_PDL_TRIGGER", 1);
     c->autotune = env_int("B2_AUTOTUNE", 4);
     c->fork = env_int("B2_FORK", 0);
@@ -2351,6 +2518,7 @@
     else if (k == "cn") c->force_cn = value;
     else if (k == "halo") c->force_halo = value;
     else if (k == "fuse") c->force_fuse = value;
+    else if (k == "proj") c->force_proj = value;
     else if (k == "fork") c->fork = value;
     else if (k == "fuse_tail") c->fuse_tail = value;
     else if (k == "i8_bn") c->i8_bn = value;
@@ -2561,7 +2729,7 @@
         if (n >= cap) break;
         const ConvConfig& g = kv.second;
         const uint32_t rec[10] = {uint32_t(kv.first.first), uint32_t(kv.first.second), uint32_t(g.bn), uint32_t(g.stages), uint32_t(g.splits),
-                                  uint32_t(g.sps), uint32_t(g.ws), uint32_t(g.cn), uint32_t(g.halo), 0u};
+                                  uint32_t(g.sps), uint32_t(g.ws), uint32_t(g.cn), uint32_t(g.halo), uint32_t(g.proj)};
         memcpy(out + size_t(n) * 10, rec, sizeof rec);
         ++n;
     }
@@ -2711,7 +2879,7 @@
              " st=" + std::to_string(L->conv.stages) + "x" + std::to_string(L->conv.sps) +
              (L->conv.ws_ctas ? " ws=" + std::to_string(L->conv.ws_ctas) : std::string()) +
              (L->conv.cn > 1 ? " cn=" + std::to_string(L->conv.cn) : std::string()) +
-             (L->conv.halo == 2 ? " halo fused" : L->conv.halo ? " halo" : "") +
+             (L->conv.halo == 2 ? " halo fused" : L->conv.halo ? " halo" : "") + (L->conv.proj ? " proj=" + L->proj_of : std::string()) +
              (L->conv.args.a_mode == b2k::A_TILED ? " tiled" : " im2col") +
              " grid=" + std::to_string(L->conv.grid_n) + "x" + std::to_string(L->conv.grid_m) + "x" +
              std::to_string(L->conv.args.splits) + " kblk=" + std::to_string(L->conv.args.num_kblocks) +
diff --git a/tensorrt_laboratory_b200/csrc/kernels.cu b/tensorrt_laboratory_b200/csrc/kernels.cu
--- a/tensorrt_laboratory_b200/csrc/kernels.cu
+++ b/tensorrt_laboratory_b200/csrc/kernels.cu
@@ -41,13 +41,12 @@
         : row0(64 * (consumer_warp >> 2) + 16 * (consumer_warp & 3) + (lane >> 2)), col0(2 * (lane & 3)) {}
 };
 
-template <int BN, int KB, int STAGES, int SPS, int CN = 1, bool DBG = false, int AV = 0, bool GELU = false, bool LIVE = false>
-__global__ void __launch_bounds__(kConvThreads, conv_min_ctas(BN))
-conv_f16_tcgen05(const __grid_constant__ CUtensorMap mapA, const __grid_constant__ CUtensorMap mapB,
-                 const __grid_constant__ CUtensorMap mapOut, const __grid_constant__ CUtensorMap mapRes,
-                 const ConvArgs p) {
+template <int BN, int KB, int STAGES, int SPS, int CN, bool DBG, int AV, bool GELU, bool LIVE, bool PROJ>
+__device__ __forceinline__ void conv_f16_tile(const CUtensorMap& mapA, const CUtensorMap& mapB, const CUtensorMap& mapOut,
+                                              const CUtensorMap& mapRes, const ConvArgs p, const CUtensorMap& mapX, const ProjArgs q) {
     static_assert(SPS == 1 || KB == 64, "multi-sub-block stages exist for the 64-wide K path only");
     static_assert(!LIVE || AV == 2, "live-row instantiations exist for the tiled packed-weight path only");
+    static_assert(!PROJ || (AV == 2 && SPS == 1 && !GELU && !LIVE), "the projection variant exists for the tiled packed-weight path only");
     using Cfg = ConvCfg<BN, STAGES, SPS>;
     constexpr int TPS = 64 / KB;
     constexpr int A_SUB = 128 * KB * 2;
@@ -58,7 +57,7 @@
 
     extern __shared__ uint8_t smem_raw[];
     uint8_t* smem = smem_raw + ((1024u - (smem_u32(smem_raw) & 1023u)) & 1023u);
-    const bool has_res = p.residual != nullptr;
+    const bool has_res = PROJ || p.residual != nullptr;
     uint8_t* sA = smem;
     uint8_t* sB = smem + STAGES * Cfg::A_STAGE;
     uint8_t* sOut = smem;
@@ -70,6 +69,7 @@
     uint64_t* res_bar = accum_bar + 1;
     uint32_t* last_flag = reinterpret_cast<uint32_t*>(res_bar + 1);
     float* s_bias = reinterpret_cast<float*>(tail + 256);
+    float* s_bias_p = s_bias + BN;
 
     const int warp = threadIdx.x >> 5;
     const int lane = threadIdx.x & 31;
@@ -106,12 +106,13 @@
         tma_prefetch_desc(&mapA);
         tma_prefetch_desc(&mapB);
         tma_prefetch_desc(&mapOut);
-        if (has_res) tma_prefetch_desc(&mapRes);
+        if (PROJ) tma_prefetch_desc(&mapX);
+        else if (has_res) tma_prefetch_desc(&mapRes);
         for (int s = 0; s < STAGES; ++s) {
             mbar_init(&full_bar[s], 1);
             mbar_init(&empty_bar[s], static_cast<uint32_t>(kConsumerWarps * cn));
         }
-        mbar_init(res_bar, 1);
+        mbar_init(res_bar, PROJ ? 32 : 1);
         fence_barrier_init();
         fence_proxy_async();
     }
@@ -120,6 +121,11 @@
     if (warp == kWgtWarp) {
 #pragma unroll
         for (int i = 0; i < BN / 32; ++i) s_bias[lane + 32 * i] = __ldg(p.bias + n0 + lane + 32 * i);
+        if constexpr (PROJ) {
+#pragma unroll
+            for (int i = 0; i < BN / 32; ++i) s_bias_p[lane + 32 * i] = __ldg(q.bias + n0 + lane + 32 * i);
+            mbar_arrive(res_bar);
+        }
     }
     if (p.pdl_trigger == 0) pdl_launch_dependents();
     if (dbg && threadIdx.x == 0) dbg[1] = clock64();
@@ -144,8 +150,14 @@
             const int ns = subs_in_step((kb - kb_begin) / SPS);
             for (int u = 0; u < ns; ++u) {
                 if (w_packed) {
-                    bulk_load_1d(&full_bar[s], b_dst + u * Cfg::B_SUBBLK,
-                                 p.wpacked + (static_cast<size_t>(kb + u) * (p.Cout >> 5) + (n0 >> 5)) * 4096, BN * 128);
+                    const uint8_t* w = p.wpacked;
+                    int wkb = kb + u;
+                    if constexpr (PROJ) {
+                        if (wkb < q.num_kblocks) w = q.wpacked;
+                        else wkb -= q.num_kblocks;
+                    }
+                    bulk_load_1d(&full_bar[s], b_dst + u * Cfg::B_SUBBLK, w + (static_cast<size_t>(wkb) * (p.Cout >> 5) + (n0 >> 5)) * 4096,
+                                 BN * 128);
                 } else {
                     tma_load_2d(&mapB, &full_bar[s], b_dst + u * Cfg::B_SUBBLK, (kb + u) * 64, n0);
                 }
@@ -167,7 +179,7 @@
             const int slice_rows = 128 / cn;
             int ms = m0 + static_cast<int>(crank) * slice_rows;
             const uint32_t slice_off = crank * static_cast<uint32_t>(slice_rows) * 128u;
-            if (!a_tiled) {
+            if (PROJ || !a_tiled) {
                 if (ms >= p.M) ms = 0;
                 img0 = ms / p.HoWo;
                 const int rem = ms - img0 * p.HoWo;
@@ -188,6 +200,11 @@
             auto load_a = [&](int kb, int s) {
                 if (skip_a) return;
                 uint8_t* a_dst = sA + s * Cfg::A_STAGE;
+                if constexpr (PROJ) {
+                    if (kb < q.num_kblocks) tma_load_im2col_4d(&mapX, &full_bar[s], a_dst, kb * 64, base_w, base_h, img0, 0, 0);
+                    else tma_load_2d(&mapA, &full_bar[s], a_dst, (kb - q.num_kblocks) * 64, m0);
+                    return;
+                }
                 if (KB == 64) {
                     const int ns = subs_in_step((kb - kb_begin) / SPS);
                     for (int u = 0; u < ns; ++u) {
@@ -247,7 +264,7 @@
             if (dbg && lane == 0) dbg[2] = clock64();
             if (!dead && elect_one_sync()) {
                 for (int i = 0; i < npre; ++i) load_a(kb_begin + i * SPS, i);
-                if (has_res && !split) load_residual();
+                if (!PROJ && has_res && !split) load_residual();
             }
             __syncwarp();
             long long tw = 0, te = 0, tl = 0;
@@ -273,6 +290,12 @@
         }
         __syncwarp();
     }
+
+    auto stage_off = [](int row, int col) -> uint32_t {
+        const int box = col / OW;
+        const int chunk = (col % OW) / 8;
+        return static_cast<uint32_t>(box * (128 * OROWB)) + swz_off<OROWB>(row, chunk) + (col % 8) * 2;
+    };
 
     const int cw = warp;
     const bool consumer = warp < kConsumerWarps;
@@ -310,7 +333,7 @@
                     const int u = t >> 2, j = t & 3;
                     const uint64_t ad = make_wgmma_desc(a_addr + u * Cfg::A_SUBBLK + wg * 8192 + j * 32, 16, 1024, WG_SW128);
                     const uint64_t bd = make_wgmma_desc(b_addr + u * Cfg::B_SUBBLK + j * 32, 16, 1024, WG_SW128);
-                    wgmma_f16<BN>(acc, ad, bd, (i > 0 || t > 0) ? 1u : 0u);
+                    wgmma_f16<BN>(acc, ad, bd, ((PROJ ? i != 0 && i != q.num_kblocks : i > 0) || t > 0) ? 1u : 0u);
                 };
                 if (SPS == 1 || subs_in_step(i) == SPS) wgmma_group<4 * SPS>(mma);
                 else wgmma_group<4>(mma);
@@ -338,6 +361,26 @@
                 wgmma_wait<1>();
                 if (i > 0) release_stage((i - 1) % STAGES);
             }
+            if constexpr (PROJ) {
+                if (i == q.num_kblocks - 1) {
+                    wgmma_wait<0>();
+                    mbar_wait(res_bar, 0);
+                    const FragPos fq(cw, lane);
+#pragma unroll
+                    for (int j = 0; j < BN / 8; ++j) {
+#pragma unroll
+                        for (int h = 0; h < 2; ++h) {
+                            const int row = fq.row0 + 8 * h, col = 8 * j + fq.col0;
+                            float v0 = acc[4 * j + 2 * h] + s_bias_p[col], v1 = acc[4 * j + 2 * h + 1] + s_bias_p[col + 1];
+                            if (q.relu) {
+                                v0 = fmaxf(v0, 0.0f);
+                                v1 = fmaxf(v1, 0.0f);
+                            }
+                            *reinterpret_cast<__half2*>(sRes + stage_off(row, col)) = __floats2half2_rn(v0, v1);
+                        }
+                    }
+                }
+            }
             if (dbg) mi += clock64() - m1c;
         }
         if constexpr (STAGES > 1) {
@@ -372,9 +415,7 @@
     const FragPos fp(cw, lane);
 
     auto finish_pair = [&](int row, int col, float v0, float v1) {
-        const int box = col / OW;
-        const int chunk = (col % OW) / 8;
-        const uint32_t so = static_cast<uint32_t>(box * (128 * OROWB)) + swz_off<OROWB>(row, chunk) + (col % 8) * 2;
+        const uint32_t so = stage_off(row, col);
         v0 += s_bias[col];
         v1 += s_bias[col + 1];
         if (has_res) {
@@ -395,7 +436,7 @@
     bool do_store = true;
     if (!split) {
         if (consumer) {
-            if (has_res) mbar_wait(res_bar, 0);
+            if (!PROJ && has_res) mbar_wait(res_bar, 0);
 #pragma unroll
             for (int j = 0; j < BN / 8; ++j)
 #pragma unroll
@@ -468,6 +509,21 @@
         asm volatile("mov.u64 %0, %%globaltimer;" : "=l"(gt));
         dbg[9] = static_cast<long long>(gt);
     }
+}
+
+template <int BN, int KB, int STAGES, int SPS, int CN = 1, bool DBG = false, int AV = 0, bool GELU = false, bool LIVE = false>
+__global__ void __launch_bounds__(kConvThreads, conv_min_ctas(BN))
+conv_f16_tcgen05(const __grid_constant__ CUtensorMap mapA, const __grid_constant__ CUtensorMap mapB,
+                 const __grid_constant__ CUtensorMap mapOut, const __grid_constant__ CUtensorMap mapRes,
+                 const ConvArgs p) {
+    conv_f16_tile<BN, KB, STAGES, SPS, CN, DBG, AV, GELU, LIVE, false>(mapA, mapB, mapOut, mapRes, p, mapA, ProjArgs{});
+}
+
+template <int BN, int STAGES>
+__global__ void __launch_bounds__(kConvThreads, conv_min_ctas(BN))
+conv_f16_proj_tcgen05(const __grid_constant__ CUtensorMap mapA, const __grid_constant__ CUtensorMap mapOut,
+                      const __grid_constant__ CUtensorMap mapX, const ConvArgs p, const ProjArgs q) {
+    conv_f16_tile<BN, 64, STAGES, 1, 1, false, 2, false, false, true>(mapA, mapA, mapOut, mapA, p, mapX, q);
 }
 
 __host__ __device__ constexpr int conv_ws_smem_bytes(int bn, int stages, int sps, bool residual) {
@@ -1311,6 +1367,39 @@
     X(32, 8, 2, 1) X(32, 8, 4, 1) X(64, 8, 2, 1) X(64, 8, 4, 1) X(64, 8, 8, 1) X(128, 8, 4, 1) \
     X(32, 32, 2, 1) X(32, 32, 4, 1) X(64, 32, 1, 1) X(64, 32, 2, 1) X(64, 32, 4, 1) X(128, 32, 2, 1) X(128, 32, 4, 1)
 
+#define B2_FOR_EACH_CONV_PROJ(X) X(64, 2) X(64, 4) X(128, 2) X(128, 4) X(256, 2)
+
+int conv_proj_smem(int bn, int stages) { return conv_smem_layout_bytes(bn, stages, true) + bn * 4; }
+bool conv_proj_config_exists(int bn, int stages) {
+#define B2_HAS_PROJ(BN_, ST_) \
+    if (bn == BN_ && stages == ST_) return true;
+    B2_FOR_EACH_CONV_PROJ(B2_HAS_PROJ)
+#undef B2_HAS_PROJ
+    return false;
+}
+static int init_conv_proj_kernels() {
+    int e = 0;
+#define B2_INIT_PROJ(BN_, ST_) \
+    if ((e = set_conv_smem(conv_f16_proj_tcgen05<BN_, ST_>, conv_proj_smem(BN_, ST_)))) return e;
+    B2_FOR_EACH_CONV_PROJ(B2_INIT_PROJ)
+#undef B2_INIT_PROJ
+    return e;
+}
+static int launch_conv_proj(const ConvLaunch& L, cudaStream_t stream) {
+    const ConvArgs& a = L.args;
+    if (L.kb != 64 || L.sps != 1 || L.cn != 1 || L.ws_ctas || a.splits != 1 || a.kb_per_split < a.num_kblocks || a.a_mode != A_TILED ||
+        !a.wpacked || a.residual || (a.relu & 8) || a.live || !L.pj.wpacked || L.pj.num_kblocks < 1 || a.num_kblocks <= L.pj.num_kblocks)
+        return static_cast<int>(cudaErrorInvalidValue);
+    const dim3 grid(L.grid_n, L.grid_m, 1);
+#define B2_CASE_PROJ(BN_, ST_)                                                                                                         \
+    if (L.bn == BN_ && L.stages == ST_)                                                                                                \
+        return launch_kernel(conv_f16_proj_tcgen05<BN_, ST_>, grid, dim3(kConvThreads), size_t(conv_proj_smem(BN_, ST_)),            \
+                             stream, true, L.mapA, L.mapOut, L.mapX, L.args, L.pj);
+    B2_FOR_EACH_CONV_PROJ(B2_CASE_PROJ)
+#undef B2_CASE_PROJ
+    return static_cast<int>(cudaErrorInvalidValue);
+}
+
 int conv_halo_smem(int bn, int w, int r, int cblocks) { return halo_smem_bytes(bn, w, r, cblocks); }
 bool conv_halo_config_exists(int bn) { return bn == 64 || bn == 128 || bn == 256; }
 static int init_conv_halo_kernels() {
@@ -1374,6 +1463,7 @@
                                                    conv_stem_ws_smem_bytes()))))
         return e;
     if ((e = init_conv_halo_kernels())) return e;
+    if ((e = init_conv_proj_kernels())) return e;
 #define B2_INIT(BN_, KB_, ST_, SPS_) \
     if ((e = init_one<BN_, KB_, ST_, SPS_>())) return e;
     B2_FOR_EACH_CONV(B2_INIT)
@@ -1387,6 +1477,7 @@
 
 int launch_conv_f16_tcgen05(const ConvLaunch& L, cudaStream_t stream) {
     if (L.halo) return launch_conv_halo(L, stream);
+    if (L.proj) return launch_conv_proj(L, stream);
     if (L.ws_ctas > 0) return L.kb == 32 ? launch_conv_stem_ws(L, stream) : launch_conv_f16_tcgen05_ws(L, stream);
     if (L.cn > 1) {
 #define B2_CASE_CL(BN_, ST_, SPS_, CN_) \
diff --git a/tensorrt_laboratory_b200/csrc/kernels.h b/tensorrt_laboratory_b200/csrc/kernels.h
--- a/tensorrt_laboratory_b200/csrc/kernels.h
+++ b/tensorrt_laboratory_b200/csrc/kernels.h
@@ -50,6 +50,13 @@
     int relu;
 };
 
+struct ProjArgs {
+    const uint8_t* wpacked;
+    const float* bias;
+    int num_kblocks;
+    int relu;
+};
+
 struct ConvLaunch {
     CUtensorMap mapA;
     CUtensorMap mapB;
@@ -65,6 +72,9 @@
     int halo;
     int ws_ctas;
     Conv1x1Args c2;
+    int proj;
+    CUtensorMap mapX;
+    ProjArgs pj;
 };
 
 int launch_conv_f16_tcgen05(const ConvLaunch& L, cudaStream_t stream);
@@ -72,6 +82,8 @@
 bool conv_config_exists(int bn, int kb, int stages, int sps = 1);
 int conv_smem_bytes(int bn, int stages, bool residual, int sps = 1);
 bool conv_cluster_config_exists(int bn, int stages, int sps, int cn);
+bool conv_proj_config_exists(int bn, int stages);
+int conv_proj_smem(int bn, int stages);
 bool conv_halo_config_exists(int bn);
 int conv_halo_smem(int bn, int w, int r, int cblocks);
 int conv_halo_fused_smem(int bn, int w, int r, int cblocks, int cout2);
diff --git a/tensorrt_laboratory_b200/csrc/plan_format.h b/tensorrt_laboratory_b200/csrc/plan_format.h
--- a/tensorrt_laboratory_b200/csrc/plan_format.h
+++ b/tensorrt_laboratory_b200/csrc/plan_format.h
@@ -45,7 +45,8 @@
     uint64_t tactics_offset;
 };
 struct TacticRec {
-    uint32_t op, batch, bn, stages, splits, sps, ws, cn, halo, reserved;
+    uint32_t op, batch, bn, stages, splits, sps, ws, cn, halo;
+    uint32_t proj;
 };
 struct TensorRec {
     char name[64];
```

Measured after the change: 33760, median of 6. 2.5% higher.
